# PatrykChrabaszcz/HpBandSter

Hardware: AMD Instinct MI355X
Metric: candidate KDE evals/sec (cand×obs pairs) at D=32, 1/2/4/8 MI355X; % VALU peak (higher is better)
Workload: dtype f16 MFMA coarse pre-screen (1 product per dim, rigorous bound), f32 accumulate, f64 re-score

## Files before the change

### hpbandster_amd/_native.py

```python

import ctypes
import os
import threading

_HERE = os.path.dirname(os.path.abspath(__file__))
LIB_PATH = os.environ.get("HBX_LIB_PATH") or os.path.join(_HERE, "_lib", "libhbx.so")
DIAGNOSTIC_BUILD = bool(os.environ.get("HBX_LIB_PATH"))

_lock = threading.Lock()
_lib = None

c_i32, c_i64, c_f64p, c_vp = ctypes.c_int32, ctypes.c_int64, ctypes.c_void_p, ctypes.c_void_p

SIGNATURES = {
    "hbx_last_error": (ctypes.c_char_p, []),
    "hbx_version": (ctypes.c_char_p, []),
    "hbx_kde_param_bytes": (c_i64, []),
    "hbx_kde_param_bw_offset": (c_i64, []),
    "hbx_kde_est_bytes": (c_i64, []),
    "hbx_acq_result_bytes": (c_i64, []),
    "hbx_max_dims": (c_i32, []),
    "hbx_sort_scratch_bytes": (c_i64, [c_i64]),
    "hbx_seg_argsort": (c_i32, [c_vp, c_vp, c_i64, c_i64, c_i64, c_vp, c_vp, c_i64, c_vp]),
    "hbx_kde_fit": (c_i32, [c_vp, c_i32, c_vp, c_i64, c_vp, c_vp, c_vp, c_vp, c_vp, c_vp, c_vp, c_vp, c_vp,
                            c_vp, c_vp]),
    "hbx_kde_bucket": (c_i32, [c_i32, c_i32, c_vp, c_vp, c_vp]),
    "hbx_kde_table_floats": (c_i64, [c_i32, c_i32, c_i32]),
    "hbx_kde_prepare": (c_i32, [c_vp, c_i32, c_vp, c_i32, c_vp, c_vp, c_vp, c_vp, c_vp, c_i64, c_vp, c_vp]),
    "hbx_kde_refit_out_bytes": (c_i64, [c_i64, c_i32]),
    "hbx_kde_refit_scratch_bytes": (c_i64, [c_i64, c_i32]),
    "hbx_kde_refit": (c_i32, [c_vp, c_vp, c_i64, c_i32, c_vp, c_vp, c_i64, c_i64, c_i64, ctypes.c_double,
                              ctypes.c_double, c_vp, c_vp, c_i64, c_vp, c_vp, c_i64, c_vp, c_vp, c_i64, c_vp]),
    "hbx_kde_refit_sync": (c_i32, [c_vp, c_vp, c_i64, c_i32, c_vp, c_vp, c_i64, c_i64, c_i64, ctypes.c_double,
                                   ctypes.c_double, c_vp, c_vp, c_i64, c_vp, c_vp, c_i64, c_vp, c_vp, c_i64,
                                   c_vp, c_vp]),
    "hbx_stream_order": (c_i32, [c_vp, c_vp]),
    "hbx_kde_logpdf": (c_i32, [c_vp, c_i64, c_i32, c_vp, c_vp, c_i32, c_i32, c_i32, c_vp, c_vp]),
    "hbx_kde_workspace_bytes": (c_i64, [c_i64, c_i64]),
    "hbx_kde_acquire": (c_i32, [c_vp, c_i64, c_i64, c_vp, c_vp, c_vp, c_vp, c_i64, c_vp, c_vp]),
    "hbx_kde_pair_bind": (c_vp, [c_i32, c_vp, c_vp, c_vp, c_vp, c_i32, c_vp, c_vp, c_vp, c_vp, c_i32, c_i32, c_i32,
                                 c_i64]),
    "hbx_kde_acquire_bound": (c_i32, [c_vp, c_vp, c_i64, c_i64, c_vp, c_i64, c_vp, c_vp, c_vp, c_vp, c_vp]),
    "hbx_kde_pair_free": (None, [c_vp]),
    "hbx_kde_batch_workspace_bytes": (c_i64, [c_i64, c_i64, c_i64]),
    "hbx_kde_acquire_batch": (c_i32, [c_vp, c_i64, c_i64, c_i64, c_vp, c_vp, c_vp, c_vp, c_vp, c_i64, c_vp]),
    "hbx_kde_topk_workspace_bytes": (c_i64, [c_i64, c_i32, c_i64]),
    "hbx_kde_topk_result_bytes": (c_i64, [c_i32]),
    "hbx_kde_acquire_topk": (c_i32, [c_vp, c_i64, c_i32, c_i64, c_vp, c_vp, c_vp, c_i64, c_vp]),
    "hbx_kde_groups_workspace_bytes": (c_i64, [c_i64, c_i64, c_i32]),
    "hbx_kde_acquire_groups": (c_i32, [c_vp, c_i32, c_vp, c_i64, c_vp, c_vp, c_vp, c_vp, c_vp, c_vp, c_vp, c_vp,
                                       c_vp, c_i64, c_vp, c_vp, c_i64, c_vp]),
    "hbx_kde_groups_batch_workspace_bytes": (c_i64, [c_i64, c_i64, c_i64, c_i32]),
    "hbx_kde_acquire_groups_batch": (c_i32, [c_vp, c_i32, c_vp, c_i64, c_vp, c_vp, c_vp, c_vp, c_vp, c_vp, c_vp,
                                             c_vp, c_vp, c_i64, c_i64, c_vp, c_vp, c_i64, c_vp]),
    "hbx_kde_groups_topk_workspace_bytes": (c_i64, [c_i64, c_i64, c_i32, c_i32]),
    "hbx_kde_acquire_groups_topk": (c_i32, [c_vp, c_i32, c_vp, c_i64, c_vp, c_vp, c_vp, c_vp, c_vp, c_vp, c_vp, c_vp,
                                            c_vp, c_i64, c_i32, c_vp, c_vp, c_i64, c_vp]),
    "hbx_kde_logpdf_groups_workspace_bytes": (c_i64, [c_i64, c_i64, c_i32]),
    "hbx_kde_logpdf_groups": (c_i32, [c_vp, c_i32, c_vp, c_i64, c_vp, c_vp, c_vp, c_vp, c_vp, c_vp, c_vp, c_vp, c_vp,
                                      c_i64, ctypes.c_double, c_i32, c_vp, c_vp, c_vp, c_vp, c_i64, c_vp]),
    "hbx_kde_logpdf_groups_stats": (c_i32, [c_vp, c_vp]),
    "hbx_kde_sample_groups": (c_i32, [c_vp, c_i32, c_vp, c_i64, c_vp, c_vp, c_vp, c_vp, ctypes.c_double,
                                      ctypes.c_uint64, ctypes.c_uint64, ctypes.c_uint32, c_i64, c_vp, c_vp, c_vp]),
    "hbx_kde_finish_groups": (c_i32, [c_vp, c_vp, c_vp, c_vp, c_i32, c_i64, c_i64, c_i64, ctypes.c_double,
                                      ctypes.c_uint64, ctypes.c_uint64, ctypes.c_uint32, c_vp, c_vp, c_vp]),
    "hbx_kde_propose_groups_workspace_bytes": (c_i64, [c_i64, c_i64, c_i64, c_i32]),
    "hbx_kde_propose_groups_ws_offsets": (c_i32, [c_i64, c_i64, c_i64, c_i32, c_vp]),
    "hbx_kde_propose_groups": (c_i32, [c_vp, c_i32, c_vp, c_i64, c_vp, c_vp, c_vp, c_vp, c_vp, c_vp, c_vp, c_vp, c_vp,
                                       ctypes.c_double, ctypes.c_double, ctypes.c_uint64, ctypes.c_uint64,
                                       ctypes.c_uint32, c_i64, c_i64, c_vp, c_vp, c_vp, c_vp, c_vp, c_i64, c_vp]),
    "hbx_philox4x32_10": (c_i32, [c_vp, c_vp, c_vp]),
    "hbx_kde_sample": (c_i32, [c_vp, c_i32, c_vp, c_i64, c_vp, c_vp, c_vp, ctypes.c_double, ctypes.c_uint64,
                               ctypes.c_uint64, ctypes.c_uint32, c_i64, c_vp, c_vp, c_vp, c_vp]),
    "hbx_norm_ppf": (c_i32, [c_vp, c_i64, c_vp, c_vp]),
    "hbx_kde_sample_table_bytes": (c_i64, [c_i64, c_i32]),
    "hbx_kde_sample_table": (c_i32, [c_vp, c_i32, c_vp, c_i64, c_vp, c_vp, c_vp, c_vp]),
    "hbx_kde_cv_terms": (c_i32, [c_vp, c_i64, c_i32, c_vp, c_vp, c_vp, c_vp, c_vp, ctypes.c_double,
                                 ctypes.c_double, ctypes.c_double, c_vp, c_vp, c_vp]),
    "hbx_event_create": (c_i32, [c_vp]),
    "hbx_event_destroy": (c_i32, [c_vp]),
    "hbx_event_elapsed_ms": (c_i32, [c_vp, c_vp, c_vp]),
    "hbx_kde_result_ptr": (c_vp, [c_vp]),
    "hbx_fetch": (c_i32, [c_vp, c_vp, c_i64, c_vp]),
    "hbx_mapped_host_buffers": (c_i64, []),
    "hbx_kde_ws_offsets": (c_i32, [c_i64, c_i64, c_i64, c_vp]),
    "hbx_kde_acquire_stats": (c_i32, [c_vp, c_i64, c_i64, c_vp]),
    "hbx_np_exp": (c_i32, [c_vp, c_i64, c_vp, c_vp]),
    "hbx_kde_pdf_scratch_bytes": (c_i64, [c_i64]),
    "hbx_kde_pdf_exact": (c_i32, [c_vp, c_i64, c_i32, c_vp, c_vp, c_vp, c_i64, c_vp, c_vp, c_i64, c_vp]),
    "hbx_kde_logpdf_exact": (c_i32, [c_vp, c_i64, c_i32, c_vp, c_vp, c_vp, c_vp, c_vp]),
    "hbx_rccl_unique_id_bytes": (c_i64, []),
    "hbx_rccl_get_unique_id": (c_i32, [c_vp]),
    "hbx_rccl_comm_init": (c_i32, [c_vp, c_i32, c_vp, c_i32, c_i32]),
    "hbx_rccl_comm_count": (c_i32, [c_vp, c_vp]),
    "hbx_rccl_comm_destroy": (c_i32, [c_vp]),
    "hbx_argmax_gather_bytes": (c_i64, [c_i32]),
    "hbx_argmax_allreduce": (c_i32, [c_vp, c_vp, c_vp, c_i32, c_vp, c_vp]),
    "hbx_argmax_records": (c_i32, [c_vp, c_i32, c_vp, c_vp]),
    "hbx_sh_promote": (c_i32, [c_vp, c_vp, c_i64, c_i64, c_i64, c_vp, c_vp, c_vp, c_vp, c_vp, c_i64, c_vp]),
    "hbx_seg_argsort_ex": (c_i32, [c_vp, c_vp, c_i64, c_i64, c_i64, c_vp, c_vp, c_i64, c_i32, c_vp]),
    "hbx_sh_promote_scratch_bytes": (c_i64, [c_i64, c_i64, c_i64, c_i32, c_i32]),
    "hbx_sh_promote_ex": (c_i32, [c_vp, c_vp, c_i64, c_i64, c_i64, c_vp, c_vp, c_vp, c_vp, c_vp, c_i64, c_i32,
                                  c_vp, c_vp]),
    "hbx_sh_promote_one": (c_i32, [c_vp, c_i64, ctypes.c_double, c_vp, c_vp, c_i32, c_vp, c_i32, c_vp]),
    "hbx_sh_advance_mapped": (c_i32, [c_vp, c_i64, ctypes.c_double, c_vp, c_vp, c_vp, c_vp, c_i32, c_vp, c_i32,
                                      c_vp]),
    "hbx_sh_advance_state": (c_i32, [c_vp, c_i64, ctypes.c_double, c_vp]),
    "hbx_host_alloc": (c_i32, [c_i64, c_vp]),
    "hbx_kde_logpdf_rtol_scratch_bytes": (c_i64, [c_i64]),
    "hbx_kde_logpdf_rtol": (c_i32, [c_vp, c_i64, c_i32, c_vp, c_vp, c_vp, c_vp, c_i32, c_i32, c_i32, ctypes.c_double,
                                    c_vp, c_vp, c_i64, c_vp]),
    "hbx_host_free": (c_i32, [c_vp]),
    "hbx_np_argsort_host": (c_i32, [c_vp, c_i64, c_vp]),
    "hbx_sh_advance_host": (c_i32, [c_vp, c_i64, c_i64, c_vp, c_vp]),
    "hbx_mt_state_bytes": (c_i64, []),
    "hbx_mt_draw": (c_i32, [c_vp, c_i32, c_i64, c_i64, c_vp]),
    "hbx_bohb_draw": (c_i32, [c_vp, c_vp, c_i64, c_i32, c_vp, c_vp, ctypes.c_double, c_i64, c_vp, c_vp, c_vp, c_vp,
                              c_vp, c_vp, c_vp]),
}

ORDER_NUMPY = 0
ORDER_STABLE = 1


def order_mode(name):
    if name in ("numpy", ORDER_NUMPY):
        return ORDER_NUMPY
    if name in ("stable", ORDER_STABLE):
        return ORDER_STABLE
    raise ValueError("tie order must be 'numpy' or 'stable', got %r" % (name,))


class HbxError(RuntimeError):
    pass


def lib():
    global _lib
    if _lib is not None:
        return _lib
    with _lock:
        if _lib is not None:
            return _lib
        if not os.path.exists(LIB_PATH):
            raise HbxError("libhbx.so not found at %s -- build it with `python -m hpbandster_amd.build` "
                           "(the engine has no CPU fallback)" % LIB_PATH)
        import torch
        L = ctypes.CDLL(LIB_PATH)
        for name, (res, args) in SIGNATURES.items():
            if DIAGNOSTIC_BUILD and not hasattr(L, name):
                continue
            f = getattr(L, name)
            f.restype = res
            f.argtypes = args
        _lib = L
        return _lib


def check(rc):
    if rc != 0:
        msg = lib().hbx_last_error()
        raise HbxError("libhbx error %d: %s" % (rc, msg.decode() if msg else "?"))


def call(name, *args):
    check(getattr(lib(), name)(*args))


def ptr(t):
    if t is None:
        return None
    if hasattr(t, "data_ptr"):
        return t.data_ptr()
    return t.ctypes.data


_RAW = None


def _raw_fns():
    global _RAW
    if _RAW is None:
        import torch
        _RAW = (getattr(torch._C, "_cuda_getDevice", None), getattr(torch._C, "_cuda_getCurrentRawStream", None))
    return _RAW


def stream_handle(stream=None, device=None):
    if stream is not None:
        return stream.cuda_stream
    import torch
    raw = _raw_fns()[1]
    if raw is not None:
        idx = None if device is None else device if isinstance(device, int) else torch.device(device).index
        return raw(torch.cuda.current_device() if idx is None else int(idx))
    return torch.cuda.current_stream(device).cuda_stream


def home_stream(dev_index):
    cur, raw = _RAW or _raw_fns()
    if cur is not None and raw is not None and cur() == dev_index:
        return raw(dev_index)
    return None


class on_device(object):

    def __init__(self, device, stream=None):
        import torch
        self._ctx = [torch.cuda.device(device)]
        if stream is not None:
            self._ctx.append(torch.cuda.stream(stream))

    def __enter__(self):
        for c in self._ctx:
            c.__enter__()
        return self

    def __exit__(self, *exc):
        for c in reversed(self._ctx):
            c.__exit__(*exc)
        return False
```

### hpbandster_amd/csrc/hbx_acquire.h

```cpp
#pragma once
#include "hbx_score.h"

struct KdePairRef {
  int32_t D;
  const void* params_good;
  const float* table_good;
  const double* X_good;
  const int64_t* rows_good;
  int32_t variant_good;
  const void* params_bad;
  const float* table_bad;
  const double* X_bad;
  const int64_t* rows_bad;
  int32_t variant_bad, dc_pad, du_pad;
  int64_t nmax;
  const KdeParams* Pg() const { return (const KdeParams*)params_good; }
  const KdeParams* Pb() const { return (const KdeParams*)params_bad; }
};

struct WsLayout {
  size_t res, U, count, flags, segcnt, segnear, best, key, first1, rescue, est_l, est_g, lo, list, near, exact_l,
      exact_g, part, total;
  size_t stage, seeds, surv, lpart;
  int32_t list_cap;
};
#define STAGED_LIST_CAP 4096
WsLayout ws_layout(int64_t Nc, int64_t nmax, int64_t B = 1);

struct AcqWs {
  AcqResult* res;
  uint32_t* U;
  int32_t *count, *flags, *segcnt, *segnear;
  uint64_t *best, *key;
  int32_t *first1, *rescue;
  KdeEst *el, *eg;
  float* lo;
  int32_t *list, *near;
  double *exact_l, *exact_g, *part;
  uint32_t* stage;
  int32_t *seeds, *surv;
  KdeEst* lpart;
  int32_t list_cap;
  AcqWs(void* workspace, const WsLayout& w) {
    char* ws = (char*)workspace;
    res = (AcqResult*)(ws + w.res);
    U = (uint32_t*)(ws + w.U);
    count = (int32_t*)(ws + w.count);
    flags = (int32_t*)(ws + w.flags);
    segcnt = (int32_t*)(ws + w.segcnt);
    segnear = (int32_t*)(ws + w.segnear);
    best = (uint64_t*)(ws + w.best);
    key = (uint64_t*)(ws + w.key);
    first1 = (int32_t*)(ws + w.first1);
    rescue = (int32_t*)(ws + w.rescue);
    el = (KdeEst*)(ws + w.est_l);
    eg = (KdeEst*)(ws + w.est_g);
    lo = (float*)(ws + w.lo);
    list = (int32_t*)(ws + w.list);
    near = (int32_t*)(ws + w.near);
    exact_l = (double*)(ws + w.exact_l);
    exact_g = (double*)(ws + w.exact_g);
    part = (double*)(ws + w.part);
    stage = (uint32_t*)(ws + w.stage);
    seeds = (int32_t*)(ws + w.seeds);
    surv = (int32_t*)(ws + w.surv);
    lpart = (KdeEst*)(ws + w.lpart);
    list_cap = w.list_cap;
  }
  KdePairArgs::AcqInitPtrs init() const { return {U, count, flags, first1, res}; }
};

struct AcqPlan {
  ScoreFns fg, fb;
  bool exact_only;
};
const KdePairRef* acq_pair(const char* who, const void* pair);
int acq_check(const char* who, const KdePairRef& p, const double* cand, int64_t Nc, const void* workspace);
int acq_plan(const KdePairRef& p, bool fast, AcqPlan* plan);
int acq_score(const AcqPlan& plan, const KdePairRef& p, const AcqWs& a, const ScoreRequest& rq, int64_t batch_B,
              ScoreResult* out);
#ifndef HBX_STAGED_MIN_PAIRS
#define HBX_STAGED_MIN_PAIRS 1e9
#endif
#ifndef HBX_STAGED_TOPK_MIN_PAIRS
#define HBX_STAGED_TOPK_MIN_PAIRS 4e9
#endif
bool acq_staged_supported(const AcqPlan& plan);
int acq_score_staged(const AcqPlan& plan, const KdePairRef& p, const double* cand, int64_t Nc, const AcqWs& a,
                     hipEvent_t* ev, hipStream_t s, bool tail);
int staged_score_l(const AcqPlan& plan, const KdePairRef& p, const double* cand, int64_t Nc, const AcqWs& a,
                   hipEvent_t* ev, hipStream_t s, uint32_t* lkey, uint32_t* hist, int32_t hist_words);
int staged_score_seeds(const AcqPlan& plan, const KdePairRef& p, const double* cand, int64_t Nc, const AcqWs& a,
                       hipStream_t s, bool mark_rest, bool update_u);
int staged_score_survivors(const AcqPlan& plan, const KdePairRef& p, const double* cand, int64_t Nc, const AcqWs& a,
                           hipStream_t s, bool lonly);
int acq_exact_only_init(int64_t Nc, uint32_t seg, const AcqWs& a, hipStream_t s);
#define EXACT_SCAN_MAX 1024
int acq_exact(const KdePairRef& p, const double* cand, int64_t Nc, const AcqWs& a, bool scan, bool combine,
              hipStream_t s);
```

### hpbandster_amd/csrc/hbx_common.h

```cpp
#pragma once

#include <hip/hip_runtime.h>
#include <stdint.h>
#include <stdlib.h>

#define HBX_MAX_D 256
#define HBX_WAVE 64

#include "hbx.h"

int hbx_fail(int code, const char* fmt, ...);

#define HBX_HIP(call)                                                                 \
  do {                                                                                \
    hipError_t _e = (call);                                                           \
    if (_e != hipSuccess)                                                             \
      return hbx_fail(HBX_ERR_HIP, "%s failed: %s (%s:%d)", #call, hipGetErrorString(_e), \
                      __FILE__, __LINE__);                                            \
  } while (0)

#define HBX_LAUNCH_CHECK()                                                            \
  do {                                                                                \
    hipError_t _e = hipGetLastError();                                                \
    if (_e != hipSuccess)                                                             \
      return hbx_fail(HBX_ERR_HIP, "kernel launch failed: %s (%s:%d)",               \
                      hipGetErrorString(_e), __FILE__, __LINE__);                    \
  } while (0)

static inline bool hbx_switch_on(const char* name) {
  const char* e = getenv(name);
  return !(e && atoi(e) == 0);
}
static inline int hbx_staged_mode() {
  const char* e = getenv("HBX_STAGED");
  if (!e) return 1;
  const int v = atoi(e);
  return v == 0 ? 0 : v == 2 ? 2 : 1;
}
static inline bool hbx_staged_tail() { return hbx_switch_on("HBX_STAGED_TAIL"); }

struct KdeParams {
  int32_t n;
  int32_t D;
  int32_t dc;
  int32_t du;
  int32_t nconst;
  int32_t nan_all;
  int32_t has_neg;
  int32_t unsupported;
  int32_t stride;
  int32_t dc_pad;
  int32_t du_pad;
  int32_t exact_only;
  double log_norm;
  double m0_log2;
  double lb_sum;
  double prod_bw_c;
  float cmax;
  float sum_abs_delta;
  float cmax2;
  int32_t pad1;
  int32_t kc;
  int32_t hmode;
  int32_t nsc;
  int32_t chunk_floats;
  int32_t oh_total;
  int32_t coarse_off;
  int32_t coarse_chunk_floats;
  const double* X;
  const int64_t* rows;
  int32_t oh_dim[64];
  int32_t oh_level[64];
  int32_t oh_col[64];
  double oh_val[64];
  int32_t oh_start[64];
  int32_t cat_maxcode[HBX_MAX_D];
  int32_t cont_dim[HBX_MAX_D];
  double cont_scale[HBX_MAX_D];
  double center[HBX_MAX_D];
  float xmax[HBX_MAX_D];
  int32_t cat_dim[HBX_MAX_D];
  float cat_delta[HBX_MAX_D];
  float cat_negf[HBX_MAX_D];
  int32_t const_dim[HBX_MAX_D];
  double const_level[HBX_MAX_D];
  int32_t vartype[HBX_MAX_D];
  int32_t nlev[HBX_MAX_D];
  double bw[HBX_MAX_D];
};

#define HBX_PARAM_STAGE ((sizeof(KdeParams) + 255) & ~(size_t)255)
#define HBX_COLSTATS_OFF (HBX_PARAM_STAGE + 8 * HBX_MAX_D + 4 * HBX_MAX_D + 64)
#define HBX_PARAM_BYTES (HBX_COLSTATS_OFF + 8 * HBX_MAX_D + 4 * HBX_MAX_D)
struct ColStats {
  double mean[HBX_MAX_D];
  int32_t maxcode[HBX_MAX_D];
};

struct KdeEst {
  float lpos;
  float lneg;
  float err;
  float pad;
};

struct AcqResult {
  int64_t index;
  double score;
  float rel;
  int32_t flags;
  int32_t shortlist;
  int32_t near;
  double pdf_l;
  double pdf_g;
};

__device__ __forceinline__ void hbx_publish_store(uint32_t* dst, uint32_t v) {
  __hip_atomic_store(dst, v, __ATOMIC_RELAXED, __HIP_MEMORY_SCOPE_SYSTEM);
}
__device__ __forceinline__ void hbx_publish_store64(uint64_t* dst, uint64_t v) {
  __hip_atomic_store(dst, v, __ATOMIC_RELAXED, __HIP_MEMORY_SCOPE_SYSTEM);
}
__device__ __forceinline__ void hbx_publish_done(int32_t* done, int32_t seq) {
  __asm__ volatile("s_waitcnt vmcnt(0)" ::: "memory");
  __hip_atomic_store(done, seq, __ATOMIC_RELAXED, __HIP_MEMORY_SCOPE_SYSTEM);
}

__device__ __forceinline__ uint32_t hbx_f2ord(float f) {
  uint32_t u = __float_as_uint(f);
  return (u & 0x80000000u) ? ~u : (u | 0x80000000u);
}
__device__ __forceinline__ float hbx_ord2f(uint32_t u) {
  return __uint_as_float((u & 0x80000000u) ? (u & 0x7fffffffu) : ~u);
}

__device__ __forceinline__ uint64_t hbx_d2ord(double d) {
  if (d != d) return ~0ull;
  if (d == 0.0) d = 0.0;
  uint64_t u = (uint64_t)__double_as_longlong(d);
  return (u & 0x8000000000000000ull) ? ~u : (u | 0x8000000000000000ull);
}

template <typename Op>
__device__ __forceinline__ uint32_t wave_reduce_dpp(uint32_t v, Op op) {
  v = op(v, (uint32_t)__builtin_amdgcn_update_dpp(0, (int)v, 0xb1, 0xf, 0xf, false));
  v = op(v, (uint32_t)__builtin_amdgcn_update_dpp(0, (int)v, 0x4e, 0xf, 0xf, false));
  v = op(v, (uint32_t)__builtin_amdgcn_update_dpp(0, (int)v, 0x141, 0xf, 0xf, false));
  v = op(v, (uint32_t)__builtin_amdgcn_update_dpp(0, (int)v, 0x140, 0xf, 0xf, false));
  return op(op((uint32_t)__builtin_amdgcn_readlane((int)v, 0), (uint32_t)__builtin_amdgcn_readlane((int)v, 16)),
            op((uint32_t)__builtin_amdgcn_readlane((int)v, 32), (uint32_t)__builtin_amdgcn_readlane((int)v, 48)));
}
struct OpAdd { __device__ uint32_t operator()(uint32_t a, uint32_t b) const { return a + b; } };
struct OpAnd { __device__ uint32_t operator()(uint32_t a, uint32_t b) const { return a & b; } };
struct OpOr { __device__ uint32_t operator()(uint32_t a, uint32_t b) const { return a | b; } };
struct OpMax { __device__ uint32_t operator()(uint32_t a, uint32_t b) const { return a > b ? a : b; } };
```

### hpbandster_amd/csrc/hbx_kde.hip

```cpp
#include "hbx_acquire.h"

#include <string.h>

#include <new>

#include "hbx_acq_impl.h"
#include "hbx_host.h"
#include "hbx_pairwise.h"
#include "hbx_rescue_impl.h"


__global__ void acq_init_kernel(uint32_t* U, int32_t* count, int32_t* flags, int32_t* first1, AcqResult* res) {
  if (threadIdx.x == 0 && blockIdx.x == 0) acq_init_state(U, count, flags, first1, res);
}

__global__ void acq_init_batch_kernel(int64_t B, uint32_t* __restrict__ U, int32_t* __restrict__ flags,
                                      int32_t* __restrict__ segcnt, uint64_t* __restrict__ best,
                                      uint64_t* __restrict__ key, int32_t* __restrict__ first1,
                                      int32_t* __restrict__ count, int32_t* __restrict__ segnear) {
  const int64_t b = (int64_t)blockIdx.x * blockDim.x + threadIdx.x;
  if (b == 0) *count = 0;
  if (b < B) {
    U[b] = hbx_f2ord(INFINITY);
    flags[b] = 0;
// ... 160 lines not shown
  const bool all = (flags[sg] & 1) != 0;
  const float l = lo[i];
  if ((l == l && (all || l <= u)) || (int32_t)i == first1[sg]) {
    const int pos = atomicAdd(count, 1);
    list[pos] = (int32_t)i;
    if (segcnt) atomicAdd(segcnt + sg, 1);
  }
}

struct PickOut {
  const double* cand;
  const uint8_t* err;
  int64_t Nc;
  int32_t D;
  char* out;
};

__global__ __launch_bounds__(256) void kde_final_kernel(const int32_t* __restrict__ list,
                                                        const int32_t* __restrict__ count,
                                                        const double* exact_l,
                                                        const double* exact_g, const int32_t* __restrict__ flags,
                                                        int64_t index_base, const KdeParams* __restrict__ Pg,
                                                        const KdeParams* __restrict__ Pb,
                                                        const KdeEst* __restrict__ el, const KdeEst* __restrict__ eg,
                                                        int32_t* __restrict__ near_list, AcqResult* __restrict__ res,
                                                        int32_t nbuf, const double* __restrict__ part,
                                                        double* exact_lw, double* exact_gw, AcqResult* host_res,
                                                        int32_t seq, PickOut pick) {
  __shared__ double bs[256];
  __shared__ AcqResult rec_sh;
  __shared__ int64_t bi[256];
  __shared__ int32_t bp[256];
  __shared__ double exl[256], exg[256];
  __shared__ double rb_sh;
  __shared__ int32_t nnear;
  const int cnt = *count;
  int err_any = 0;
  if (pick.out && pick.err) {
    bool e = false;
    for (int64_t i = threadIdx.x; i < pick.Nc; i += 256) e = e || pick.err[i] != 0;
    err_any = __syncthreads_or(e);
  }
  const bool small = cnt <= 256;
  const int tp = threadIdx.x;
  const int64_t my_idx = (small && tp < cnt) ? list[tp] : 0;
  const double my_rel = (small && tp < cnt) ? score_rel(Pg, Pb, el, eg, my_idx) : 0.0;
  if (part && cnt <= EXACT_SPLIT_CAP) {
    for (int pk = threadIdx.x >> 6; pk < 2 * cnt; pk += 4) {
      const bool isl = pk & 1;
      const int n = (isl ? Pg : Pb)->n;
      const double* us = part + (int64_t)pk * nbuf * PW_SPLIT_UNITS;
      double acc = 0.0;
      for (int c = 0, b = 0; c < n; c += PW_BUF, ++b) {
        const int m = (n - c) < PW_BUF ? (n - c) : PW_BUF;
        acc = acc + pw_combine_units_wave<PW_SPLIT_CUT>(m, us + b * PW_SPLIT_UNITS);
      }
      if ((threadIdx.x & 63) == 0) {
        const double pdf = acc / (double)n;
        (isl ? exact_lw : exact_gw)[pk >> 1] = pdf;
        if (small) (isl ? exl : exg)[pk >> 1] = pdf;
      }
    }
    __threadfence_block();
    __syncthreads();
  } else if (small) {
    if (tp < cnt) {
      exl[tp] = exact_l[tp];
      exg[tp] = exact_g[tp];
    }
    __syncthreads();
  }
  double best = INFINITY;
  int64_t bidx = INT64_MAX;
  int32_t bpos = -1;
  if (threadIdx.x == 0) nnear = 0;
  for (int p = threadIdx.x; p < cnt; p += 256) {
    const double s = bohb_score(small ? exg[p] : exact_g[p], small ? exl[p] : exact_l[p]);
    const int64_t idx = small ? my_idx : list[p];
    if (s < INFINITY && (s < best || (s == best && idx < bidx))) {
      best = s;
      bidx = idx;
      bpos = p;
    }
  }
  bs[threadIdx.x] = best;
  bi[threadIdx.x] = bidx;
  bp[threadIdx.x] = bpos;
  __syncthreads();
  for (int w = 128; w > 0; w >>= 1) {
    if (threadIdx.x < w) {
      const double s2 = bs[threadIdx.x + w];
      const int64_t i2 = bi[threadIdx.x + w];
      if (s2 < bs[threadIdx.x] || (s2 == bs[threadIdx.x] && i2 < bi[threadIdx.x])) {
        bs[threadIdx.x] = s2;
        bi[threadIdx.x] = i2;
        bp[threadIdx.x] = bp[threadIdx.x + w];
      }
    }
    __syncthreads();
  }
  const int32_t wp = bp[0];
  double rb = 0.0;
  if (small) {
    if (tp == wp) rb_sh = my_rel;
    __syncthreads();
    if (wp >= 0) rb = rb_sh;
  }
  if (wp >= 0) {
    const double sb = bs[0];
    if (!small) rb = score_rel(Pg, Pb, el, eg, list[wp]);
    for (int p = threadIdx.x; p < cnt; p += 256) {
      const double s = bohb_score(small ? exg[p] : exact_g[p], small ? exl[p] : exact_l[p]);
      const int64_t ip = small ? my_idx : list[p];
      if (p == wp || near_best(s, small ? my_rel : score_rel(Pg, Pb, el, eg, ip), sb, rb))
        near_list[atomicAdd(&nnear, 1)] = (int32_t)ip;
    }
  }
  __syncthreads();
  if (threadIdx.x == 0) {
    AcqResult r;
    r.index = -1;
    r.score = r.pdf_l = r.pdf_g = NAN;
    r.shortlist = cnt;
    r.flags = *flags | (nnear > 1 ? HBX_ACQ_NEAR_TIE : 0);
    r.near = nnear;
    r.rel = (float)rb;
    if (wp >= 0) {
      r.index = bi[0] + index_base;
      r.score = bs[0];
      r.pdf_l = small ? exl[wp] : exact_l[wp];
      r.pdf_g = small ? exg[wp] : exact_g[wp];
    }
    *res = r;
    rec_sh = r;
  }
  if (host_res || pick.out) {
    static_assert(sizeof(AcqResult) % 4 == 0, "record of whole words");
    __syncthreads();
    uint64_t* out = (uint64_t*)(pick.out ? pick.out : (char*)host_res);
    const uint64_t tag = (uint64_t)(uint32_t)seq << 32;
    constexpr int RW = (int)(sizeof(AcqResult) / 4);
    if (threadIdx.x < RW) hbx_publish_store64(out + threadIdx.x, tag | ((const uint32_t*)&rec_sh)[threadIdx.x]);
    if (pick.out) {
      if (threadIdx.x == 0) hbx_publish_store64(out + RW, tag | (err_any ? 1u : 0u));
      const int64_t idx = rec_sh.index - index_base;
      if (rec_sh.index >= 0 && idx < pick.Nc)
        for (int w = threadIdx.x; w < 2 * pick.D; w += 256)
          hbx_publish_store64(out + RW + 1 + w, tag | ((const uint32_t*)(pick.cand + idx * pick.D))[w]);
    }
  }
}


__global__ __launch_bounds__(256) void kde_batch_min_kernel(const int32_t* __restrict__ list,
                                                            const int32_t* __restrict__ count, uint32_t seg,
                                                            const double* __restrict__ exact_l,
                                                            const double* __restrict__ exact_g,
                                                            uint64_t* __restrict__ best) {
  const int p = blockIdx.x * 256 + threadIdx.x;
  if (p >= *count) return;
  const double s = bohb_score(exact_g[p], exact_l[p]);
  if (s < INFINITY) atomicMin((unsigned long long*)best + (uint32_t)list[p] / seg,
                              (unsigned long long)__double_as_longlong(s));
}

__global__ __launch_bounds__(256) void kde_batch_key_kernel(const int32_t* __restrict__ list,
                                                            const int32_t* __restrict__ count, uint32_t seg,
                                                            const double* __restrict__ exact_l,
                                                            const double* __restrict__ exact_g,
                                                            const uint64_t* __restrict__ best,
                                                            uint64_t* __restrict__ key) {
  const int p = blockIdx.x * 256 + threadIdx.x;
  if (p >= *count) return;
  const double s = bohb_score(exact_g[p], exact_l[p]);
  const uint32_t i = (uint32_t)list[p], sg = i / seg;
  if (s < INFINITY && (uint64_t)__double_as_longlong(s) == best[sg])
    atomicMin((unsigned long long*)key + sg, ((unsigned long long)(i - sg * seg) << 32) | (uint32_t)p);
}

__global__ __launch_bounds__(256) void kde_batch_near_kernel(const int32_t* __restrict__ list,
                                                             const int32_t* __restrict__ count, uint32_t seg,
                                                             const double* __restrict__ exact_l,
                                                             const double* __restrict__ exact_g,
                                                             const uint64_t* __restrict__ key,
                                                             const KdeParams* __restrict__ Pg,
                                                             const KdeParams* __restrict__ Pb,
                                                             const KdeEst* __restrict__ el,
                                                             const KdeEst* __restrict__ eg,
                                                             int32_t* __restrict__ near_flag,
                                                             int32_t* __restrict__ segnear) {
  const int p = blockIdx.x * 256 + threadIdx.x;
  if (p >= *count) return;
  const uint32_t i = (uint32_t)list[p], sg = i / seg;
  const uint64_t k = key[sg];
  int f = 0;
  if (k != ~0ull) {
    const int wp = (int)(uint32_t)k;
    const double sb = bohb_score(exact_g[wp], exact_l[wp]);
    const double rb = score_rel(Pg, Pb, el, eg, list[wp]);
    const double s = bohb_score(exact_g[p], exact_l[p]);
    f = (p == wp || near_best(s, score_rel(Pg, Pb, el, eg, i), sb, rb)) ? 1 : 0;
  }
  near_flag[p] = f;
  if (f) atomicAdd(segnear + sg, 1);
}

__global__ __launch_bounds__(256) void kde_batch_final_kernel(int64_t B, const uint64_t* __restrict__ key,
                                                              const int32_t* __restrict__ segcnt,
                                                              const int32_t* __restrict__ flags,
                                                              const int32_t* __restrict__ segnear,
                                                              const int32_t* __restrict__ list,
                                                              const double* __restrict__ exact_l,
                                                              const double* __restrict__ exact_g,
                                                              const KdeParams* __restrict__ Pg,
                                                              const KdeParams* __restrict__ Pb,
                                                              const KdeEst* __restrict__ el,
                                                              const KdeEst* __restrict__ eg,
                                                              int64_t index_base, AcqResult* __restrict__ res) {
  const int64_t b = (int64_t)blockIdx.x * 256 + threadIdx.x;
  if (b >= B) return;
  AcqResult r;
  r.shortlist = segcnt[b];
  r.near = segnear[b];
  r.flags = flags[b] | (r.near > 1 ? HBX_ACQ_NEAR_TIE : 0);
  r.rel = 0.f;
  const uint64_t k = key[b];
  if (k == ~0ull) {
    r.index = -1;
    r.score = NAN;
    r.pdf_l = NAN;
    r.pdf_g = NAN;
  } else {
    const int p = (int)(uint32_t)k;
    r.index = (int64_t)(k >> 32) + index_base;
    r.pdf_l = exact_l[p];
    r.pdf_g = exact_g[p];
    r.score = bohb_score(r.pdf_g, r.pdf_l);
    r.rel = (float)score_rel(Pg, Pb, el, eg, list[p]);
  }
  res[b] = r;
}

__global__ __launch_bounds__(256) void kde_exact_only_init_kernel(int64_t Nc, uint32_t seg, KdeEst* __restrict__ el,
                                                                  KdeEst* __restrict__ eg, float* __restrict__ lo,
                                                                  int32_t* __restrict__ flags) {
  const int64_t i = (int64_t)blockIdx.x * 256 + threadIdx.x;
  if (i >= Nc) return;
  const KdeEst e = {0.f, -INFINITY, -2.f, 0.f};
  el[i] = e;
  eg[i] = e;
  lo[i] = 0.f;
  if ((uint32_t)i % seg == 0) flags[(uint32_t)i / seg] = HBX_ACQ_OVERFLOW;
}

__global__ __launch_bounds__(256) void kde_exact_logs_kernel(const int32_t* __restrict__ list,
                                                             const int32_t* __restrict__ count,
                                                             const double* __restrict__ exact_l,
                                                             const double* __restrict__ exact_g,
                                                             float* __restrict__ logl, float* __restrict__ logg) {
  const int p = blockIdx.x * 256 + threadIdx.x;
  if (p >= *count) return;
  const int i = list[p];
  if (logl) logl[i] = (float)log(exact_l[p]);
  if (logg) logg[i] = (float)log(exact_g[p]);
}


WsLayout ws_layout(int64_t Nc, int64_t nmax, int64_t B) {
  WsLayout w;
  size_t o = 0;
  auto take = [&](size_t bytes) {
    size_t r = o;
    o += (bytes + 255) & ~(size_t)255;
    return r;
  };
  w.res = take(sizeof(AcqResult));
  w.count = take(4);
  w.U = take(4 * B);
  w.flags = take(4 * B);
  w.segcnt = take(4 * B);
  w.segnear = take(4 * B);
  w.best = take(8 * B);
  w.key = take(8 * B);
  w.first1 = take(4 * B);
  w.rescue = take(4);
  const int sp = obs_splits((unsigned)((Nc + 511) / 512), nmax, true);
  const int64_t cap16 = 16 * Nc < 196608 ? 16 * Nc : 196608;
  const int64_t nest = Nc * sp > cap16 ? Nc * sp : cap16;
  w.est_l = take(sizeof(KdeEst) * nest);
  w.est_g = take(sizeof(KdeEst) * nest);
  w.lo = take(4 * Nc);
  w.list = take(4 * Nc);
  w.near = take(4 * Nc);
  w.exact_l = take(8 * Nc);
  w.exact_g = take(8 * Nc);
  w.part = take(8 * (size_t)2 * EXACT_SPLIT_CAP * PW_SPLIT_UNITS * ((nmax + PW_BUF - 1) / PW_BUF));
  static_assert(sizeof(AcqResult) + 4 * HBX_ST_WORDS <= 256, "the state words fit the result slot's padding");
  w.stage = w.res + sizeof(AcqResult);
  const int64_t tiles = (Nc + 511) / 512;
  w.list_cap = (int32_t)(512 * (tiles < 1 ? 1 : tiles > STAGED_LIST_CAP / 512 ? STAGED_LIST_CAP / 512 : tiles));
  w.seeds = take(4 * (size_t)w.list_cap);
  w.surv = take(4 * Nc);
  w.lpart = take(sizeof(KdeEst) * (size_t)OBS_SPLIT_MAX * w.list_cap);
  w.total = o;
  return w;
}

int acq_check(const char* who, const KdePairRef& p, const double* cand, int64_t Nc, const void* workspace) {
  if ((!cand && Nc > 0) || !p.params_good || !p.table_good || !p.X_good || !p.rows_good || !p.params_bad ||
      !p.table_bad || !p.X_bad || !p.rows_bad || !workspace)
    return hbx_fail(HBX_ERR_ARG, "%s: null pointer", who);
  if (Nc < 0 || Nc > INT32_MAX) return hbx_fail(HBX_ERR_ARG, "Nc=%lld out of range", (long long)Nc);
  return HBX_OK;
}

const KdePairRef* acq_pair(const char* who, const void* pair) {
  if (!pair) hbx_fail(HBX_ERR_ARG, "%s: null pair", who);
  return (const KdePairRef*)pair;
}

int acq_plan(const KdePairRef& p, bool fast, AcqPlan* plan) {
  plan->exact_only = KdeVariant::decode(p.variant_good).exact_only || KdeVariant::decode(p.variant_bad).exact_only;
  plan->fg = pick_logpdf(p.dc_pad, p.du_pad, p.variant_good, fast);
  plan->fb = pick_logpdf(p.dc_pad, p.du_pad, p.variant_bad, fast);
  if (!plan->exact_only && (!plan->fg.main || !plan->fb.main))
    return hbx_fail(HBX_ERR_UNSUPPORTED, "no kernel for dc_pad=%d du_pad=%d", p.dc_pad, p.du_pad);
  return HBX_OK;
}

int acq_score(const AcqPlan& plan, const KdePairRef& p, const AcqWs& a, const ScoreRequest& rq, int64_t batch_B,
              ScoreResult* out) {
  *out = ScoreResult{};
  const hipStream_t s = rq.s;
  const bool scored = rq.Nc > 0 && !plan.exact_only;
  if (scored) {
    const int rc = launch_score2({plan.fg, p.params_good, p.table_good, a.el},
                                 {plan.fb, p.params_bad, p.table_bad, a.eg}, rq, out);
    if (rc) return rc;
  }
  if (batch_B) {
    hipLaunchKernelGGL(acq_init_batch_kernel, dim3((unsigned)((batch_B + 255) / 256)), dim3(256), 0, s, batch_B, a.U,
                       a.flags, a.segcnt, a.best, a.key, a.first1, a.count, a.segnear);
    HBX_LAUNCH_CHECK();
  } else if (!out->inited) {
    hipLaunchKernelGGL(acq_init_kernel, dim3(1), dim3(64), 0, s, a.U, a.count, a.flags, a.first1, a.res);
    HBX_LAUNCH_CHECK();
  }
  if (scored && (out->nsplit[0] > 1 || out->nsplit[1] > 1)) {
    hipLaunchKernelGGL(kde_merge_splits_kernel, dim3((unsigned)((2 * rq.Nc + 255) / 256)), dim3(256), 0, s, a.el,
                       a.eg, rq.Nc, out->nsplit[0], out->nsplit[1]);
    HBX_LAUNCH_CHECK();
  }
  return HBX_OK;
}

int acq_exact_only_init(int64_t Nc, uint32_t seg, const AcqWs& a, hipStream_t s) {
  hipLaunchKernelGGL(kde_exact_only_init_kernel, dim3((unsigned)((Nc + 255) / 256)), dim3(256), 0, s, Nc, seg, a.el,
                     a.eg, a.lo, a.flags);
  HBX_LAUNCH_CHECK();
  return HBX_OK;
}

struct AcqCall {
  const char* who;
  const double* cand;
  int64_t Nc, seg, index_base;
  float *logl_out, *logg_out;
  AcqResult* batch_res;
  void* workspace;
  int64_t ws_bytes;
  void *events, *stream;
  AcqResult* host_res;
  int32_t seq;
  PickOut pick;
};

static int acquire_impl(const void* pair, const AcqCall& c) {
  const KdePairRef* pp = acq_pair(c.who, pair);
  if (!pp) return HBX_ERR_ARG;
  const KdePairRef& p = *pp;
  const double* cand = c.cand;
  const int64_t Nc = c.Nc, seg = c.seg;
  float *logl_out = c.logl_out, *logg_out = c.logg_out;
  AcqResult* batch_res = c.batch_res;
  int rc = acq_check(c.who, p, cand, Nc, c.workspace);
  if (rc) return rc;
  if (seg < 1) return hbx_fail(HBX_ERR_ARG, "%s: segment length %lld", c.who, (long long)seg);
  const int64_t B = batch_res ? (Nc + seg - 1) / seg : 1;
  const WsLayout w = ws_layout(Nc, p.nmax, B);
  if ((size_t)c.ws_bytes < w.total)
    return hbx_fail(HBX_ERR_ARG, "workspace too small: %lld < %lld bytes", (long long)c.ws_bytes,
                    (long long)w.total);
  const bool fast = !logl_out && !logg_out;
  AcqPlan plan;
  rc = acq_plan(p, fast, &plan);
  if (rc) return rc;
  const AcqWs a(c.workspace, w);
  hipStream_t s = (hipStream_t)c.stream;
  hipEvent_t* ev = (hipEvent_t*)c.events;
  const uint32_t sg = (uint32_t)(batch_res ? seg : (Nc > 0 ? Nc : 1));
  if (B == 0) return HBX_OK;
  bool rescue_inline = false;
  const int stg = (!batch_res && fast && Nc > 0) ? hbx_staged_mode() : 0;
  const bool staged = stg && acq_staged_supported(plan) &&
                      (stg == 2 || (double)Nc * (double)p.nmax >= HBX_STAGED_MIN_PAIRS);
  const bool tail = staged && hbx_staged_tail();
  if (staged) {
    rc = acq_score_staged(plan, p, cand, Nc, a, ev, s, tail);
    rescue_inline = true;
  } else {
    const ScoreRequest rq{cand, Nc, p.D, ev, a.rescue, batch_res ? KdePairArgs::AcqInitPtrs{} : a.init(),
                          fast ? p.nmax : 0, !batch_res, s};
    ScoreResult sr;
    rc = acq_score(plan, p, a, rq, batch_res ? B : 0, &sr);
    rescue_inline = sr.rescue_inline;
  }
  if (rc) return rc;
  const dim3 grid((unsigned)((Nc + 255) / 256));
  bool fuse_combine = false;
  if (Nc > 0) {
    if (plan.exact_only) {
      rc = acq_exact_only_init(Nc, sg, a, s);
      if (rc) return rc;
    } else if (!tail) {
      const CombineRescue rs{cand, p.D, p.Pg(), p.Pb(), a.rescue};
      const bool sgn = KdeVariant::decode(p.variant_good).has_neg;
      const combine_fn cf = !rescue_inline ? kde_combine_kernel<false, false>
                            : sgn          ? kde_combine_kernel<true, true>
                                           : kde_combine_kernel<false, true>;
      hipLaunchKernelGGL(cf, dim3((unsigned)((Nc + 256 * COMBINE_SUB - 1) / (256 * COMBINE_SUB))), dim3(256), 0, s,
                         a.el, a.eg, Nc, sg, logl_out, logg_out, a.lo, a.U, a.flags, a.first1, rs);
      HBX_LAUNCH_CHECK();
    }
    const bool scan = !batch_res && Nc <= EXACT_SCAN_MAX && !tail;
    if (!scan && !tail) {
      hipLaunchKernelGGL(kde_shortlist_kernel, grid, dim3(256), 0, s, a.lo, Nc, sg, a.U, a.flags, a.list, a.count,
                         batch_res ? a.segcnt : (int32_t*)nullptr, a.first1, a.rescue);
      HBX_LAUNCH_CHECK();
    }
    fuse_combine = !batch_res && !(plan.exact_only && (logl_out || logg_out));
    rc = acq_exact(p, cand, Nc, a, scan, !fuse_combine, s);
    if (rc) return rc;
    if (plan.exact_only && (logl_out || logg_out)) {
      hipLaunchKernelGGL(kde_exact_logs_kernel, grid, dim3(256), 0, s, a.list, a.count, a.exact_l, a.exact_g, logl_out,
                         logg_out);
      HBX_LAUNCH_CHECK();
    }
  }
  if (!batch_res) {
    hipLaunchKernelGGL(kde_final_kernel, dim3(1), dim3(256), 0, s, a.list, a.count, a.exact_l, a.exact_g, a.flags,
                       c.index_base, p.Pg(), p.Pb(), a.el, a.eg, a.near, a.res,
                       (int32_t)((p.nmax + PW_BUF - 1) / PW_BUF), fuse_combine ? a.part : (const double*)nullptr,
                       a.exact_l, a.exact_g, c.host_res, c.seq, c.pick);
    HBX_LAUNCH_CHECK();
    return HBX_OK;
  }
  if (Nc > 0) {
    hipLaunchKernelGGL(kde_batch_min_kernel, grid, dim3(256), 0, s, a.list, a.count, sg, a.exact_l, a.exact_g, a.best);
    HBX_LAUNCH_CHECK();
    hipLaunchKernelGGL(kde_batch_key_kernel, grid, dim3(256), 0, s, a.list, a.count, sg, a.exact_l, a.exact_g, a.best,
                       a.key);
    HBX_LAUNCH_CHECK();
    hipLaunchKernelGGL(kde_batch_near_kernel, grid, dim3(256), 0, s, a.list, a.count, sg, a.exact_l, a.exact_g, a.key,
                       p.Pg(), p.Pb(), a.el, a.eg, a.near, a.segnear);
    HBX_LAUNCH_CHECK();
    hipLaunchKernelGGL(kde_batch_final_kernel, dim3((unsigned)((B + 255) / 256)), dim3(256), 0, s, B, a.key, a.segcnt,
                       a.flags, a.segnear, a.list, a.exact_l, a.exact_g, p.Pg(), p.Pb(), a.el, a.eg, c.index_base,
                       batch_res);
    HBX_LAUNCH_CHECK();
  }
  return HBX_OK;
}

extern "C" {

int64_t hbx_kde_workspace_bytes(int64_t Nc, int64_t nmax) { return (int64_t)ws_layout(Nc, nmax).total; }

int64_t hbx_kde_batch_workspace_bytes(int64_t Nc, int64_t seg, int64_t nmax) {
  if (seg < 1) return -1;
  return (int64_t)ws_layout(Nc, nmax, (Nc + seg - 1) / seg).total;
}

void* hbx_kde_result_ptr(void* workspace) { return (char*)workspace + ws_layout(0, 0).res; }

int hbx_kde_acquire(const double* cand, int64_t Nc, int64_t index_base, const void* pair, float* logl_out,
                    float* logg_out, void* workspace, int64_t ws_bytes, void* events, void* stream) {
  return acquire_impl(pair, {"hbx_kde_acquire", cand, Nc, Nc > 0 ? Nc : 1, index_base, logl_out, logg_out, nullptr,
                             workspace, ws_bytes, events, stream, nullptr, 0, PickOut{}});
}

int hbx_kde_acquire_batch(const double* cand, int64_t Nc, int64_t seg, int64_t index_base, const void* pair,
                          float* logl_out, float* logg_out, void* results, void* workspace, int64_t ws_bytes,
                          void* stream) {
  if (!results) return hbx_fail(HBX_ERR_ARG, "hbx_kde_acquire_batch: null results");
  return acquire_impl(pair, {"hbx_kde_acquire_batch", cand, Nc, seg, index_base, logl_out, logg_out,
                             (AcqResult*)results, workspace, ws_bytes, nullptr, stream, nullptr, 0, PickOut{}});
}

void* hbx_kde_pair_bind(int32_t D, const void* params_good, const float* table_good, const double* X_good,
                        const int64_t* rows_good, int32_t variant_good, const void* params_bad,
                        const float* table_bad, const double* X_bad, const int64_t* rows_bad, int32_t variant_bad,
                        int32_t dc_pad, int32_t du_pad, int64_t nmax) {
  if (D <= 0 || D > HBX_MAX_D || !params_good || !params_bad || nmax < 0) {
    hbx_fail(HBX_ERR_ARG, "hbx_kde_pair_bind: bad arguments (D=%d, nmax=%lld)", D, (long long)nmax);
    return nullptr;
  }
  KdePairRef* b = new (std::nothrow) KdePairRef{D, params_good, table_good, X_good, rows_good, variant_good,
                                                params_bad, table_bad, X_bad, rows_bad, variant_bad, dc_pad,
                                                du_pad, nmax};
  if (!b) hbx_fail(HBX_ERR_ARG, "hbx_kde_pair_bind: out of host memory");
  return b;
}

void hbx_kde_pair_free(void* pair) { delete (KdePairRef*)pair; }

int hbx_kde_acquire_bound(const void* pair, const double* cand, int64_t Nc, int64_t index_base, void* workspace,
                          int64_t ws_bytes, const uint8_t* err, void* events, void* stream, void* rec_out,
                          double* row_out) {
  const char* who = "hbx_kde_acquire_bound";
  if (!pair || !rec_out || Nc < 0) return hbx_fail(HBX_ERR_ARG, "hbx_kde_acquire_bound: bad arguments");
  const KdePairRef& b = *(const KdePairRef*)pair;
  MappedBuf* mb = nullptr;
  int rc = hbx_mapped_acq(&mb);
  if (rc) return rc;
  char* pub = mb->p + PUB_OFF;
  const int32_t seq = mb->seq;
  const hipStream_t s = (hipStream_t)stream;
  const bool pick = err || row_out;
  rc = acquire_impl(pair, {who, cand, Nc, Nc > 0 ? Nc : 1, index_base, nullptr, nullptr, nullptr, workspace, ws_bytes,
                           events, stream, pick ? nullptr : (AcqResult*)pub, seq,
                           pick ? PickOut{cand, err, Nc, b.D, pub} : PickOut{}});
  if (rc) return rc;
  constexpr int RW = (int)(sizeof(AcqResult) / 4);
  constexpr int64_t SPIN = 20000000;
  const volatile uint64_t* w = (const volatile uint64_t*)pub;
  uint32_t words[RW];
  rc = wait_tagged(w, RW, seq, words, s, SPIN, who);
  if (rc) return rc;
  AcqResult r;
  memcpy(&r, words, sizeof(AcqResult));
  if (pick) {
    uint32_t e = 0;
    rc = wait_tagged(w + RW, 1, seq, &e, s, SPIN, who);
    if (rc) return rc;
    if (e) r.flags |= HBX_ACQ_DOMAIN_ERR;
    if (row_out && r.index >= 0 && r.index - index_base < Nc) {
      rc = wait_tagged(w + RW + 1, 2 * b.D, seq, (uint32_t*)row_out, s, SPIN, who);
      if (rc) return rc;
    }
  }
  memcpy(rec_out, &r, sizeof(AcqResult));
  return HBX_OK;
}

int hbx_kde_ws_offsets(int64_t Nc, int64_t seg, int64_t nmax, int64_t* out) {
  if (!out || seg < 1) return hbx_fail(HBX_ERR_ARG, "hbx_kde_ws_offsets: bad arguments");
  const WsLayout w = ws_layout(Nc, nmax, seg >= Nc ? 1 : (Nc + seg - 1) / seg);
  out[0] = (int64_t)w.count;
  out[1] = (int64_t)w.list;
  out[2] = (int64_t)w.near;
  out[3] = (int64_t)w.exact_l;
  out[4] = (int64_t)w.exact_g;
  return HBX_OK;
}

}
```

### hpbandster_amd/csrc/hbx_kde_impl.h

```cpp
#pragma once
#include <math.h>
#include <stdlib.h>
#include <string.h>

#include <vector>

#include "hbx_common.h"

#define HBX_LN2f 0.69314718055994531f
#define HBX_LN_CLAMP (-18.420680743952367)
#define HBX_INV_SQRT_2PI 0.3989422804014327
#ifndef EXACT_GRID
#define EXACT_GRID 2048
#endif
#define SUM_BLOCK 32
#define OBS_CHUNK 64
#define KROW 80
#define MFMA_WAVES 8
#ifndef H_ROW_TILES
#define H_ROW_TILES 2
#endif
#ifndef H_WAVES_PER_EU
#if H_ROW_TILES <= 2
#define H_WAVES_PER_EU 4
#else
#define H_WAVES_PER_EU 2
#endif
#endif
#define H16_WAVES 8
#ifndef H32C_WAVES
#define H32C_WAVES 8
#endif
#ifndef H32C_EU
#define H32C_EU 4
#endif
#ifndef H32C_CT
#define H32C_CT 2
#endif
#define H32C_ROW_DS 33
#define H32C_ROW_DMIN 16

#define OH_MAX_KC 4
__host__ __device__ constexpr int kp_of(int dc_pad) { return (dc_pad + 2 + 3) & ~3; }
__host__ __device__ constexpr int cat_floats(int du_pad, int kc, int sgn) {
  return kc == 0 ? OBS_CHUNK * du_pad : OBS_CHUNK * kc * 16 * (sgn ? 2 : 1);
}
__host__ __device__ constexpr int chunk_floats(int dc_pad, int du_pad, int kc = 0, int sgn = 0) {
  return kp_of(dc_pad) * KROW + cat_floats(du_pad, kc, sgn);
}
#define H_CMAX 60000.f
__host__ __device__ constexpr int nsc_of(int dc_pad) { return (4 * dc_pad + 31) / 32; }
__host__ __device__ constexpr int h_ktp(int dc_pad, int kc) { return 32 * (nsc_of(dc_pad) + kc) + 16; }
__host__ __device__ constexpr int h_kpp(int kc) { return 32 * kc + 16; }
__host__ __device__ constexpr int h_chunk_floats(int dc_pad, int kc, int sgn) {
  return (OBS_CHUNK + OBS_CHUNK * h_ktp(dc_pad, kc) / 2 + (sgn ? OBS_CHUNK * h_kpp(kc) / 2 : 0) + 2047) & ~2047;
}
__host__ __device__ constexpr int h32_nd(int nsc) { return (6 + 24 * nsc + 15) / 16; }
__host__ __device__ constexpr int h32_kp(int kc) { return (kc + 1) / 2; }
__host__ __device__ constexpr bool h32_ok(int nsc, int kp, int sgn = 0) {
  return kp <= 2 && (h32_nd(nsc) + 2 * kp <= 8 || (nsc == 4 && kp == 1)) && (!sgn || kp >= 1);
}
__host__ __device__ constexpr int h32_ksp(int kp) { return kp == 3 ? 4 : kp; }
__host__ __device__ constexpr int h32_ixw(int kp) { return kp == 1 ? 4 : 2 * h32_ksp(kp); }
__host__ __device__ constexpr int h32_par(int nsc, int kp) {
  return (16 * h32_nd(nsc) + 32 * kp + 2 * h32_ixw(kp) + 7) & ~7;
}
__host__ __device__ constexpr int h32_ktp(int nsc, int kp, int sgn = 0) {
  return 8 * (((h32_par(nsc, kp) + (sgn ? 16 * kp : 0) + 7) / 8) | 1);
}
__host__ __device__ constexpr int h32_chunk_floats(int nsc, int kp, int sgn = 0) {
  return (OBS_CHUNK * h32_ktp(nsc, kp, sgn) / 2 + 255) & ~255;
}
#define H32_ROW_MAX 112
__host__ __device__ constexpr int h32c_nd(int nsc) { return (6 + 8 * nsc + 15) / 16; }
__host__ __device__ constexpr int h32c_par(int nsc, int kp) { return (16 * h32c_nd(nsc) + 16 * kp + 2 * h32_ixw(kp) + 7) & ~7; }
__host__ __device__ constexpr int h32c_ktp(int nsc, int kp) { return 8 * (((h32c_par(nsc, kp) + 7) / 8) | 1); }
__host__ __device__ constexpr int h32c_chunk_floats(int nsc, int kp) {
  return (OBS_CHUNK * h32c_ktp(nsc, kp) / 2 + 255) & ~255;
}
struct KdeVariant {
  int has_neg;
  int kc;
  int hmode;
  int exact_only;
  int h32;
  int coarse;
  int small_codes;
  __host__ __device__ int encode() const {
    return has_neg | (kc << 1) | (hmode << 4) | (exact_only << 5) | (h32 << 6) | (coarse << 7) | (small_codes << 8);
  }
  __host__ __device__ static KdeVariant decode(int v) {
    return {v & 1, (v >> 1) & 7, (v >> 4) & 1, (v >> 5) & 1, (v >> 6) & 1, (v >> 7) & 1, (v >> 8) & 1};
  }
};


typedef float f32x4 __attribute__((ext_vector_type(4)));

__device__ __forceinline__ float cat_match(float a, float b) {
  const float d = a - b;
  return __builtin_amdgcn_fmed3f(fmaf(-d, d, 1.f), 0.f, 1.f);
}

__device__ __forceinline__ float cand_code(double xv) {
  return (xv == rint(xv) && fabs(xv) < 1e6) ? (float)xv : -1e9f;
}

__device__ __forceinline__ KdeEst finish_est_terms(const KdeParams* __restrict__ P, float S, float Sn, float off,
                                                   bool nan_c, float ci, float bnd, bool SIGNED, float sum_terms) {
  KdeEst o;
  o.pad = 0.f;
  if (nan_c || S != S) {
    o.lpos = NAN;
    o.lneg = -INFINITY;
    o.err = 0.f;
    return o;
  }
  const float lnorm = (float)P->log_norm;
  const float Sp = SIGNED ? (S - Sn) : S;
  o.lpos = (Sp > 0.f) ? (__log2f(Sp) + off) * HBX_LN2f + lnorm : -INFINITY;
  o.lneg = (SIGNED && Sn > 0.f) ? (__log2f(Sn) + off) * HBX_LN2f + lnorm : -INFINITY;
  const float u = 0x1p-24f;
  const float Mabs = fabsf(ci) + P->cmax + bnd + P->sum_abs_delta;
  const float dt = 3.f * (float)(P->dc + P->du + 4) * u * Mabs;
  const float es = sum_terms * u * (SIGNED ? 3.f : 1.f);
  o.err = 2.f * (dt * HBX_LN2f + es) + 16.f * u;
  return o;
}

__device__ __forceinline__ KdeEst finish_est(const KdeParams* __restrict__ P, float S, float Sn, float off,
                                             bool nan_c, float ci, float bnd, bool SIGNED, int chunk) {
  return finish_est_terms(P, S, Sn, off, nan_c, ci, bnd, SIGNED,
                          (float)chunk + (float)P->n / (float)chunk + 24.f);
}

__device__ __forceinline__ void stage_rows(const double* __restrict__ src, int64_t nv, int D, int DS, double* xs,
                                           int lane) {
  if (D <= 64) {
    const int rpp = 64 / D;
    const int lr = lane / D, lc = lane - lr * D;
    if (lr < rpp) {
      const int npf = (int)nv / rpp;
      const unsigned vo = (unsigned)(lr * D + lc), xo = (unsigned)(lr * DS + lc);
      const int sq = __builtin_amdgcn_readfirstlane(rpp * D), xq = __builtin_amdgcn_readfirstlane(rpp * DS);
      for (int p0 = 0; p0 < npf; p0 += 16) {
        double t[16];
#pragma unroll
        for (int q = 0; q < 16; ++q)
          if (p0 + q < npf) t[q] = (src + (int64_t)(p0 + q) * sq)[vo];
#pragma unroll
        for (int q = 0; q < 16; ++q)
          if (p0 + q < npf) (xs + (p0 + q) * xq)[xo] = t[q];
      }
      const int row = npf * rpp + lr;
      if (row < (int)nv) xs[row * DS + lc] = src[row * D + lc];
    }
    return;
  }
  const int tot = (int)nv * D;
  for (int e0 = 0; e0 < tot; e0 += 16 * 64) {
    double t[16];
    int at[16];
#pragma unroll
    for (int q = 0; q < 16; ++q) {
      const int e = min(e0 + 64 * q + lane, tot - 1);
      const int row = e / D;
      at[q] = row * DS + (e - row * D);
      t[q] = src[e];
    }
#pragma unroll
    for (int q = 0; q < 16; ++q) xs[at[q]] = t[q];
  }
}

typedef _Float16 f16x8 __attribute__((ext_vector_type(8)));
typedef _Float16 f16x16 __attribute__((ext_vector_type(16)));

typedef void (*logpdf_fn)(const double*, int64_t, int32_t, const KdeParams*, const float*, KdeEst*);

#ifndef HBX_PAIR_INIT
#define HBX_PAIR_INIT 1
#endif

struct KdePairArgs {
  const KdeParams* P0;
  const KdeParams* P1;
  const float* table0;
  const float* table1;
  KdeEst* out0;
  KdeEst* out1;
  unsigned nblk0;
  int32_t* rescue;
  struct AcqInitPtrs {
    uint32_t* U;
    int32_t* count;
    int32_t* flags;
    int32_t* first1;
    struct AcqResult* res;
  } init;
  unsigned tiles = 0;
  int32_t nsplit0 = 1, nsplit1 = 1;
  int32_t row_stage = 1;
};
typedef void (*logpdf_pair_fn)(const double*, int64_t, int32_t, KdePairArgs);
typedef void (*logpdf_co_fn)(const double*, int64_t, int32_t, const KdeParams*, const float*, KdeEst*, int32_t);

struct KdeListArgs {
  const KdeParams* P;
  const float* table;
  KdeEst* out;
  KdeEst* part;
  const int32_t* idx;
  const int32_t* count;
  int32_t* rescue;
  int32_t cap, maxcount, nsplit;
  unsigned tiles_cap;
  int32_t row_stage;
};
typedef void (*logpdf_list_fn)(const double*, int32_t, KdeListArgs);

enum {
  HBX_ST_FLAG = 0,
  HBX_ST_LMAX,
  HBX_ST_USEED,
  HBX_ST_NSEED,
  HBX_ST_NSURV,
  HBX_ST_NPRE,
  HBX_ST_WORDS
};

__device__ __forceinline__ void acq_init_state(uint32_t* U, int32_t* count, int32_t* flags, int32_t* first1,
                                               AcqResult* res) {
  uint32_t* st = (uint32_t*)(res + 1);
  st[HBX_ST_FLAG] = 0;
  st[HBX_ST_LMAX] = hbx_f2ord(-INFINITY);
  st[HBX_ST_USEED] = hbx_f2ord(INFINITY);
  st[HBX_ST_NSEED] = 0;
  st[HBX_ST_NSURV] = 0;
  st[HBX_ST_NPRE] = 0;
  *U = hbx_f2ord(INFINITY);
  *first1 = INT32_MAX;
  *count = 0;
  *flags = 0;
  res->index = -1;
  res->score = NAN;
  res->pdf_l = NAN;
  res->pdf_g = NAN;
  res->shortlist = 0;
  res->flags = 0;
  res->near = 0;
  res->rel = 0.f;
}

__host__ __device__ inline KdeEst kde_est_neutral() {
  KdeEst e;
  e.lpos = -INFINITY;
  e.lneg = -INFINITY;
  e.err = 0.f;
  e.pad = 0.f;
  return e;
}

__host__ __device__ inline void obs_split_range(int nchunks, int r, int nsplit, int* c0, int* nch) {
  const int per = (nchunks + nsplit - 1) / nsplit;
  *c0 = r * per;
  const int e = (*c0 + per) < nchunks ? (*c0 + per) : nchunks;
  *nch = e - *c0;
}

struct RefitMeta {
  int64_t seg[2];
  int64_t n_good, n_bad;
  double fac_good, fac_bad;
  int32_t vt[HBX_MAX_D];
};
struct RefitMetaArgs {
  int64_t n, n_good, n_bad;
  double fac_good, fac_bad;
  int32_t D;
  uint32_t vt[HBX_MAX_D / 32];
};
#define REFIT_SORT_SMALL 1024
#define REFIT_INLINE 256
int refit_sort_small(double* X, double* loss, const double* staged, const double* staged_inline, int64_t n_new,
                     const RefitMetaArgs& a, RefitMeta* m, int64_t* order, int32_t* arrays, hipStream_t s);

int refit_fit_colstats(const double* X, int32_t D, const int64_t* seg_off, const int64_t* order, const int64_t* n_good,
                       const int64_t* n_bad, const double* fac_good, const double* fac_bad, const int32_t* vartype,
                       double* bw_good, double* bw_bad, int32_t* nlev_good, int32_t* nlev_bad, ColStats* cs_good,
                       ColStats* cs_bad, hipStream_t s);
#define FIT_TILE_ROWS 16384

logpdf_fn hbx_pick_f32(int dc_pad, int du_pad, bool sg);
logpdf_fn hbx_pick_oh(int dc_pad, int kc, bool sg);
logpdf_fn hbx_pick_h(int nsc, int kc, bool sg);
logpdf_pair_fn hbx_pick_h_pair(int nsc, int kc, bool sg);
logpdf_fn hbx_pick_h32(int nsc, int kp, bool sg, bool fast);
logpdf_co_fn hbx_pick_h32_co(int nsc, int kp);
logpdf_pair_fn hbx_pick_h32_pair(int nsc, int kp, bool sg, bool fast, bool coarse = false);
logpdf_pair_fn hbx_pick_h32_pair1(int nsc, int kp);
logpdf_list_fn hbx_pick_h32_list(int nsc, int kp);

int hbx_logpdf_estimate(const double* cand, int64_t Nc, int32_t D, const void* params, const float* table,
                        int32_t dc_pad, int32_t du_pad, int32_t variant, KdeEst* est, hipStream_t s);
int hbx_logpdf_exact_listed(const double* cand, int64_t Nc, int32_t D, const KdeParams* P, const double* X,
                            const int64_t* rows, double* out, const int32_t* list, const int32_t* count,
                            bool per_point, hipStream_t s);
```

### hpbandster_amd/csrc/hbx_prep.hip

```cpp
#include <math.h>
#include <string.h>

#include "hbx_prep.h"
#include "hbx_sort.h"

__host__ __device__ static int table_stride(int dc_pad, int du_pad) { return chunk_floats(dc_pad, du_pad); }
static int64_t n_chunks(int64_t n) { return (n + OBS_CHUNK - 1) / OBS_CHUNK; }
__device__ __forceinline__ int64_t n_chunks_dev(int64_t n) { return (n + OBS_CHUNK - 1) / OBS_CHUNK; }
static int64_t table_floats(int64_t n, int dc_pad, int du_pad) {
  if (dc_pad < 0 || du_pad < 0) return 1;
  int a = chunk_floats(dc_pad, du_pad, 0, 0), b = chunk_floats(dc_pad, du_pad, OH_MAX_KC, 1);
  const int c = h_chunk_floats(dc_pad, OH_MAX_KC, 1), d = h32_chunk_floats(nsc_of(dc_pad), OH_MAX_KC, 1);
  a = a > b ? a : b;
  a = a > d ? a : d;
  const int e = h32c_chunk_floats(nsc_of(dc_pad), 2);
  return n_chunks(n) * (int64_t)((a > c ? a : c) + e);
}

__device__ __forceinline__ void prep_publish_rows(const PrepPub& q, int k, int t, int nt) {
  const uint64_t tag = (uint64_t)(uint32_t)q.seq << 32;
  auto put = [&](int64_t i, uint32_t w) {
    __hip_atomic_store(q.dst + i, tag | w, __ATOMIC_RELAXED, __HIP_MEMORY_SCOPE_SYSTEM);
  };
  if (k == 0) {
    const int64_t* order = (const int64_t*)q.src;
    for (int i = t; i < q.n; i += nt) put(i, (uint32_t)order[i]);
  }
  const int64_t bw0 = (int64_t)q.n + 2 * (int64_t)q.D * k, nl0 = (int64_t)q.n + 4 * (int64_t)q.D + (int64_t)q.D * k;
  for (int i = t; i < 2 * q.D; i += nt) put(bw0 + i, q.src[q.bw_off[k] + i]);
  for (int i = t; i < q.D; i += nt) put(nl0 + i, q.src[q.nl_off[k] + i]);
}
__device__ __forceinline__ void prep_publish_vals(const PrepPub& q, const int32_t (&vals)[8], int k) {
  for (int i = 0; i < 8; ++i)
    __hip_atomic_store(q.ll + 8 * k + i, ((uint64_t)(uint32_t)q.seq << 32) | (uint32_t)vals[i], __ATOMIC_RELAXED,
                       __HIP_MEMORY_SCOPE_SYSTEM);
}
__device__ __forceinline__ void prep_publish_info(const PrepPub& q, const PrepArgs& A, int k) {
  for (int i = 0; i < 8; ++i)
    __hip_atomic_store(q.ll + 8 * k + i, ((uint64_t)(uint32_t)q.seq << 32) | (uint32_t)A.info[i], __ATOMIC_RELAXED,
                       __HIP_MEMORY_SCOPE_SYSTEM);
}

__device__ __forceinline__ bool prep_cat(const PrepArgs& A, int d) { return (A.vt[d >> 5] >> (d & 31)) & 1u; }


__global__ __launch_bounds__(256) void kde_colstats_kernel(PrepSet ps) {
  const PrepArgs& A = (int)blockIdx.x >= ps.k[0].D ? ps.k[1] : ps.k[0];
  const int d = blockIdx.x % ps.k[0].D;
  const int n = A.n, D = A.D;
  ColStats* cs = col_stats(A.P);
  __shared__ double red[4];
  __shared__ int mred[4];
  if (!prep_cat(A, d)) {
    double acc = 0.0;
    for (int j = threadIdx.x; j < n; j += 256) acc += A.X[A.rows[j] * (int64_t)D + d];
    for (int o = 32; o > 0; o >>= 1) acc += __shfl_xor(acc, o);
    if ((threadIdx.x & 63) == 0) red[threadIdx.x >> 6] = acc;
    __syncthreads();
    if (threadIdx.x == 0) cs->mean[d] = ((red[0] + red[1]) + (red[2] + red[3])) / (double)n;
  } else {
    int m = -1;
    for (int j = threadIdx.x; j < n; j += 256) {
      const double v = A.X[A.rows[j] * (int64_t)D + d];
      m = max(m, (!(v >= 0.0 && v < 1024.0) || v != floor(v)) ? 100000 : (int)v);
    }
    for (int o = 32; o > 0; o >>= 1) m = max(m, __shfl_xor(m, o));
    if ((threadIdx.x & 63) == 0) mred[threadIdx.x >> 6] = m;
    __syncthreads();
    if (threadIdx.x == 0) {
      const int mm = max(max(mred[0], mred[1]), max(mred[2], mred[3]));
      cs->maxcode[d] = mm >= 100000 ? -1 : mm;
    }
  }
}

__device__ __forceinline__ int32_t* prep_counter(KdeParams* P) {
  return (int32_t*)((char*)P + HBX_PARAM_STAGE + 8 * HBX_MAX_D + 4 * HBX_MAX_D + 32);
}

#ifdef PREP_STAMPS
__device__ unsigned long long prep_stamps[32];
#define PSTAMP(i) \
  if (threadIdx.x == 0) prep_stamps[i] = __builtin_amdgcn_s_memtime()
#else
#define PSTAMP(i)
#endif

struct ParamsScratch {
  double t0[HBX_MAX_D], t1[HBX_MAX_D], h[HBX_MAX_D], mean[HBX_MAX_D];
  int32_t c[HBX_MAX_D], maxc[HBX_MAX_D], cm[HBX_MAX_D], cd[HBX_MAX_D];
  int32_t ix[HBX_MAX_D];
  uint8_t kind[HBX_MAX_D];
  int32_t ohs[HBX_MAX_D];
  int32_t du, dcp, dup, exo, neg, dc_tot, du_tot, dc, nconst, kc, tot;
};

__device__ __forceinline__ void kde_params_body(const PrepArgs& A, KdeParams* P, const ColStats* cs, ParamsScratch& S) {
  const int D = A.D, n = A.n;
  const int tid = threadIdx.x;
  uint32_t* pz = (uint32_t*)P;
  for (int i = tid; i < (int)(sizeof(KdeParams) / 4); i += blockDim.x) pz[i] = 0u;
  if (tid == 0) S.neg = 0;
  const double LOG2E = 1.4426950408889634;
  if (blockIdx.x == 0) PSTAMP(0);
  for (int d = tid; d < D; d += blockDim.x) {
    const double h = A.bw[d];
    const int c = A.nlev[d];
    S.h[d] = h;
    S.c[d] = c;
    S.mean[d] = cs->mean[d];
    S.maxc[d] = cs->maxcode[d];
    if (!prep_cat(A, d)) {
      S.kind[d] = 0;
      S.t0[d] = (h > 0.0) ? log(h) : 0.0;
      S.t1[d] = (h > 0.0) ? sqrt(LOG2E / 2.0) / h : 0.0;
    } else {
      S.kind[d] = (c == 1 && h == 0.0) ? 2 : ((c < 2 || !(h > 0.0) || h != h) ? 3 : 1);
      const double a = 1.0 - h, b = h / (double)(c - 1);
      S.t0[d] = log2(b);
      S.t1[d] = (a == 0.0) ? -INFINITY : log2(fabs(a));
    }
  }
  __syncthreads();
  if (blockIdx.x == 0) PSTAMP(1);
  if (tid < 64) {
    const uint64_t below = (1ull << tid) - 1ull;
    int bc = 0, bu = 0, bk = 0, nu = 0;
    for (int g = 0; g < D; g += 64) {
      const int d = g + tid;
      const int kd = d < D ? S.kind[d] : -1;
      const uint64_t mc = __ballot(kd == 0), mu = __ballot(kd == 1), mk = __ballot(kd == 2), ma = __ballot(kd >= 1);
      if (d < D) S.ix[d] = kd == 0 ? bc + __popcll(mc & below) : kd == 1 ? bu + __popcll(mu & below)
                                                                         : bk + __popcll(mk & below);
      bc += __popcll(mc);
      bu += __popcll(mu);
      bk += __popcll(mk);
      nu += __popcll(ma);
    }
    if (tid == 0) {
      S.dc_tot = bc;
      S.du_tot = nu;
      S.du = bu;
      S.nconst = bk;
    }
  }
  __syncthreads();
  for (int d = tid; d < D; d += blockDim.x) {
    const double h = S.h[d];
    const int kd = S.kind[d], ix = S.ix[d];
    P->vartype[d] = kd != 0 ? 1 : 0;
    P->nlev[d] = S.c[d];
    P->bw[d] = h;
    if (kd == 0) {
      P->cont_dim[ix] = d;
      const double m = S.mean[d];
      P->center[ix] = (m == m && m - m == 0.0) ? m : 0.0;
      if (!(h > 0.0)) {
        P->nan_all = 1;
        P->cont_scale[ix] = 0.0;
      } else {
        P->cont_scale[ix] = S.t1[d];
      }
    } else if (kd == 2) {
      P->const_dim[ix] = d;
    } else if (kd == 3) {
      P->unsupported = 1;
    } else {
      const double a = 1.0 - h;
      P->cat_dim[ix] = d;
      P->cat_maxcode[ix] = S.maxc[d];
      S.cm[ix] = S.maxc[d];
      S.cd[ix] = d;
      P->cat_delta[ix] = (a == 0.0) ? -1e30f : (float)(S.t1[d] - S.t0[d]);
      P->cat_negf[ix] = (a < 0.0) ? 1.f : 0.f;
      if (a < 0.0) {
        P->has_neg = 1;
        S.neg = 1;
      }
    }
  }
  if (tid == 0) {
    double sum_ln_h = 0.0, m0 = 0.0, lb_sum = 0.0, prod_bw_c = 1.0;
    float sad = 0.f;
#pragma unroll 4
    for (int d = 0; d < D; ++d) {
      const int kd = S.kind[d];
      const double h = S.h[d], lb = S.t0[d], la = S.t1[d];
      prod_bw_c *= (kd == 0) ? h : 1.0;
      sum_ln_h += (kd == 0 && h > 0.0) ? lb : 0.0;
      m0 += (kd == 1) ? ((la > lb) ? la : lb) : 0.0;
      lb_sum += (kd == 1) ? lb : 0.0;
      sad += (kd == 1 && 1.0 - h != 0.0) ? fabsf((float)(la - lb)) : 0.f;
    }
    int dcp, dup;
    bucket_dims(S.dc_tot, S.du_tot, &dcp, &dup);
    P->n = n;
    P->D = D;
    P->dc_pad = dcp;
    P->du_pad = dup;
    const int exo = (dcp < 0 || dup < 0) ? 1 : 0;
    P->exact_only = exo;
    P->stride = exo ? 0 : table_stride(dcp, dup);
    const int dc = S.dc_tot;
    P->dc = dc;
    P->du = S.du;
    S.dcp = dcp;
    S.dup = dup;
    S.exo = exo;
    P->nconst = S.nconst;
    P->m0_log2 = m0;
    P->lb_sum = lb_sum;
    P->prod_bw_c = prod_bw_c;
    P->sum_abs_delta = sad;
    P->log_norm = -log((double)n) - sum_ln_h - 0.5 * (double)dc * log(2.0 * M_PI) + m0 * M_LN2;
    P->X = A.X;
    P->rows = A.rows;
  }
  __syncthreads();
  if (blockIdx.x == 0) PSTAMP(2);
  for (int t = tid; t < 64; t += blockDim.x) {
    P->oh_col[t] = 0;
    P->oh_val[t] = NAN;
  }
  const int du = S.du;
  if (tid == 0) {
    int tot = 0;
    bool ok = true;
    for (int u = 0; u < du; ++u) {
      if (S.cm[u] < 0) {
        ok = false;
      } else {
        S.ohs[u] = (tot + 1) & ~1;
        tot = S.ohs[u] + S.cm[u] + 1;
      }
    }
    S.kc = (!S.exo && du > 0 && ok && 2 * tot <= 32 * OH_MAX_KC && tot <= 64) ? (2 * tot + 31) / 32 : 0;
    S.tot = tot;
  }
  __syncthreads();
  const int kc = S.kc;
  if (kc > 0) {
    for (int u = tid; u < du; u += blockDim.x) {
      int t = S.ohs[u];
      P->oh_start[u] = t;
      if (t > 0 && (u == 0 || t != S.ohs[u - 1] + S.cm[u - 1] + 1)) {
        P->oh_dim[t - 1] = u;
        P->oh_level[t - 1] = -1;
      }
      for (int l = 0; l <= S.cm[u]; ++l, ++t) {
        P->oh_dim[t] = u;
        P->oh_level[t] = l;
        P->oh_col[t] = S.cd[u];
        P->oh_val[t] = (double)l;
      }
    }
  }
  if (threadIdx.x != 0) return;
  const int dcp = S.dcp, dup = S.dup, has_neg = S.neg;
  if (S.exo) {
    P->hmode = 0;
    P->nsc = 0;
    P->chunk_floats = 0;
    return;
  }
  if (kc > 0) {
    P->kc = kc;
    P->oh_total = S.tot;
  }
  const bool hm_ok = (du == 0 || kc > 0) && dcp >= 8;
  int hmode = (hm_ok && A.hm_allowed) ? 1 : 0;
  if (hmode && A.h32_allowed && h32_ok(nsc_of(dcp), h32_kp(kc), has_neg)) hmode = 2;
  P->hmode = hmode;
  P->nsc = nsc_of(dcp);
  P->chunk_floats = hmode == 2 ? h32_chunk_floats(nsc_of(dcp), h32_kp(kc), has_neg)
                               : (hmode ? h_chunk_floats(dcp, kc, has_neg) : chunk_floats(dcp, dup, kc, kc ? has_neg : 0));
  const bool co = hmode == 2 && !has_neg && A.co_allowed;
  P->coarse_chunk_floats = co ? h32c_chunk_floats(nsc_of(dcp), h32_kp(kc)) : 0;
  P->coarse_off = co ? (int32_t)(n_chunks_dev(n) * P->chunk_floats) : 0;
  if (blockIdx.x == 0) PSTAMP(3);
}

__global__ __launch_bounds__(256) void kde_params_kernel(PrepSet ps) {
  const PrepArgs& A = blockIdx.x ? ps.k[1] : ps.k[0];
  __shared__ ParamsScratch S;
  if (threadIdx.x == 0) *prep_counter(A.P) = 0;
  if (ps.pub.dst) prep_publish_rows(ps.pub, blockIdx.x ? 1 : 0, threadIdx.x, blockDim.x);
  kde_params_body(A, A.P, col_stats(A.P), S);
  if (ps.pub.dst) __asm__ volatile("s_waitcnt vmcnt(0)" ::: "memory");
}

__device__ __forceinline__ uint64_t onehot_hits(const double* x, const KdeParams* P, bool ok) {
  uint64_t hit = 0;
  if (!ok) return hit;
  for (int u = 0; u < P->du; ++u) {
    const double v = x[P->cat_dim[u]];
    if (v >= 0.0 && v <= (double)P->cat_maxcode[u]) {
      const int l = (int)v;
      if (v == (double)l) hit |= 1ull << (P->oh_start[u] + l);
    }
  }
  return hit;
}

__device__ __forceinline__ void kde_table_body(const double* __restrict__ x, const KdeParams* __restrict__ P,
                                               KdeParams* __restrict__ Pw, float* __restrict__ table, int j,
                                               int hm, int chunk_f, float* cmax_acc, _Float16* hst) {
  const int n = P->n;
  const int nslots = ((n + OBS_CHUNK - 1) / OBS_CHUNK) * OBS_CHUNK;
  const bool ok = j < n;
  const bool slot = j < nslots;
  const int dc = P->dc, du = P->du, dcp = P->dc_pad, dup = P->du_pad;
  const int KP = kp_of(dcp);
  float* ch = table + (int64_t)(j / OBS_CHUNK) * chunk_f;
  const int jj = j % OBS_CHUNK;
  const int KTP = hm == 2 ? h32_ktp(P->nsc, h32_kp(P->kc), P->has_neg) : h_ktp(dcp, P->kc);
  _Float16* hrow = (_Float16*)(hm == 2 ? ch : ch + OBS_CHUNK) + jj * KTP;
  _Float16* crow = (hm == 2 && P->coarse_off > 0 && slot)
                       ? (_Float16*)(table + P->coarse_off + (int64_t)(j / OBS_CHUNK) * P->coarse_chunk_floats) +
                             jj * h32c_ktp(P->nsc, h32_kp(P->kc))
                       : nullptr;
  double C = 0.0;
  typedef _Float16 h8 __attribute__((ext_vector_type(8)));
  h8 grp = {};
  const int nd32 = h32_nd(P->nsc);
  if (hm == 2) {
    for (int q = 0; q < 2 * nd32; ++q) *(h8*)(hst + 8 * q) = h8{};
    for (int k0 = 0; k0 < dcp; k0 += 8) {
      float v[8];
#pragma unroll
      for (int i = 0; i < 8; ++i) {
        const int k = k0 + i;
        const bool live = ok && k < dc;
        const double xv = x[live ? P->cont_dim[k] : 0];
        v[i] = live ? (float)(P->cont_scale[k] * (xv - P->center[k])) : 0.f;
      }
#pragma unroll
      for (int i = 0; i < 8; ++i) {
        const int k = k0 + i;
        C -= (double)v[i] * (double)v[i];
        if (slot && k < dcp) {
          const float vc = fminf(fmaxf(v[i], -60000.f), 60000.f);
          const _Float16 h = (_Float16)vc;
          const _Float16 l = (_Float16)(vc - (float)h);
          hst[6 + 3 * k] = h;
          hst[7 + 3 * k] = l;
          hst[8 + 3 * k] = h;
        }
      }
      __shared__ __align__(16) uint32_t vab[8][64];
      const int ln = threadIdx.x & 63;
#pragma unroll
      for (int i = 0; i < 8; ++i) vab[i][ln] = __float_as_uint(fabsf(v[i]));
      __syncthreads();
      {
        const int i = ln >> 3, p8 = ln & 7;
        const uint4 q0 = *(const uint4*)&vab[i][8 * p8], q1 = *(const uint4*)&vab[i][8 * p8 + 4];
        uint32_t mx = max(max(max(q0.x, q0.y), max(q0.z, q0.w)), max(max(q1.x, q1.y), max(q1.z, q1.w)));
        mx = max(mx, lane_xor_u32(mx, 1, ln));
        mx = max(mx, lane_xor_u32(mx, 2, ln));
        mx = max(mx, lane_xor_u32(mx, 4, ln));
        if (p8 == 0 && k0 + i < dc) atomicMax((unsigned int*)&Pw->xmax[k0 + i], mx);
      }
      __syncthreads();
    }
  }
#pragma unroll 8
  for (int k = 0; k < (hm == 2 ? 0 : hm ? dcp : KP - 2); ++k) {
    float v = 0.f;
    if (ok && k < dc) v = (float)(P->cont_scale[k] * (x[P->cont_dim[k]] - P->center[k]));
    C -= (double)v * (double)v;
    if (slot) {
      if (hm) {
        const float vc = fminf(fmaxf(v, -60000.f), 60000.f);
        const _Float16 h = (_Float16)vc;
        const _Float16 l = (_Float16)(vc - (float)h);
        const int o = 4 * (k & 1);
        grp[o + 0] = h;
        grp[o + 1] = l;
        grp[o + 2] = h;
        grp[o + 3] = l;
        if (k & 1) *(h8*)(hrow + 4 * (k - 1)) = grp;
      } else {
        ch[(2 + k) * KROW + jj] = v;
      }
    }
    const uint32_t a = wave_reduce_dpp(__float_as_uint(fabsf(v)), OpMax());
    if ((threadIdx.x & 63) == 0 && k < dc) atomicMax((unsigned int*)&Pw->xmax[k], a);
  }
  if (blockIdx.x == 1) PSTAMP(14);
  const h8 z8 = {};
  if (hm == 1 && slot) {
    for (int k = 4 * dcp; k < 32 * P->nsc; k += 8) *(h8*)(hrow + k) = z8;
    for (int k = 32 * (P->nsc + P->kc); k < KTP; k += 8) *(h8*)(hrow + k) = z8;
  }
  if (hm == 2 && slot)
    for (int k = (16 * nd32 + 32 * h32_kp(P->kc) + 2 * h32_ixw(h32_kp(P->kc))) & ~7; k < KTP; k += 8)
      *(h8*)(hrow + k) = z8;
  if (P->kc == 0) {
    if (hm == 0)
      for (int u = 0; u < dup; ++u) {
        const float v = (ok && u < du) ? (float)x[P->cat_dim[u]] : -2.0f;
        if (slot) ch[KP * KROW + jj * dup + u] = v;
      }
  } else if (slot && hm == 2) {
    const int kp = h32_kp(P->kc);
    _Float16* cz = hrow + 16 * nd32;
    _Float16* cp = hrow + h32_par(P->nsc, kp);
    _Float16* cc = crow ? crow + 16 * h32c_nd(P->nsc) : nullptr;
    const int ksp = h32_ksp(kp);
    if (blockIdx.x == 1) PSTAMP(17);
    for (int q = 0; q < 2 * kp; ++q) {
      *(h8*)(cz + 8 * q) = z8;
      *(h8*)(cz + 16 * kp + 8 * q) = z8;
      if (cc) *(h8*)(cc + 8 * q) = z8;
      if (P->has_neg) *(h8*)(cp + 8 * q) = z8;
    }
    if (blockIdx.x == 1) PSTAMP(18);
    uint64_t hit = 0;
    for (int u0 = 0; u0 < (ok ? du : 0); u0 += 8) {
      int cd[8], cm[8], os[8];
      float dlt[8], ngf[8];
      double v[8];
#pragma unroll
      for (int i = 0; i < 8; ++i) {
        cd[i] = P->cat_dim[u0 + i];
        cm[i] = u0 + i < du ? P->cat_maxcode[u0 + i] : -1;
        os[i] = P->oh_start[u0 + i];
        dlt[i] = P->cat_delta[u0 + i];
        ngf[i] = P->cat_negf[u0 + i];
      }
#pragma unroll
      for (int i = 0; i < 8; ++i) v[i] = x[u0 + i < du ? cd[i] : 0];
#pragma unroll
      for (int i = 0; i < 8; ++i) {
        if (!(v[i] >= 0.0 && v[i] <= (double)cm[i]) || v[i] != (double)(int)v[i]) continue;
        const int t = os[i] + (int)v[i], h = t >> 1;
        hit |= 1ull << t;
        const float dl = fminf(fmaxf(dlt[i], -60000.f), 60000.f);
        const float hi = (float)(_Float16)dl;
        cz[h] = (_Float16)hi;
        cz[16 * kp + h] = (_Float16)(fabsf(dl) < 60000.f ? dl - hi : 0.f);
        if (cc) cc[h] = (_Float16)hi;
        if (P->has_neg && ngf[i] != 0.f) cp[h] = (_Float16)0.5f;
      }
    }
    if (blockIdx.x == 1) PSTAMP(19);
    if (blockIdx.x == 1) PSTAMP(20);
    uint32_t iw[8];
#pragma unroll
    for (int q = 0; q < 8; ++q) {
      const int hh = q / ksp, st = q - hh * ksp, sh = 32 * st + 16 * hh;
      const uint32_t win = (st < kp && hh < 2 && sh < 64) ? (uint32_t)(hit >> sh) & 0xFFFFu : 0u;
      iw[q] = (st < kp && hh < 2) ? 0x8888u | ((win & 0xAAAAu) >> 1) : 0u;
    }
    for (int w = 0; w < (crow ? 2 : 1); ++w) {
      uint32_t* ix = w == 0 ? (uint32_t*)(hrow + 16 * nd32 + 32 * kp) : (uint32_t*)(crow + 16 * h32c_nd(P->nsc) + 16 * kp);
      if (kp == 1) {
        const int b = (jj >> 4) & 1;
        for (int q = 0; q < 4; ++q) ix[q] = (q >> 1) == b ? iw[q & 1] : 0u;
      } else {
        for (int q = 0; q < 2 * ksp; ++q) ix[q] = iw[q];
      }
    }
  } else if (slot) {
    const int W = P->kc * 32;
    _Float16* oh;
    _Float16* par;
    if (hm == 1) {
      oh = hrow + 32 * P->nsc;
      par = (_Float16*)(ch + OBS_CHUNK + OBS_CHUNK * KTP / 2) + jj * h_kpp(P->kc);
    } else {
      oh = (_Float16*)(ch + KP * KROW) + jj * W;
      par = (_Float16*)(ch + KP * KROW) + OBS_CHUNK * W + jj * W;
    }
    const uint64_t hit = onehot_hits(x, P, ok);
    h8 og = {}, pg = {};
#pragma unroll 8
// ... 336 lines not shown
```

### hpbandster_amd/csrc/hbx_score_h32.hip

```cpp
#include "hbx_common.h"
#include "hbx_kde_impl.h"

typedef float f32x16 __attribute__((ext_vector_type(16)));
typedef uint32_t u32x2 __attribute__((ext_vector_type(2)));
typedef uint32_t u32x4 __attribute__((ext_vector_type(4)));

#define H32_CMAX 30000.f

template <int KS> struct H32Idx { typedef u32x4 T; };
template <> struct H32Idx<1> { typedef u32x2 T; };
template <> struct H32Idx<2> { typedef u32x2 T; };
template <int KS, typename T> __device__ __forceinline__ int h32_idx(const T& v, int s, int h) {
  if constexpr (KS == 1) return (int)(h ? v[1] : v[0]);
  else return (int)v[s];
}

template <int I, int NM, int NV, int NRL, bool RD = true>
struct SgbH32 {
  static __device__ __forceinline__ void run() {
    __builtin_amdgcn_sched_group_barrier(0x008, 1, 0);
    constexpr int nr = !RD ? 0 : I == NM - 1 ? NRL : 1;
    if constexpr (nr > 0) __builtin_amdgcn_sched_group_barrier(0x100, nr, 0);
    constexpr int n = NV / NM + (I < NV % NM ? 1 : 0);
    if constexpr (n > 0) __builtin_amdgcn_sched_group_barrier(0x002, n, 0);
    SgbH32<I + 1, NM, NV, NRL, RD>::run();
  }
};
template <int NM, int NV, int NRL, bool RD>
struct SgbH32<NM, NM, NV, NRL, RD> {
  static __device__ __forceinline__ void run() {}
};

__device__ __forceinline__ void stage_rows_list(const double* __restrict__ cand, const int32_t* __restrict__ idx,
                                                int64_t nv, int D, int DS, double* xs, int lane) {
  const int tot = (int)nv * D;
  for (int e0 = 0; e0 < tot; e0 += 8 * 64) {
    double t[8];
    int at[8];
#pragma unroll
    for (int q = 0; q < 8; ++q) {
      const int e = min(e0 + 64 * q + lane, tot - 1);
      const int row = e / D, col = e - row * D;
      at[q] = row * DS + col;
      t[q] = cand[(int64_t)idx[row] * D + col];
    }
#pragma unroll
    for (int q = 0; q < 8; ++q) xs[at[q]] = t[q];
  }
}

template <int NSC, int KP, bool SG, bool FAST, bool CO = false, int CT = 1, bool LIST = false>
__device__ __forceinline__ void kde_logpdf_h32_body(const double* __restrict__ cand, int64_t Nc, int32_t D,
                                                    const KdeParams* __restrict__ P,
                                                    const float* __restrict__ table, KdeEst* __restrict__ out,
                                                    const unsigned blk, int32_t* __restrict__ rescue_cnt = nullptr,
                                                    const int split = 0, const int nsplit = 1,
                                                    const int32_t* __restrict__ idx = nullptr,
                                                    const bool scatter = false, const bool row_stage = true) {
  constexpr int ND = CO ? h32c_nd(NSC) : h32_nd(NSC);
  constexpr int KS = KP;
  constexpr int KL = (FAST || CO) ? 0 : KP;
  constexpr int NMT = ND + KS + KL;
  constexpr int KTP = CO ? h32c_ktp(NSC, KP) : h32_ktp(NSC, KP, SG);
  constexpr int CHF = CO ? h32c_chunk_floats(NSC, KP) : h32_chunk_floats(NSC, KP, SG);
  constexpr int PAR = h32_par(NSC, KP);
  static_assert(!SG || KP > 0, "signed sums come from categorical dims");
  static_assert(!FAST || KP > 0, "the fast instance drops the one-hot lo parts");
  static_assert(!CO || !SG, "the coarse instance is built for unsigned sums");
  static_assert(CT == 1 || (CT == 2 && CO), "two candidate column tiles per wave: the coarse instance");
  constexpr int HW = CO ? H32C_WAVES : H16_WAVES;
  constexpr int AUXF = HW * 32 * CT * 4;
  constexpr int NBUF = 2 * (4 * CHF + AUXF) * 4 <= 160 * 1024 ? 4 : 3;
  static_assert(2 * (NBUF * CHF + AUXF) * 4 <= 160 * 1024, "two blocks per CU");
  constexpr int GP = CHF * 4 / 1024;
  constexpr int GL = GP / HW, NX = GP % HW;
  static_assert(GP * 1024 == CHF * 4, "chunk must be a multiple of 1 KB");
  struct ContPrm { double scale, center; float xmax; int32_t col; };
  struct OhPrm { double val; int32_t col, pad; };
  constexpr int PRM_BYTES = 8 * NSC * (int)sizeof(ContPrm) + 32 * (KP > 0 ? KP : 1) * (int)sizeof(OhPrm);
  constexpr int RDS = !CO ? 0 : ((8 * NSC + 16 * KP) | 1) < H32C_ROW_DS ? ((8 * NSC + 16 * KP) | 1) : H32C_ROW_DS;
  constexpr int RSF = RDS >= (H32C_ROW_DMIN | 1) ? (HW * 32 * RDS * 8 + PRM_BYTES) / 4 : 0;
  constexpr int LDSF = NBUF * CHF + AUXF > RSF ? NBUF * CHF + AUXF : RSF;
  static_assert(2 * LDSF * 4 <= 160 * 1024, "two blocks per CU");
  __shared__ __align__(16) float lds[LDSF];
  float* aux = lds + NBUF * CHF;
  if constexpr (CO) table += P->coarse_off;
  int c0 = 0, nchunks = (P->n + OBS_CHUNK - 1) / OBS_CHUNK;
  if (nsplit > 1) {
    obs_split_range(nchunks, split, nsplit, &c0, &nchunks);
    if constexpr (!LIST) out += (int64_t)split * Nc;
    if (nchunks <= 0) {
      const int64_t cb = (int64_t)blk * HW * 32 * CT;
      for (int k = threadIdx.x; k < HW * 32 * CT; k += blockDim.x)
        if (cb + k < Nc) out[cb + k] = kde_est_neutral();
      return;
    }
    table += (int64_t)c0 * CHF;
  }

  const int lane = threadIdx.x & 63, wave = __builtin_amdgcn_readfirstlane(threadIdx.x >> 6);
  const int c = lane & 31, h = lane >> 5;
  const int64_t cbase = ((int64_t)blk * HW + wave) * 32 * CT;
  const bool xpiece = wave < NX;
  const int dc = P->dc;

  static_assert(PRM_BYTES <= NBUF * CHF * 4, "parameters must fit in the ring");
  const int DS = D | 1;
  const int64_t rows_bytes = (int64_t)HW * 32 * CT * DS * 8;
  const bool stage_on = !CO || row_stage;
  const bool rows_fit = stage_on && rows_bytes + PRM_BYTES <= (int64_t)NBUF * CHF * 4;
  const bool tile_fit = RSF > 0 && stage_on && !rows_fit && D >= H32C_ROW_DMIN && DS <= RDS;
  ContPrm* cprm = (ContPrm*)((char*)lds + (rows_fit ? rows_bytes : tile_fit ? (int64_t)HW * 32 * DS * 8 : 0));
  OhPrm* oprm = (OhPrm*)(cprm + 8 * NSC);
  const int tid = threadIdx.x;
  if (tid < 8 * NSC) {
    const bool act = tid < dc;
    cprm[tid] = ContPrm{act ? P->cont_scale[tid] : 0.0, act ? P->center[tid] : 0.0, act ? P->xmax[tid] : 0.f,
                        act ? P->cont_dim[tid] : 0};
  }
  if (tid < 32 * KP) oprm[tid] = OhPrm{P->oh_val[tid], P->oh_col[tid], 0};
  const bool staged = rows_fit && cbase < Nc;
  const int64_t nv = (Nc - cbase) < 32 * CT ? (Nc - cbase) : 32 * CT;
  double* xs = (double*)lds + (int64_t)wave * 32 * (tile_fit ? 1 : CT) * DS;
  if constexpr (LIST) {
    if (staged) stage_rows_list(cand, idx + cbase, nv, D, DS, xs, lane);
  } else {
    if (staged) stage_rows(cand + cbase * (int64_t)D, nv, D, DS, xs, lane);
  }
  const bool tstaged = tile_fit && cbase < Nc;
  auto stage_tile = [&](const int t) -> int {
    const int nt = (int)nv - 32 * t < 32 ? (int)nv - 32 * t : 32;
    if (nt > 0) {
      if constexpr (LIST) stage_rows_list(cand, idx + cbase + 32 * t, nt, D, DS, xs, lane);
      else stage_rows(cand + (cbase + 32 * t) * (int64_t)D, nt, D, DS, xs, lane);
    }
    return nt;
  };
  int nt0 = 0;
  if constexpr (RSF > 0)
    if (tstaged) nt0 = stage_tile(0);
  __syncthreads();

  f16x8 bd[CT][ND];
  f16x16 bsp[CT][KS > 0 ? KS : 1];
  float ci[CT], bnd[CT], cer[CT];
  auto build = [&](const double* x, const int t) {
    ci[t] = bnd[t] = cer[t] = 0.f;
    auto coord = [&](int d) {
      const ContPrm q = cprm[d];
      const float v0 = (float)(q.scale * (x[q.col] - q.center));
      return d < dc ? v0 : 0.f;
    };
#pragma unroll
    for (int s = 0; s < ND; ++s) bd[t][s] = f16x8{};
    if (h == 0) bd[t][0][0] = bd[t][0][1] = bd[t][0][2] = (_Float16)1.f;
    if constexpr (CO) {
#pragma unroll
      for (int j = 0; j < 8 * ND; ++j) {
        const int d = 16 * (j >> 3) + 8 * h + (j & 7) - 6;
        if (d < 0) continue;
        const bool act = d < 8 * NSC;
        const ContPrm q = cprm[act ? d : 0];
        const float v0 = (float)(q.scale * (x[q.col] - q.center));
        const float v = (act && d < dc) ? v0 : 0.f;
        ci[t] = fmaf(-v, v, ci[t]);
        const float xm = act ? q.xmax : 0.f;
        bnd[t] = fmaf(2.f * fabsf(v), xm, bnd[t]);
        const float xc = fminf(fmaxf(2.f * v, -60000.f), 60000.f);
        const _Float16 hi = (_Float16)xc;
        bd[t][j >> 3][j & 7] = hi;
        cer[t] = fmaf(fabsf((float)hi), fmaf(0x1p-11f, xm, 0x1p-25f), cer[t]);
        cer[t] = fmaf(fabsf(xc - (float)hi), xm, cer[t]);
      }
      ci[t] += __shfl_xor(ci[t], 32);
      bnd[t] += __shfl_xor(bnd[t], 32);
      cer[t] += __shfl_xor(cer[t], 32);
    } else {
#pragma unroll
      for (int d = 0; d < 8 * NSC; ++d) {
        const float v = coord(d);
        ci[t] = fmaf(-v, v, ci[t]);
        bnd[t] = fmaf(2.f * fabsf(v), cprm[d].xmax, bnd[t]);
        const float xc = fminf(fmaxf(2.f * v, -60000.f), 60000.f);
        const _Float16 hi = (_Float16)xc;
        const _Float16 lo = (_Float16)(xc - (float)hi);
#pragma unroll
        for (int comp = 0; comp < 3; ++comp) {
          const int k = 6 + 3 * d + comp;
          if (h == ((k >> 3) & 1)) bd[t][k >> 4][k & 7] = comp < 2 ? hi : lo;
        }
      }
    }
#pragma unroll
    for (int s = 0; s < KS; ++s) {
#pragma unroll
      for (int j = 0; j < 8; ++j) {
        const OhPrm o0 = oprm[32 * s + 8 * h + j], o1 = oprm[32 * s + 16 + 8 * h + j];
        bsp[t][s][j] = (x[o0.col] == o0.val) ? (_Float16)1.f : (_Float16)0.f;
        bsp[t][s][8 + j] = (x[o1.col] == o1.val) ? (_Float16)1.f : (_Float16)0.f;
      }
    }
  };
#pragma unroll
  for (int t = 0; t < CT; ++t) {
    int loc = 32 * t + c < nv ? 32 * t + c : (int)nv - 1;
    if (staged || (RSF > 0 && tstaged)) {
      if constexpr (RSF > 0) {
        if (tstaged) {
          const int nt = t == 0 ? nt0 : stage_tile(t);
          loc = c < nt ? c : nt > 0 ? nt - 1 : 0;
        }
      }
      build(xs + loc * DS, t);
    } else {
      int64_t ii = cbase + 32 * t + c;
      if (ii >= Nc) ii = Nc - 1;
      if constexpr (LIST) ii = idx[ii];
      build(cand + ii * (int64_t)D, t);
    }
    asm volatile("" ::: "memory");
  }

  auto issue = [&](int cc, int slot, int part) {
    const float* src = table + (int64_t)(cc < nchunks ? cc : nchunks - 1) * CHF;
    float* dst = lds + slot * CHF;
#pragma unroll
    for (int g = 0; g < GL + (NX ? 1 : 0); ++g) {
      const int piece = (g < GL || xpiece) ? wave + g * HW : wave % GP;
      if (g % 2 == part)
        __builtin_amdgcn_global_load_lds((__attribute__((address_space(1))) const void*)(src + piece * 256 + lane * 4),
                                         (__attribute__((address_space(3))) void*)(dst + piece * 256), 16, 0, 0);
    }
  };
  constexpr int GW = GL + (NX ? 1 : 0);
  constexpr int PD = NBUF - 1;
  __syncthreads();
#pragma unroll
  for (int i = 0; i < PD; ++i) {
    issue(i, i, 0);
    issue(i, i, 1);
  }
  asm volatile("s_waitcnt vmcnt(%0)" ::"n"(GW * (PD - 1)) : "memory");
  __builtin_amdgcn_s_barrier();

  f16x8 ad[ND];
  f16x8 asp[KS > 0 ? KS : 1];
  f16x8 asl[KL > 0 ? KL : 1];
  f16x8 apar[SG ? KS : 1];
  typename H32Idx<KS>::T aix;
  const int ixo = 16 * ND + (CO ? 16 : 32) * KP + (KP == 1 ? 4 * ((c >> 4) & 1) : 2 * h32_ksp(KP) * h) - 8 * h;
  auto arow = [&](const float* buf, int jt) { return (const _Float16*)buf + (32 * jt + c) * KTP + 8 * h; };
  auto readA = [&](const float* buf, int jt) {
    const _Float16* a = arow(buf, jt);
#pragma unroll
    for (int s = 0; s < ND; ++s) ad[s] = *(const f16x8*)(a + 16 * s);
#pragma unroll
    for (int s = 0; s < KS; ++s) asp[s] = *(const f16x8*)(a + 16 * ND + 16 * s);
#pragma unroll
    for (int s = 0; s < KL; ++s) asl[s] = *(const f16x8*)(a + 16 * ND + 16 * KP + 16 * s);
    if constexpr (SG)
#pragma unroll
      for (int s = 0; s < KS; ++s) apar[s] = *(const f16x8*)(a + PAR + 16 * s);
    if constexpr (KS > 0) aix = *(const typename H32Idx<KS>::T*)(a + ixo);
  };
  const f32x16 zero16 = {};
  auto mma = [&](f32x16& acc, const int t) {
    acc = __builtin_amdgcn_mfma_f32_32x32x16_f16(ad[0], bd[t][0], zero16, 0, 0, 0);
#pragma unroll
    for (int s = 1; s < ND; ++s) acc = __builtin_amdgcn_mfma_f32_32x32x16_f16(ad[s], bd[t][s], acc, 0, 0, 0);
#pragma unroll
    for (int s = 0; s < KS; ++s)
      acc = __builtin_amdgcn_smfmac_f32_32x32x32_f16(asp[s], bsp[t][s], acc, h32_idx<KS>(aix, s, h), 0, 0);
#pragma unroll
    for (int s = 0; s < KL; ++s)
      acc = __builtin_amdgcn_smfmac_f32_32x32x32_f16(asl[s], bsp[t][s], acc, h32_idx<KS>(aix, s, h), 0, 0);
  };
  auto mma_rd = [&](f32x16& acc, f32x16& accp, const float* nb, int jt, const int t = CT - 1) {
    const _Float16* a = arow(nb, jt);
    acc = __builtin_amdgcn_mfma_f32_32x32x16_f16(ad[0], bd[t][0], zero16, 0, 0, 0);
    ad[0] = *(const f16x8*)a;
#pragma unroll
    for (int s = 1; s < ND; ++s) {
      acc = __builtin_amdgcn_mfma_f32_32x32x16_f16(ad[s], bd[t][s], acc, 0, 0, 0);
      ad[s] = *(const f16x8*)(a + 16 * s);
    }
#pragma unroll
    for (int s = 0; s < KS; ++s) {
      acc = __builtin_amdgcn_smfmac_f32_32x32x32_f16(asp[s], bsp[t][s], acc, h32_idx<KS>(aix, s, h), 0, 0);
      asp[s] = *(const f16x8*)(a + 16 * ND + 16 * s);
      if (!SG && KL == 0 && s == KS - 1) aix = *(const typename H32Idx<KS>::T*)(a + ixo);
    }
#pragma unroll
    for (int s = 0; s < KL; ++s) {
      acc = __builtin_amdgcn_smfmac_f32_32x32x32_f16(asl[s], bsp[t][s], acc, h32_idx<KS>(aix, s, h), 0, 0);
      asl[s] = *(const f16x8*)(a + 16 * ND + 16 * KP + 16 * s);
      if (!SG && s == KL - 1) aix = *(const typename H32Idx<KS>::T*)(a + ixo);
    }
    if constexpr (SG) {
#pragma unroll
      for (int s = 0; s < KS; ++s) {
        accp = __builtin_amdgcn_smfmac_f32_32x32x32_f16(apar[s], bsp[t][s], s == 0 ? zero16 : accp, h32_idx<KS>(aix, s, h),
                                                        0, 0);
        apar[s] = *(const f16x8*)(a + PAR + 16 * s);
        if (s == KS - 1) aix = *(const typename H32Idx<KS>::T*)(a + ixo);
      }
    }
  };
#pragma unroll
  for (int t = 0; t < CT; ++t) {
    f32x16 a0, a1;
    readA(lds, 0);
    mma(a0, t);
    readA(lds, 1);
    mma(a1, t);
    float mx = fmaxf(a0[0], a1[0]);
#pragma unroll
    for (int r = 1; r < 16; ++r) mx = fmaxf(mx, fmaxf(a0[r], a1[r]));
    mx = fmaxf(mx, __shfl_xor(mx, 32));
    const float d = rintf(-(ci[t] + mx));
    const float dl = (d > 0.f && d < 1e30f) ? d : 0.f;
    const float cs = ci[t] + dl;
    const bool big = fabsf(cs) > H32_CMAX;
    const float cv = big ? 0.f : cs;
    const _Float16 p0 = (_Float16)cv;
    const float r1 = cv - (float)p0;
    const _Float16 p1 = (_Float16)r1;
    const _Float16 p2 = (_Float16)(r1 - (float)p1);
    if (h == 0) {
      bd[t][0][3] = p0;
      bd[t][0][4] = p1;
      bd[t][0][5] = p2;
    }
    if (h == 0) {
      float* ax = aux + ((wave * CT + t) * 32 + c) * 4;
      ax[0] = ci[t];
      ax[1] = bnd[t];
      ax[2] = dl;
      ax[3] = big ? -1.f : cer[t] * (1.f + 0x1p-18f);
    }
  }

  auto tile_sum = [&](const f32x16& a, const f32x16& ap, float& sn) -> float {
    float e[16];
#pragma unroll
    for (int r = 0; r < 16; ++r) e[r] = __builtin_amdgcn_exp2f(a[r]);
    if constexpr (SG) {
      sn = __builtin_amdgcn_fractf(ap[0]) * e[0];
#pragma unroll
      for (int r = 1; r < 16; ++r) sn = fmaf(__builtin_amdgcn_fractf(ap[r]), e[r], sn);
    }
#pragma unroll
    for (int w = 8; w >= 1; w >>= 1)
#pragma unroll
      for (int r = 0; r < w; ++r) e[r] = e[2 * r] + e[2 * r + 1];
    return e[0];
  };
  auto schedule = [&]() {
    SgbH32<0, NMT, 32, (KS > 0 ? 2 : 1)>::run();
    __builtin_amdgcn_sched_barrier(0);
  };
  auto schedule_nr = [&]() {
    SgbH32<0, NMT, 32, (KS > 0 ? 2 : 1), false>::run();
    __builtin_amdgcn_sched_barrier(0);
  };

  float S[CT], Sb[CT], Sn = 0.f, Snb = 0.f;
#pragma unroll
  for (int t = 0; t < CT; ++t) S[t] = Sb[t] = 0.f;
  f32x16 accA, accB, accpA, accpB;
#pragma unroll
  for (int r = 0; r < 16; ++r) {
    accB[r] = -INFINITY;
    accpB[r] = 0.f;
  }
  readA(lds, 0);
  auto chunk1 = [&](int cc, int b) {
    const float* buf = lds + b * CHF;
    const float* nbuf = lds + ((b + 1) % NBUF) * CHF;
    issue(cc + PD, (b + PD) % NBUF, 0);
    mma_rd(accA, accpA, buf, 1);
    float tn;
    Sb[0] += tile_sum(accB, accpB, tn);
    S[0] += Sb[0];
    if constexpr (SG) {
      Snb += tn;
      Sn += Snb;
    }
    schedule();
    issue(cc + PD, (b + PD) % NBUF, 1);
    asm volatile("s_waitcnt vmcnt(%0) lgkmcnt(0)" ::"n"(GW * (PD - 1)) : "memory");
    __builtin_amdgcn_s_barrier();
    mma_rd(accB, accpB, nbuf, 0);
    Sb[0] = tile_sum(accA, accpA, tn);
    if constexpr (SG) Snb = tn;
    schedule();
  };
  auto chunk2s = [&](int cc, int b) {
    const float* buf = lds + b * CHF;
    const float* nbuf = lds + ((b + 1) % NBUF) * CHF;
    float tn;
    issue(cc + PD, (b + PD) % NBUF, 0);
    mma(accA, 0);
    Sb[0] += tile_sum(accB, accpB, tn);
    S[0] += Sb[0];
    schedule_nr();
    mma_rd(accB, accpB, buf, 1, 1);
    Sb[0] = tile_sum(accA, accpA, tn);
    schedule();
    issue(cc + PD, (b + PD) % NBUF, 1);
    mma(accA, 1);
    Sb[CT - 1] = tile_sum(accB, accpB, tn);
    schedule_nr();
    asm volatile("s_waitcnt vmcnt(%0) lgkmcnt(0)" ::"n"(GW * (PD - 1)) : "memory");
    __builtin_amdgcn_s_barrier();
    mma_rd(accB, accpB, nbuf, 0, 0);
    Sb[CT - 1] += tile_sum(accA, accpA, tn);
    S[CT - 1] += Sb[CT - 1];
    schedule();
  };
  auto chunk = [&](int cc, int b) {
    if constexpr (CT == 1) chunk1(cc, b);
    else chunk2s(cc, b);
  };
  int cc = 0;
  for (; cc + NBUF <= nchunks; cc += NBUF) {
    chunk(cc, 0);
    chunk(cc + 1, 1);
    chunk(cc + 2, 2);
    if constexpr (NBUF == 4) chunk(cc + 3, 3);
  }
  for (; cc < nchunks; ++cc) chunk(cc, cc % NBUF);
  {
    float tn;
    constexpr int tl = 0;
    Sb[tl] += tile_sum(accB, accpB, tn);
    S[tl] += Sb[tl];
    if constexpr (SG) Sn += Snb + tn;
  }
  asm volatile("s_waitcnt vmcnt(0)" ::: "memory");
#pragma unroll
  for (int t = 0; t < CT; ++t) S[t] += __shfl_xor(S[t], 32);
  if constexpr (SG) Sn = 2.f * (Sn + __shfl_xor(Sn, 32));
#pragma unroll
  for (int t = 0; t < CT; ++t) {
  if (h == 0) {
    const int64_t ii = cbase + 32 * t + c;
    if (ii < Nc) {
      const float* ax = aux + ((wave * CT + t) * 32 + c) * 4;
      const float ci_q = ax[0], bnd_q = ax[1], dq = ax[2];
      const bool big = ax[3] < 0.f;
      const float cer_q = big ? 0.f : ax[3];
      int64_t irow = ii;
      if constexpr (LIST) irow = idx[ii];
      const int64_t iout = LIST && !scatter ? ii : irow;
      const double* x = cand + irow * (int64_t)D;
      bool nq = P->nan_all != 0;
      for (int k = 0; k < P->nconst; ++k)
        if (x[P->const_dim[k]] != P->const_level[k]) nq = true;
      KdeEst o = finish_est_terms(P, S[t], Sn, -dq, nq, ci_q - dq, bnd_q, SG, (float)(nchunks + (SG ? 18 : 6) + 24));
      if (o.err > 0.f) o.err += (6.f * 0x1p-22f * bnd_q + 0x1p-19f) * HBX_LN2f;
      if constexpr (FAST || CO) {
        float lo_err = CO ? cer_q : 0.f;
        for (int u = 0; u < P->du; ++u) {
          const float dl = fminf(fmaxf(P->cat_delta[u], -60000.f), 60000.f);
          if (fabsf(dl) < 60000.f) lo_err += fabsf(dl - (float)(_Float16)dl);
        }
        if (o.err > 0.f) o.err = (1.f + o.err) * exp2f(lo_err * (1.f + 0x1p-20f)) * (1.f + 0x1p-20f) - 1.f;
      }
      if (!nq && S[t] == S[t] && (big || S[t] < 0x1p-64f || S[t] > 0x1p100f)) {
        o.err = -1.f;
        if (rescue_cnt) atomicAdd(rescue_cnt, 1);
      }
      out[iout] = o;
    }
  }
  }
}

template <int NSC, int KP, bool FAST>
__global__ __launch_bounds__(64 * H16_WAVES) __attribute__((amdgpu_waves_per_eu(4))) void kde_logpdf_h32_kernel(
    const double* __restrict__ cand, int64_t Nc, int32_t D, const KdeParams* __restrict__ P,
    const float* __restrict__ table, KdeEst* __restrict__ out) {
  kde_logpdf_h32_body<NSC, KP, false, FAST>(cand, Nc, D, P, table, out, blockIdx.x);
}

template <int NSC, int KP>
__global__ __launch_bounds__(64 * H32C_WAVES) __attribute__((amdgpu_waves_per_eu(H32C_EU))) void kde_logpdf_h32_co_kernel(
    const double* __restrict__ cand, int64_t Nc, int32_t D, const KdeParams* __restrict__ P,
    const float* __restrict__ table, KdeEst* __restrict__ out, int32_t row_stage) {
  kde_logpdf_h32_body<NSC, KP, false, false, true, H32C_CT>(cand, Nc, D, P, table, out, blockIdx.x, nullptr, 0, 1, nullptr,
                                                             false, row_stage != 0);
}

template <int NSC, int KP, bool FAST, bool CO>
__global__ __launch_bounds__(64 * (CO ? H32C_WAVES : H16_WAVES)) __attribute__((amdgpu_waves_per_eu(CO ? H32C_EU : 4))) void kde_logpdf_h32_pair_kernel(
    const double* __restrict__ cand, int64_t Nc, int32_t D, KdePairArgs a) {
#if HBX_PAIR_INIT
  if (a.init.U && blockIdx.x == 0 && threadIdx.x == 0)
    acq_init_state(a.init.U, a.init.count, a.init.flags, a.init.first1, a.init.res);
#endif
  const bool second = blockIdx.x >= a.nblk0;
  const unsigned loc = second ? blockIdx.x - a.nblk0 : blockIdx.x;
  const int ns = second ? a.nsplit1 : a.nsplit0;
  const unsigned tile = ns > 1 ? loc % a.tiles : loc;
  const int split = ns > 1 ? (int)(loc / a.tiles) : 0;
  kde_logpdf_h32_body<NSC, KP, false, FAST, CO, CO ? H32C_CT : 1>(cand, Nc, D, second ? a.P1 : a.P0, second ? a.table1 : a.table0,
                                                second ? a.out1 : a.out0, tile, a.rescue, split, ns, nullptr, false,
                                                a.row_stage != 0);
}

template <int NSC, int KP>
__global__ __launch_bounds__(64 * H32C_WAVES) __attribute__((amdgpu_waves_per_eu(H32C_EU))) void kde_logpdf_h32_pair1_kernel(
    const double* __restrict__ cand, int64_t Nc, int32_t D, KdePairArgs a) {
#if HBX_PAIR_INIT
  if (a.init.U && blockIdx.x == 0 && threadIdx.x == 0)
    acq_init_state(a.init.U, a.init.count, a.init.flags, a.init.first1, a.init.res);
#endif
  const bool second = blockIdx.x >= a.nblk0;
  const unsigned loc = second ? blockIdx.x - a.nblk0 : blockIdx.x;
  const int ns = second ? a.nsplit1 : a.nsplit0;
  const unsigned tile = ns > 1 ? loc % a.tiles : loc;
  const int split = ns > 1 ? (int)(loc / a.tiles) : 0;
  kde_logpdf_h32_body<NSC, KP, false, false, true, 1>(cand, Nc, D, second ? a.P1 : a.P0, second ? a.table1 : a.table0,
                                                       second ? a.out1 : a.out0, tile, a.rescue, split, ns, nullptr, false,
                                                       a.row_stage != 0);
}

template <int NSC, int KP>
__global__ __launch_bounds__(64 * H32C_WAVES) __attribute__((amdgpu_waves_per_eu(H32C_EU))) void kde_logpdf_h32_list_kernel(
    const double* __restrict__ cand, int32_t D, KdeListArgs a) {
  int32_t cnt = *a.count;
  if (cnt > a.maxcount) cnt = a.maxcount;
  constexpr int CPB = 32 * H32C_CT * H32C_WAVES;
  const bool splits = cnt <= a.cap;
  if (splits && blockIdx.x >= a.tiles_cap * (unsigned)a.nsplit) return;
  const unsigned tile = splits ? blockIdx.x % a.tiles_cap : blockIdx.x;
  const int split = splits ? (int)(blockIdx.x / a.tiles_cap) : 0;
  if ((int64_t)tile * CPB >= cnt) return;
  kde_logpdf_h32_body<NSC, KP, false, false, true, H32C_CT, true>(
      cand, cnt, D, a.P, a.table, splits ? a.part + (int64_t)split * a.cap : a.out, tile, a.rescue, split,
      splits ? a.nsplit : 1, a.idx, !splits, a.row_stage != 0);
}

template <int NSC, int KP, bool FAST>
__global__ __launch_bounds__(64 * H16_WAVES) __attribute__((amdgpu_waves_per_eu(2))) void kde_logpdf_h32s_kernel(
    const double* __restrict__ cand, int64_t Nc, int32_t D, const KdeParams* __restrict__ P,
    const float* __restrict__ table, KdeEst* __restrict__ out) {
  kde_logpdf_h32_body<NSC, KP, true, FAST>(cand, Nc, D, P, table, out, blockIdx.x);
}

template <int NSC, int KP, bool FAST>
__global__ __launch_bounds__(64 * H16_WAVES) __attribute__((amdgpu_waves_per_eu(2))) void kde_logpdf_h32s_pair_kernel(
    const double* __restrict__ cand, int64_t Nc, int32_t D, KdePairArgs a) {
#if HBX_PAIR_INIT
  if (a.init.U && blockIdx.x == 0 && threadIdx.x == 0)
    acq_init_state(a.init.U, a.init.count, a.init.flags, a.init.first1, a.init.res);
#endif
  const bool second = blockIdx.x >= a.nblk0;
  const unsigned loc = second ? blockIdx.x - a.nblk0 : blockIdx.x;
  const int ns = second ? a.nsplit1 : a.nsplit0;
  const unsigned tile = ns > 1 ? loc % a.tiles : loc;
  const int split = ns > 1 ? (int)(loc / a.tiles) : 0;
  kde_logpdf_h32_body<NSC, KP, true, FAST>(cand, Nc, D, second ? a.P1 : a.P0, second ? a.table1 : a.table0,
                                           second ? a.out1 : a.out0, tile, a.rescue, split, ns);
}

template <int NSC, int KP, bool SG, bool PAIR, bool FAST, bool CO>
static constexpr auto h32_inst() {
  if constexpr (PAIR) {
    if constexpr (SG) return (logpdf_pair_fn)kde_logpdf_h32s_pair_kernel<NSC, KP, FAST>;
    else return (logpdf_pair_fn)kde_logpdf_h32_pair_kernel<NSC, KP, FAST, CO>;
  } else {
    static_assert(!CO, "hbx_pick_h32_co");
    if constexpr (SG) return (logpdf_fn)kde_logpdf_h32s_kernel<NSC, KP, FAST>;
    else return (logpdf_fn)kde_logpdf_h32_kernel<NSC, KP, FAST>;
  }
}

template <int NSC, int KP, bool SG, bool PAIR>
static auto pick32_fast(bool fast, bool coarse) {
  if constexpr (!SG && PAIR)
    if (coarse) return h32_inst<NSC, KP, SG, PAIR, false, true>();
  if constexpr (KP > 0)
    if (fast) return h32_inst<NSC, KP, SG, PAIR, true, false>();
  return h32_inst<NSC, KP, SG, PAIR, false, false>();
}

template <int NSC, bool SG, bool PAIR>
static auto pick32_kp(int kp, bool fast, bool coarse) {
  switch (kp) {
    case 0: if constexpr (h32_ok(NSC, 0, SG)) return pick32_fast<NSC, 0, SG, PAIR>(fast, coarse); break;
    case 1: if constexpr (h32_ok(NSC, 1, SG)) return pick32_fast<NSC, 1, SG, PAIR>(fast, coarse); break;
    case 2: if constexpr (h32_ok(NSC, 2, SG)) return pick32_fast<NSC, 2, SG, PAIR>(fast, coarse); break;
  }
  return decltype(h32_inst<NSC, 1, SG, PAIR, false, false>())(nullptr);
}

template <bool SG, bool PAIR>
static auto pick32(int nsc, int kp, bool fast, bool coarse) {
  switch (nsc) {
    case 1: return pick32_kp<1, SG, PAIR>(kp, fast, coarse);
    case 2: return pick32_kp<2, SG, PAIR>(kp, fast, coarse);
    case 3: return pick32_kp<3, SG, PAIR>(kp, fast, coarse);
    case 4: return pick32_kp<4, SG, PAIR>(kp, fast, coarse);
  }
  return decltype(pick32_kp<1, SG, PAIR>(0, false, false))(nullptr);
}

logpdf_fn hbx_pick_h32(int nsc, int kp, bool sg, bool fast) {
  return sg ? pick32<true, false>(nsc, kp, fast, false) : pick32<false, false>(nsc, kp, fast, false);
}

logpdf_pair_fn hbx_pick_h32_pair(int nsc, int kp, bool sg, bool fast, bool coarse) {
  return sg ? pick32<true, true>(nsc, kp, fast, false) : pick32<false, true>(nsc, kp, fast, coarse);
}

template <int NSC>
static logpdf_pair_fn pick32_pair1_kp(int kp) {
  switch (kp) {
    case 0: if constexpr (h32_ok(NSC, 0, false)) return kde_logpdf_h32_pair1_kernel<NSC, 0>; break;
    case 1: if constexpr (h32_ok(NSC, 1, false)) return kde_logpdf_h32_pair1_kernel<NSC, 1>; break;
    case 2: if constexpr (h32_ok(NSC, 2, false)) return kde_logpdf_h32_pair1_kernel<NSC, 2>; break;
  }
  return nullptr;
}

template <int NSC>
static logpdf_list_fn pick32_list_kp(int kp) {
  switch (kp) {
    case 0: if constexpr (h32_ok(NSC, 0, false)) return kde_logpdf_h32_list_kernel<NSC, 0>; break;
    case 1: if constexpr (h32_ok(NSC, 1, false)) return kde_logpdf_h32_list_kernel<NSC, 1>; break;
    case 2: if constexpr (h32_ok(NSC, 2, false)) return kde_logpdf_h32_list_kernel<NSC, 2>; break;
  }
  return nullptr;
}

logpdf_list_fn hbx_pick_h32_list(int nsc, int kp) {
  switch (nsc) {
    case 1: return pick32_list_kp<1>(kp);
    case 2: return pick32_list_kp<2>(kp);
    case 3: return pick32_list_kp<3>(kp);
    case 4: return pick32_list_kp<4>(kp);
  }
  return nullptr;
}

template <int NSC>
static logpdf_co_fn pick32_co_kp(int kp) {
  switch (kp) {
    case 0: if constexpr (h32_ok(NSC, 0, false)) return kde_logpdf_h32_co_kernel<NSC, 0>; break;
    case 1: if constexpr (h32_ok(NSC, 1, false)) return kde_logpdf_h32_co_kernel<NSC, 1>; break;
    case 2: if constexpr (h32_ok(NSC, 2, false)) return kde_logpdf_h32_co_kernel<NSC, 2>; break;
  }
  return nullptr;
}

logpdf_co_fn hbx_pick_h32_co(int nsc, int kp) {
  switch (nsc) {
    case 1: return pick32_co_kp<1>(kp);
    case 2: return pick32_co_kp<2>(kp);
    case 3: return pick32_co_kp<3>(kp);
    case 4: return pick32_co_kp<4>(kp);
  }
  return nullptr;
}

logpdf_pair_fn hbx_pick_h32_pair1(int nsc, int kp) {
  switch (nsc) {
    case 1: return pick32_pair1_kp<1>(kp);
    case 2: return pick32_pair1_kp<2>(kp);
    case 3: return pick32_pair1_kp<3>(kp);
    case 4: return pick32_pair1_kp<4>(kp);
  }
  return nullptr;
}
```

### hpbandster_amd/csrc/hbx_staged.hip

```cpp
#include "hbx_acquire.h"

#include <hip/hip_ext.h>

#include "hbx_acq_impl.h"
#include "hbx_rescue_impl.h"

#define STAGED_PT 4
#define HBX_LN4f 1.3862943611198906f

template <bool KEYS>
__global__ __launch_bounds__(256) void staged_l_kernel(KdeEst* __restrict__ el, int64_t Nc, int32_t ns,
                                                       const double* __restrict__ cand, int32_t D,
                                                       const KdeParams* __restrict__ Pl,
                                                       const int32_t* __restrict__ rescue_cnt,
                                                       float* __restrict__ lhi, uint32_t* __restrict__ stage,
                                                       uint32_t* __restrict__ lkey, uint32_t* __restrict__ hist,
                                                       int32_t hist_words) {
  if constexpr (KEYS) {
    if (blockIdx.x == 0)
      for (int j = threadIdx.x; j < hist_words; j += 256) hist[j] = 0;
  }
  const int32_t nres = *rescue_cnt;
  KdeEst e[STAGED_PT];
  if (ns == 1) {
#pragma unroll
    for (int r = 0; r < STAGED_PT; ++r) {
      const int64_t i = ((int64_t)blockIdx.x * STAGED_PT + r) * 256 + threadIdx.x;
      if (i < Nc) e[r] = el[i];
    }
  }
  float best = -INFINITY;
#pragma unroll
  for (int r = 0; r < STAGED_PT; ++r) {
    const int64_t i = ((int64_t)blockIdx.x * STAGED_PT + r) * 256 + threadIdx.x;
    if (i >= Nc) continue;
    bool mark = false;
    if (ns > 1) {
      if (nres != 0)
        for (int q = 0; q < ns; ++q) mark = mark || el[(int64_t)q * Nc + i].err == -1.f;
      if (!mark) e[r] = merge_splits(el, Nc, i, ns);
    } else {
      mark = e[r].err == -1.f;
    }
    if (mark) e[r] = kde_rescue_one<0, false, true>(cand, i, D, Pl);
    if (ns > 1 || mark) el[i] = e[r];
    float lo = -INFINITY, hi = NAN, pt;
    if (e[r].lpos == e[r].lpos) {
      est_interval(e[r], &lo, &hi, &pt);
      best = fmaxf(best, lo);
    }
    lhi[i] = hi;
    if constexpr (KEYS) lkey[i] = hbx_f2ord(-lo);
  }
  __shared__ float rb[4];
  for (int o = 32; o > 0; o >>= 1) best = fmaxf(best, __shfl_xor(best, o));
  if ((threadIdx.x & 63) == 0) rb[threadIdx.x >> 6] = best;
  __syncthreads();
  if (threadIdx.x == 0) {
    const float b = fmaxf(fmaxf(rb[0], rb[1]), fmaxf(rb[2], rb[3]));
    const uint32_t o = hbx_f2ord(b);
    if (o > __hip_atomic_load(stage + HBX_ST_LMAX, __ATOMIC_RELAXED, __HIP_MEMORY_SCOPE_AGENT))
      atomicMax(stage + HBX_ST_LMAX, o);
  }
}

__device__ __forceinline__ int32_t staged_reserve(int n, int32_t* __restrict__ count) {
  __shared__ int32_t wtot[4];
  __shared__ int32_t base;
  const int lane = threadIdx.x & 63, wv = threadIdx.x >> 6;
  int incl = n;
  for (int o = 1; o < 64; o <<= 1) {
    const int t = __shfl_up(incl, o);
    if (lane >= o) incl += t;
  }
  if (lane == 63) wtot[wv] = incl;
  __syncthreads();
  int woff = 0, total = 0;
  for (int w = 0; w < 4; ++w) {
    if (w < wv) woff += wtot[w];
    total += wtot[w];
  }
  if (threadIdx.x == 0) base = total > 0 ? atomicAdd(count, total) : 0;
  __syncthreads();
  return base + woff + incl - n;
}

__global__ __launch_bounds__(256) void staged_seed_kernel(float* __restrict__ lhi, int64_t Nc,
                                                          KdeEst* __restrict__ eg, int32_t* __restrict__ seeds,
                                                          int32_t cap, uint32_t* __restrict__ stage,
                                                          int32_t mark_rest) {
  const float thr = hbx_ord2f(stage[HBX_ST_LMAX]) - HBX_LN4f;
  bool f[STAGED_PT];
  int n = 0;
#pragma unroll
  for (int r = 0; r < STAGED_PT; ++r) {
    const int64_t i = ((int64_t)blockIdx.x * STAGED_PT + r) * 256 + threadIdx.x;
    f[r] = false;
    if (i < Nc) {
      const float h = lhi[i];
      f[r] = h == h && h >= thr;
    }
    n += f[r] ? 1 : 0;
  }
  int32_t off = staged_reserve(n, (int32_t*)stage + HBX_ST_NSEED);
  const KdeEst none = {0.f, -INFINITY, HBX_EST_NOT_EVAL, 0.f};
#pragma unroll
  for (int r = 0; r < STAGED_PT; ++r) {
    const int64_t i = ((int64_t)blockIdx.x * STAGED_PT + r) * 256 + threadIdx.x;
    if (i >= Nc) continue;
    bool seeded = false;
    if (f[r]) {
      if (off < cap) {
        seeds[off] = (int32_t)i;
        seeded = true;
      }
      ++off;
    }
    if (seeded) lhi[i] = NAN;
    else if (mark_rest) eg[i] = none;
  }
}

__global__ __launch_bounds__(256) void staged_merge_kernel(const KdeEst* __restrict__ part, int32_t cap, int32_t ns,
                                                           const int32_t* __restrict__ idx,
                                                           const int32_t* __restrict__ count, int32_t maxcount,
                                                           const KdeEst* __restrict__ el, KdeEst* __restrict__ eg,
                                                           const KdeParams* __restrict__ Pb,
                                                           uint32_t* __restrict__ stage, int32_t update_u) {
  int32_t cnt = *count;
  if (cnt > maxcount) cnt = maxcount;
  if (cnt > cap) return;
  const int32_t k = blockIdx.x * 256 + threadIdx.x;
  float h = INFINITY;
  if (k < cnt) {
    const int32_t i = idx[k];
    bool mark = false;
    for (int q = 0; q < ns; ++q) mark = mark || part[(int64_t)q * cap + k].err == -1.f;
    KdeEst e = {0.f, -INFINITY, -1.f, 0.f};
    if (!mark) e = merge_splits(part, cap, k, ns);
    eg[i] = e;
    if (update_u && !mark) {
      const ScoreIv v = score_interval(el[i], e);
      if (!v.lnan) h = v.shi;
    }
  }
  if (update_u) {
    const bool guard = Pb->log_norm + log((double)(Pb->n > 1 ? Pb->n : 1)) < 600.0;
    for (int o = 32; o > 0; o >>= 1) h = fminf(h, __shfl_xor(h, o));
    if ((threadIdx.x & 63) == 0 && guard && h < INFINITY) {
      const uint32_t o = hbx_f2ord(h);
      if (o < __hip_atomic_load(stage + HBX_ST_USEED, __ATOMIC_RELAXED, __HIP_MEMORY_SCOPE_AGENT))
        atomicMin(stage + HBX_ST_USEED, o);
    }
  }
}

__global__ __launch_bounds__(256) void staged_survivor_kernel(float* __restrict__ lhi, int64_t Nc,
                                                              int32_t* __restrict__ surv,
                                                              uint32_t* __restrict__ stage,
                                                              int32_t* __restrict__ flags) {
  const float U = hbx_ord2f(stage[HBX_ST_USEED]);
  const float C = (float)HBX_LN_CLAMP;
  bool f[STAGED_PT];
  int n = 0;
#pragma unroll
  for (int r = 0; r < STAGED_PT; ++r) {
    const int64_t i = ((int64_t)blockIdx.x * STAGED_PT + r) * 256 + threadIdx.x;
    f[r] = false;
    if (i < Nc) {
      const float h = lhi[i];
      f[r] = h == h && (C - fmaxf(h, C)) <= U;
      if (flags && h == h) {
        lhi[i] = C - fmaxf(h, C);
        if (h > 700.f) atomicOr(flags, 1);
      }
    }
    n += f[r] ? 1 : 0;
  }
  int32_t off = staged_reserve(n, (int32_t*)stage + HBX_ST_NSURV);
#pragma unroll
  for (int r = 0; r < STAGED_PT; ++r) {
    const int64_t i = ((int64_t)blockIdx.x * STAGED_PT + r) * 256 + threadIdx.x;
    if (i < Nc && f[r]) surv[off++] = (int32_t)i;
  }
  if (blockIdx.x == 0 && threadIdx.x == 0) stage[HBX_ST_FLAG] = 1;
}

struct StagedTailArgs {
  const KdeEst* part;
  int32_t cap, ns;
  const int32_t* seeds;
  const int32_t* surv;
  int64_t Nc;
  const double* cand;
  int32_t D;
  const KdeParams* Pb;
  const KdeEst* el;
  KdeEst* eg;
  float* lo;
  uint32_t* U;
  int32_t* flags;
  int32_t* first1;
  int32_t* list;
  int32_t* count;
  int32_t* rescue_cnt;
  uint32_t* stage;
};

__device__ __forceinline__ uint32_t ld_agent(const uint32_t* p) {
  return __hip_atomic_load(p, __ATOMIC_RELAXED, __HIP_MEMORY_SCOPE_AGENT);
}
__device__ __forceinline__ int32_t ld_agent(const int32_t* p) {
  return __hip_atomic_load(p, __ATOMIC_RELAXED, __HIP_MEMORY_SCOPE_AGENT);
}

#define TAIL_THREADS 1024
#define TAIL_PT 4
__global__ __launch_bounds__(256) void staged_tail_kernel(StagedTailArgs t) {
  constexpr int TAIL_THREADS_A = 256;
  constexpr int NW = TAIL_THREADS_A / 64;
  __shared__ int32_t swc[NW];
  __shared__ uint32_t pbase;
  const int lane = threadIdx.x & 63, wv = threadIdx.x >> 6;
  int64_t nseed = (int32_t)t.stage[HBX_ST_NSEED], nsurv = (int32_t)t.stage[HBX_ST_NSURV];
  if (nseed > t.cap) nseed = t.cap;
  if (nsurv > t.Nc) nsurv = t.Nc;
  const bool split = nsurv <= t.cap;
  const int64_t total = nseed + nsurv;
  constexpr int64_t EPB = (int64_t)TAIL_PT * TAIL_THREADS_A;
  const int64_t nwork = (total + EPB - 1) / EPB;
  if (blockIdx.x >= nwork) return;
  const int32_t nres = *t.rescue_cnt;
  int32_t idx[TAIL_PT];
  KdeEst ea[TAIL_PT], eb[TAIL_PT];
  float slo[TAIL_PT];
#pragma unroll
  for (int r = 0; r < TAIL_PT; ++r) {
    const int64_t k = (int64_t)blockIdx.x * EPB + r * TAIL_THREADS_A + threadIdx.x;
    idx[r] = -1;
    if (k < total) idx[r] = k < nseed ? t.seeds[k] : t.surv[k - nseed];
  }
#pragma unroll
  for (int r = 0; r < TAIL_PT; ++r) {
    const int64_t k = (int64_t)blockIdx.x * EPB + r * TAIL_THREADS_A + threadIdx.x;
    if (idx[r] < 0) continue;
    ea[r] = t.el[idx[r]];
    if (k < nseed || !split) eb[r] = t.eg[idx[r]];
  }
  float h = INFINITY;
  int32_t f1 = INT32_MAX;
  bool of = false;
#pragma unroll
  for (int r = 0; r < TAIL_PT; ++r) {
    const int64_t k = (int64_t)blockIdx.x * EPB + r * TAIL_THREADS_A + threadIdx.x;
    slo[r] = NAN;
    if (idx[r] < 0) continue;
    const int64_t i = idx[r];
    bool store = false;
    if (!(k < nseed || !split)) {
      const int64_t ks = k - nseed;
      bool mark = false;
      for (int q = 0; q < t.ns; ++q) mark = mark || t.part[(int64_t)q * t.cap + ks].err == -1.f;
      eb[r] = {0.f, -INFINITY, -1.f, 0.f};
      if (!mark) eb[r] = merge_splits(t.part, t.cap, ks, t.ns);
      store = true;
    }
    if (nres != 0 && eb[r].err == -1.f) {
      eb[r] = kde_rescue_one<0, false, true>(t.cand, i, t.D, t.Pb);
      store = true;
    }
    if (store) t.eg[i] = eb[r];
    const ScoreIv v = score_interval(ea[r], eb[r]);
    slo[r] = v.one ? NAN : v.slo;
    t.lo[i] = slo[r];
    if (!v.lnan) h = fminf(h, v.shi);
    if (v.one && (int32_t)i < f1) f1 = (int32_t)i;
    of = of || v.of;
  }
  float hw = h;
  int32_t fw = f1;
  for (int o = 32; o > 0; o >>= 1) {
    hw = fminf(hw, __shfl_xor(hw, o));
    fw = min(fw, __shfl_xor(fw, o));
  }
  const bool ofw = __ballot(of) != 0;
  bool lowered = false;
  if (lane == 0) {
    const uint32_t o = hbx_f2ord(hw);
    if (hw < INFINITY && o < ld_agent(t.U)) atomicMin(t.U, o);
    if (fw != INT32_MAX && fw < ld_agent(t.first1)) lowered = atomicMin(t.first1, fw) > fw;
    if (ofw) atomicOr(t.flags, 1);
  }
  lowered = __shfl(lowered ? 1 : 0, 0) != 0;
  __syncthreads();
  const float useed = hbx_ord2f(t.stage[HBX_ST_USEED]);
  const float u = fminf(useed, hbx_ord2f(ld_agent(t.U)));
  int n = 0;
#pragma unroll
  for (int r = 0; r < TAIL_PT; ++r) {
    const float l = slo[r];
    if (!(idx[r] >= 0 && ((l == l && l <= u) || (lowered && idx[r] == fw)))) idx[r] = -1;
    n += idx[r] >= 0 ? 1 : 0;
  }
  {
    int incl = n;
    for (int o = 1; o < 64; o <<= 1) {
      const int v = __shfl_up(incl, o);
      if (lane >= o) incl += v;
    }
    if (lane == 63) swc[wv] = incl;
    __syncthreads();
    int off = incl - n, tot = 0;
#pragma unroll
    for (int w = 0; w < NW; ++w) {
      off += w < wv ? swc[w] : 0;
      tot += swc[w];
    }
    if (threadIdx.x == 0) pbase = tot > 0 ? atomicAdd(t.stage + HBX_ST_NPRE, (uint32_t)tot) : 0u;
    __syncthreads();
    off += (int)pbase;
#pragma unroll
    for (int r = 0; r < TAIL_PT; ++r)
      if (idx[r] >= 0) t.list[off++] = idx[r];
  }
}

__global__ __launch_bounds__(TAIL_THREADS) void staged_shortlist_kernel(StagedTailArgs t) {
  constexpr int NW = TAIL_THREADS / 64;
  constexpr int64_t EPB = (int64_t)TAIL_PT * TAIL_THREADS;
  __shared__ int32_t swc[NW];
  const int lane = threadIdx.x & 63, wv = threadIdx.x >> 6;
  const int64_t npre = t.stage[HBX_ST_NPRE];
  const float uf = hbx_ord2f(t.U[0]);
  const int32_t ff = t.first1[0];
  const bool all = (t.flags[0] & 1) != 0;
  const int64_t nscan = all ? t.Nc : npre;
  int64_t base = 0;
  for (int64_t c0 = 0; c0 < nscan; c0 += EPB) {
    const int64_t c = c0 + (int64_t)TAIL_PT * threadIdx.x;
    int32_t ci[TAIL_PT];
    float cl[TAIL_PT];
#pragma unroll
    for (int r = 0; r < TAIL_PT; ++r) ci[r] = c + r < nscan ? (all ? (int32_t)(c + r) : t.list[c + r]) : -1;
#pragma unroll
    for (int r = 0; r < TAIL_PT; ++r) cl[r] = ci[r] >= 0 ? t.lo[ci[r]] : NAN;
    int n = 0;
#pragma unroll
    for (int r = 0; r < TAIL_PT; ++r) {
      if (!(ci[r] >= 0 && ((cl[r] == cl[r] && (all || cl[r] <= uf)) || ci[r] == ff))) ci[r] = -1;
      n += ci[r] >= 0 ? 1 : 0;
    }
    int incl = n;
    for (int o = 1; o < 64; o <<= 1) {
      const int v = __shfl_up(incl, o);
      if (lane >= o) incl += v;
    }
    if (lane == 63) swc[wv] = incl;
    __syncthreads();
    int64_t off = base + incl - n;
    int tot = 0;
#pragma unroll
    for (int w = 0; w < NW; ++w) {
      off += w < wv ? swc[w] : 0;
      tot += swc[w];
    }
#pragma unroll
    for (int r = 0; r < TAIL_PT; ++r)
      if (ci[r] >= 0) t.list[off++] = ci[r];
    base += tot;
    __syncthreads();
  }
  if (threadIdx.x == 0) {
    *t.count = (int32_t)base;
    *t.rescue_cnt = 0;
  }
}


bool acq_staged_supported(const AcqPlan& plan) {
  return HBX_PAIR_INIT && !plan.exact_only && plan.fg.list && plan.fb.list && plan.fg.pair && plan.fg.split_ok;
}

static dim3 staged_gsel(int64_t Nc) { return dim3((unsigned)((Nc + 256 * STAGED_PT - 1) / (256 * STAGED_PT))); }

static KdeListArgs staged_list_args(const AcqPlan& plan, const KdePairRef& p, const AcqWs& a) {
  const int32_t cap = a.list_cap;
  return KdeListArgs{p.Pb(), p.table_bad, a.eg, a.lpart, a.seeds, (const int32_t*)a.stage + HBX_ST_NSEED, a.rescue,
                     cap,    cap,         list_splits(p.nmax), (unsigned)(cap / plan.fb.cands_per_block),
                     hbx_row_stage()};
}

int staged_score_l(const AcqPlan& plan, const KdePairRef& p, const double* cand, int64_t Nc, const AcqWs& a,
                   hipEvent_t* ev, hipStream_t s, uint32_t* lkey, uint32_t* hist, int32_t hist_words) {
  const ScoreFns& f = plan.fg;
  const PairShape sh = pair_shape(f, true, 1, Nc, p.nmax);
  const int ns = sh.nsplit;
  const unsigned grid = sh.tiles * (unsigned)ns;
  KdePairArgs ka{p.Pg(), p.Pg(), p.table_good, p.table_good, a.el, a.el, grid, a.rescue, a.init()};
  ka.tiles = sh.tiles;
  ka.nsplit0 = ka.nsplit1 = ns;
  ka.row_stage = hbx_row_stage();
  if (ev)
    hipExtLaunchKernelGGL(sh.kernel, dim3(grid), dim3(f.threads), 0, s, ev[0], nullptr, 0, cand, Nc, p.D, ka);
  else
    hipLaunchKernelGGL(sh.kernel, dim3(grid), dim3(f.threads), 0, s, cand, Nc, p.D, ka);
  HBX_LAUNCH_CHECK();
  if (lkey)
    hipLaunchKernelGGL(staged_l_kernel<true>, staged_gsel(Nc), dim3(256), 0, s, a.el, Nc, (int32_t)ns, cand, p.D,
                       p.Pg(), a.rescue, a.lo, a.stage, lkey, hist, hist_words);
  else
    hipLaunchKernelGGL(staged_l_kernel<false>, staged_gsel(Nc), dim3(256), 0, s, a.el, Nc, (int32_t)ns, cand, p.D,
                       p.Pg(), a.rescue, a.lo, a.stage, (uint32_t*)nullptr, (uint32_t*)nullptr, 0);
  HBX_LAUNCH_CHECK();
  return HBX_OK;
}

int staged_score_seeds(const AcqPlan& plan, const KdePairRef& p, const double* cand, int64_t Nc, const AcqWs& a,
                       hipStream_t s, bool mark_rest, bool update_u) {
  const int32_t cap = a.list_cap;
  hipLaunchKernelGGL(staged_seed_kernel, staged_gsel(Nc), dim3(256), 0, s, a.lo, Nc, a.eg, a.seeds, cap, a.stage,
                     (int32_t)(mark_rest ? 1 : 0));
  HBX_LAUNCH_CHECK();
  const ScoreFns& fb = plan.fb;
  const KdeListArgs la = staged_list_args(plan, p, a);
  hipLaunchKernelGGL(fb.list, dim3(la.tiles_cap * (unsigned)la.nsplit), dim3(fb.threads), 0, s, cand, p.D, la);
  HBX_LAUNCH_CHECK();
  hipLaunchKernelGGL(staged_merge_kernel, dim3((unsigned)((cap + 255) / 256)), dim3(256), 0, s, a.lpart, cap,
                     la.nsplit, a.seeds, la.count, cap, a.el, a.eg, p.Pb(), a.stage, (int32_t)(update_u ? 1 : 0));
  HBX_LAUNCH_CHECK();
  return HBX_OK;
}

int staged_score_survivors(const AcqPlan& plan, const KdePairRef& p, const double* cand, int64_t Nc, const AcqWs& a,
                           hipStream_t s, bool lonly) {
  const ScoreFns& fb = plan.fb;
  hipLaunchKernelGGL(staged_survivor_kernel, staged_gsel(Nc), dim3(256), 0, s, a.lo, Nc, a.surv, a.stage,
                     lonly ? a.flags : (int32_t*)nullptr);
  HBX_LAUNCH_CHECK();
  KdeListArgs la = staged_list_args(plan, p, a);
  la.idx = a.surv;
  la.count = (const int32_t*)a.stage + HBX_ST_NSURV;
  la.maxcount = (int32_t)Nc;
  const unsigned gfull = (unsigned)((Nc + fb.cands_per_block - 1) / fb.cands_per_block);
  const unsigned gsplit = la.tiles_cap * (unsigned)la.nsplit;
  hipLaunchKernelGGL(fb.list, dim3(gfull > gsplit ? gfull : gsplit), dim3(fb.threads), 0, s, cand, p.D, la);
  HBX_LAUNCH_CHECK();
  return HBX_OK;
}

int acq_score_staged(const AcqPlan& plan, const KdePairRef& p, const double* cand, int64_t Nc, const AcqWs& a,
                     hipEvent_t* ev, hipStream_t s, bool tail) {
  int rc = staged_score_l(plan, p, cand, Nc, a, ev, s, nullptr, nullptr, 0);
  if (rc) return rc;
  rc = staged_score_seeds(plan, p, cand, Nc, a, s, !tail, true);
  if (rc) return rc;
  rc = staged_score_survivors(plan, p, cand, Nc, a, s, tail);
  if (rc) return rc;
  const int32_t cap = a.list_cap;
  const int32_t ls = list_splits(p.nmax);
  if (tail) {
    const StagedTailArgs ta{a.lpart, cap,     ls,   a.seeds, a.surv,  Nc,       cand,   p.D,     p.Pb(),
                            a.el,    a.eg,    a.lo, a.U,     a.flags, a.first1, a.list, a.count, a.rescue,
                            a.stage};
    hipLaunchKernelGGL(staged_tail_kernel, dim3((unsigned)((Nc + cap + 1023) / 1024)), dim3(256), 0, s, ta);
    HBX_LAUNCH_CHECK();
    hipLaunchKernelGGL(staged_shortlist_kernel, dim3(1), dim3(TAIL_THREADS), 0, s, ta);
  } else {
    hipLaunchKernelGGL(staged_merge_kernel, dim3((unsigned)((cap + 255) / 256)), dim3(256), 0, s, a.lpart, cap, ls,
                       a.surv, (const int32_t*)a.stage + HBX_ST_NSURV, (int32_t)Nc, a.el, a.eg, p.Pb(), a.stage, 0);
  }
  HBX_LAUNCH_CHECK();
  if (ev) {
    HBX_HIP(hipEventRecord(ev[1], s));
    HBX_HIP(hipEventRecord(ev[2], s));
  }
  return HBX_OK;
}

extern "C" {

int hbx_kde_acquire_stats(const void* workspace, int64_t Nc, int64_t nmax, int64_t* out) {
  if (!workspace || !out || Nc < 0) return hbx_fail(HBX_ERR_ARG, "hbx_kde_acquire_stats: bad arguments");
  const WsLayout w = ws_layout(Nc, nmax);
  uint32_t st[HBX_ST_WORDS];
  HBX_HIP(hipDeviceSynchronize());
  HBX_HIP(hipMemcpy(st, (const char*)workspace + w.stage, sizeof(st), hipMemcpyDeviceToHost));
  const bool staged = st[HBX_ST_FLAG] == 1;
  const int64_t seeds = staged ? ((int64_t)st[HBX_ST_NSEED] < w.list_cap ? (int64_t)st[HBX_ST_NSEED] : w.list_cap) : 0;
  const int64_t surv = staged ? (int64_t)st[HBX_ST_NSURV] : 0;
  out[0] = staged ? 1 : 0;
  out[1] = seeds;
  out[2] = surv;
  out[3] = staged ? seeds + surv : Nc;
  return HBX_OK;
}

}
```

### hpbandster_amd/kde.py

```python

import ctypes
import math
import struct
import threading

import numpy as np

from . import _native as N

RESULT_FMT = "<qdfiiidd"
RESULT_BYTES = struct.calcsize(RESULT_FMT)
ACQ_OVERFLOW, ACQ_NEAR_TIE, ACQ_RESOLVED, ACQ_DOMAIN_ERR = 1, 2, 4, 8


def _torch():
    import torch
    return torch


def default_device():
    torch = _torch()
    if not torch.cuda.is_available():
        raise N.HbxError("hpbandster_amd needs a ROCm GPU (torch.cuda.is_available() is False); "
                         "the engine has no CPU path")
# ... 86 lines not shown


class TopK(object):
    __slots__ = ("index", "score", "pdf_l", "pdf_g", "rel", "count", "shortlist", "flags")

    def __init__(self, index, score, pdf_l, pdf_g, rel, shortlist=0, flags=0):
        self.index = np.asarray(index, dtype=np.int64)
        self.score = np.asarray(score, dtype=np.float64)
        self.pdf_l = np.asarray(pdf_l, dtype=np.float64)
        self.pdf_g = np.asarray(pdf_g, dtype=np.float64)
        self.rel = np.asarray(rel, dtype=np.float32)
        self.count = int(self.index.size)
        if not (self.score.size == self.pdf_l.size == self.pdf_g.size == self.rel.size == self.count):
            raise ValueError("TopK: arrays of different lengths")
        self.shortlist, self.flags = int(shortlist), int(flags)

    @classmethod
    def from_bytes(cls, b):
        count, shortlist, flags, _ = struct.unpack("<iiii", bytes(b[:TOPK_HEAD_BYTES]))
        r = np.frombuffer(bytes(b), dtype=TOPK_REC, count=count, offset=TOPK_HEAD_BYTES)
        return cls(r["index"].copy(), r["score"].copy(), r["pdf_l"].copy(), r["pdf_g"].copy(), r["rel"].copy(),
                   shortlist, flags)

    def __len__(self):
        return self.count

    def __repr__(self):
        return "TopK(count=%d, shortlist=%d, flags=%d, index=%r)" % (self.count, self.shortlist, self.flags,
                                                                     self.index[:8].tolist())


def _rows_of(cands, idx):
    idx = np.asarray(idx, dtype=np.int64)
    if isinstance(cands, np.ndarray):
        return np.asarray(cands, dtype=np.float64)[idx]
    torch = _torch()
    return cands[torch.from_numpy(idx).to(cands.device)].cpu().numpy()


class DeviceKDE(object):

    def __init__(self, X_dev, rows_dev, var_type, bw, nlev, data_host, stream=None, prepared=None, home=None):
        self.var_type = var_type
        self.k_vars = len(var_type)
        self.bw = np.asarray(bw, dtype=np.float64)
        self.nlev = np.asarray(nlev, dtype=np.int32)
        self._data = data_host
        self.nobs = int(rows_dev.shape[0])
        self.X_dev = X_dev
        self.rows_dev = rows_dev
        self.device = X_dev.device
        D = self.k_vars
        if prepared is None:
            torch = _torch()
            L = N.lib()
            vt = var_type_codes(var_type)
            dcp, dup = scoring_bucket(vt)
            with N.on_device(self.device, stream):
                self.params = torch.empty(int(L.hbx_kde_param_bytes()), dtype=torch.uint8, device=self.device)
                tf = int(L.hbx_kde_table_floats(self.nobs, dcp, dup))
                self.table = torch.empty(tf, dtype=torch.float32, device=self.device)
                info = np.zeros(8, dtype=np.int32)
                bw_c = np.ascontiguousarray(self.bw)
                nlev_c = np.ascontiguousarray(self.nlev)
                home = N.stream_handle(stream, self.device)
                N.check(L.hbx_kde_prepare(N.ptr(X_dev), D, N.ptr(rows_dev), self.nobs, N.ptr(vt), N.ptr(bw_c),
                                          N.ptr(nlev_c), N.ptr(self.params), N.ptr(self.table), self.table.numel(),
                                          N.ptr(info), home))
        else:
            self.params, self.table, info = prepared
        self._home = home
        self._ordered = set()
        self._lv_src = self._lv_key = self._lv_dev = self._bw_ptr = self._tab = None
        self.variant, self.nan_all, unsupported, self.dc, self.du, self.nconst, self.dc_pad, self.du_pad = \
            info.tolist()
        self.has_neg, self.kc = self.variant & 1, (self.variant >> 1) & 7
        self.exact_only = bool((self.variant >> 5) & 1)
        if unsupported:
            raise N.HbxError("KDE bandwidth/level combination not modelled (bw=%r, nlev=%r)" % (self.bw, self.nlev))

    @property
    def data(self):
        if isinstance(self._data, tuple):
            src, idx = self._data
            self._data = src[idx]
        return self._data

    def _order(self, sh):
        h = self._home
        if h is None or sh == h or sh in self._ordered:
            return
        N.check(N.lib().hbx_stream_order(sh, h))
        self._ordered.add(sh)

    def pdf(self, data_predict=None, stream=None):
        torch = _torch()
        L = N.lib()
        if data_predict is None:
            pts = np.asarray(self.data, dtype=np.float64)
        else:
            pts = np.asarray(data_predict, dtype=np.float64)
            if pts.ndim <= 1:
                pts = pts.reshape(-1, self.k_vars) if pts.size != self.k_vars else pts.reshape(1, -1)
        pts = np.ascontiguousarray(pts.reshape(-1, self.k_vars))
        with N.on_device(self.device, stream):
            p_dev = torch.from_numpy(pts).to(self.device)
            out = torch.empty(pts.shape[0], dtype=torch.float64, device=self.device)
            sb = int(L.hbx_kde_pdf_scratch_bytes(self.nobs))
            scratch = torch.empty(sb, dtype=torch.uint8, device=self.device)
            sh = N.stream_handle(stream, self.device)
            self._order(sh)
            N.check(L.hbx_kde_pdf_exact(N.ptr(p_dev), pts.shape[0], self.k_vars, N.ptr(self.params),
                                        N.ptr(self.X_dev), N.ptr(self.rows_dev), self.nobs, N.ptr(out), N.ptr(scratch),
                                        sb, sh))
            return np.squeeze(out.cpu().numpy())

    def sample(self, levels, bw_factor, Nc, seed, counter_base, stream_id=0, stream=None, table=None, out=None):
        sh = N.home_stream(self.device.index) if stream is None else None
        if sh is not None:
            return self._sample(levels, bw_factor, Nc, seed, counter_base, stream_id, sh, table, out)
        with N.on_device(self.device, stream):
            return self._sample(levels, bw_factor, Nc, seed, counter_base, stream_id,
                                N.stream_handle(stream, self.device), table, out)

    def _sample(self, levels, bw_factor, Nc, seed, counter_base, stream_id, sh, table, out):
        torch = _torch()
        L = N.lib()
        D = self.k_vars
        self._order(sh)
        if levels is not self._lv_src:
            lv = np.ascontiguousarray(np.asarray(levels, dtype=np.int32))
            if lv.shape != (D,):
                raise N.HbxError("levels must have %d entries" % D)
            key = lv.tobytes()
            if self._lv_key != key:
                self._lv_dev, self._lv_key = _levels_on_device(key, lv, self.device), key
                self._tab = None
            self._lv_src = levels
        bw_ptr = self._bw_ptr
        if bw_ptr is None:
            bw_ptr = self._bw_ptr = N.ptr(self.params) + int(L.hbx_kde_param_bw_offset())
        Nc = int(Nc)
        if table is None:
            table = Nc >= 4 * self.nobs
        tab = None
        if table:
            if self._tab is None:
                self._tab = torch.empty(int(L.hbx_kde_sample_table_bytes(self.nobs, D)) // 8, dtype=torch.float64,
                                        device=self.device)
                N.check(L.hbx_kde_sample_table(N.ptr(self.X_dev), D, N.ptr(self.rows_dev), self.nobs,
                                               bw_ptr, N.ptr(self._lv_dev), N.ptr(self._tab), sh))
            tab = self._tab
        if out is not None:
            cands, datum, err = out
            if tuple(cands.shape) != (Nc, D) or datum.numel() < Nc or err.numel() < Nc:
                raise N.HbxError("sample: output tensors of the wrong size")
        else:
            cands = torch.empty((Nc, D), dtype=torch.float64, device=self.device)
            datum = torch.empty(Nc, dtype=torch.int64, device=self.device)
            err = torch.empty(Nc, dtype=torch.uint8, device=self.device)
        N.check(L.hbx_kde_sample(N.ptr(self.X_dev), D, N.ptr(self.rows_dev), self.nobs, bw_ptr,
                                 N.ptr(self._lv_dev), N.ptr(tab), float(bw_factor), int(seed) & (2 ** 64 - 1),
                                 int(counter_base) & (2 ** 64 - 1), int(stream_id) & 0xFFFFFFFF, Nc, N.ptr(cands),
                                 N.ptr(datum), N.ptr(err), sh))
        return cands, datum, err

    def logpdf(self, cands, rtol=1e-5, stream=None):
        torch = _torch()
        L = N.lib()
        C = np.ascontiguousarray(np.asarray(cands, dtype=np.float64).reshape(-1, self.k_vars))
        Nc = C.shape[0]
        if Nc == 0:
            return np.zeros(0)
        with N.on_device(self.device, stream):
            c_dev = torch.from_numpy(C).to(self.device)
            out = torch.empty(Nc, dtype=torch.float64, device=self.device)
            sb = int(L.hbx_kde_logpdf_rtol_scratch_bytes(Nc))
            scr = torch.empty(sb, dtype=torch.uint8, device=self.device)
            sh = N.stream_handle(stream, self.device)
            self._order(sh)
            N.check(L.hbx_kde_logpdf_rtol(N.ptr(c_dev), Nc, self.k_vars, N.ptr(self.params), N.ptr(self.table),
                                          N.ptr(self.X_dev), N.ptr(self.rows_dev), self.dc_pad, self.du_pad,
                                          self.variant, float(rtol), N.ptr(out), N.ptr(scr), sb, sh))
            return out.cpu().numpy()

    def _logpdf_exact(self, C, stream):
        torch = _torch()
        L = N.lib()
        if not (self.has_neg or self.nan_all or self.nconst):
            with N.on_device(self.device, stream):
                p_dev = torch.from_numpy(np.ascontiguousarray(C)).to(self.device)
                o = torch.empty(C.shape[0], dtype=torch.float64, device=self.device)
                sh = N.stream_handle(stream, self.device)
                self._order(sh)
                N.check(L.hbx_kde_logpdf_exact(N.ptr(p_dev), C.shape[0], self.k_vars, N.ptr(self.params),
                                               N.ptr(self.X_dev), N.ptr(self.rows_dev), N.ptr(o), sh))
                return o.cpu().numpy()
        exact = np.atleast_1d(self.pdf(C, stream=stream))
        with np.errstate(divide="ignore", invalid="ignore"):
            return np.log(exact)

    def logpdf_est(self, cand_dev, stream=None):
        torch = _torch()
        L = N.lib()
        Nc = int(cand_dev.shape[0])
        with N.on_device(self.device, stream):
            est = torch.empty((Nc, 4), dtype=torch.float32, device=self.device)
            sh = N.stream_handle(stream, self.device)
            self._order(sh)
            N.check(L.hbx_kde_logpdf(N.ptr(cand_dev), Nc, self.k_vars, N.ptr(self.params), N.ptr(self.table),
                                     self.dc_pad, self.du_pad, self.variant, N.ptr(est), sh))
            e = est.cpu().numpy()
        return e[:, 0], e[:, 1], e[:, 2]


_LEVELS = {}


def _levels_on_device(key, lv, device):
    t = _LEVELS.get((str(device), key))
    if t is None:
        t = _LEVELS[(str(device), key)] = _torch().from_numpy(lv.copy()).to(device)
    return t


class KDEPair(object):

    def __init__(self, good, bad):
        self.good = good
        self.bad = bad
        if (good.dc_pad, good.du_pad) != (bad.dc_pad, bad.du_pad):
            raise N.HbxError("good/bad KDEs prepared for different kernel buckets")
        self.nmax = max(good.nobs, bad.nobs)
        self._wsb = {}
        self._roff = None
        self._home = good._home if good._home == bad._home else None
        dev = good.device
        self._dev_index = dev.index if dev.index is not None else _torch().cuda.current_device()
        L = N.lib()
        self._ws_cache = {}
        self._bound = None
        self._bound_fn = L.hbx_kde_acquire_bound
        self._free_fn = L.hbx_kde_pair_free
        self._bound = L.hbx_kde_pair_bind(
            good.k_vars, good.params.data_ptr(), good.table.data_ptr(), good.X_dev.data_ptr(),
            good.rows_dev.data_ptr(), good.variant, bad.params.data_ptr(), bad.table.data_ptr(),
            bad.X_dev.data_ptr(), bad.rows_dev.data_ptr(), bad.variant, good.dc_pad, good.du_pad, self.nmax)
        if not self._bound:
            raise N.HbxError("hbx_kde_pair_bind: %s" % L.hbx_last_error().decode())

    def __del__(self):
        b, self._bound = getattr(self, "_bound", None), None
        if b:
            self._free_fn(b)

    def __getitem__(self, key):
        if key == "good":
            return self.good
        if key == "bad":
            return self.bad
        raise KeyError(key)

    def keys(self):
        return ["good", "bad"]

    def _order(self, sh):
        if sh != self._home:
            self.good._order(sh)
            self.bad._order(sh)

    def result_offset(self):
        if self._roff is None:
            self._roff = int(N.lib().hbx_kde_result_ptr(4096)) - 4096
        return self._roff

    def workspace_bytes(self, Nc):
        wsb = self._wsb.get(Nc)
        if wsb is None:
            wsb = self._wsb[Nc] = int(N.lib().hbx_kde_workspace_bytes(int(Nc), self.nmax))
        return wsb

    def _thread_workspace(self, Nc):
        key = (threading.get_ident(), Nc)
        ws = self._ws_cache.get(key)
        if ws is None:
            ws = self._ws_cache[key] = _torch().empty(self.workspace_bytes(Nc), dtype=_torch().uint8,
                                                      device=self.good.device)
        return ws

    def _acquire_bound(self, cand_ptr, Nc, index_base, ws, sh, err=None, events=None, row=None):
        if sh != self._home:
            self._order(sh)
        rec = _record_buffer()
        N.check(self._bound_fn(self._bound, cand_ptr, Nc, int(index_base), ws.data_ptr(), ws.numel(),
                               err.data_ptr() if err is not None else None,
                               events.address if events is not None else None, sh, rec,
                               row.ctypes.data if row is not None else None))
        return AcqResult.from_bytes(rec.raw[:RESULT_BYTES])

    def acquire_stats(self, workspace, Nc):
        out = (ctypes.c_int64 * 4)()
        N.check(N.lib().hbx_kde_acquire_stats(workspace.data_ptr(), int(Nc), self.nmax, ctypes.addressof(out)))
        return {"staged": bool(out[0]), "seeds": int(out[1]), "survivors": int(out[2]), "evaluated": int(out[3])}

    def acquire(self, cands, index_base=0, logs=False, stream=None, workspace=None, sync=True, events=None,
                ties="pinned"):
        if ties not in ("pinned", "process"):
            raise ValueError("ties must be 'pinned' or 'process'")
        sh = N.home_stream(self._dev_index) if sync and not logs and stream is None else None
        if sh is not None:
            r = self._acquire_sync(cands, index_base, workspace, events, sh)
            if r is not None:
                if ties == "process" and r.flags & ACQ_NEAR_TIE:
                    with N.on_device(self.good.device):
                        ws = workspace if workspace is not None else self._thread_workspace(len(cands))
                        self._resolve(r, ws, len(cands), len(cands), cands, int(index_base))
                return r
        with N.on_device(self.good.device, stream):
            return self._acquire(cands, index_base, logs, stream, workspace, sync, events, ties)

    def _acquire_sync(self, cands, index_base, workspace, events, sh):
        torch = _torch()
        if type(cands) is not torch.Tensor or cands.dtype is not torch.float64 or not cands.is_cuda:
            return None
        D = self.good.k_vars
        if cands.dim() != 2 or cands.shape[1] != D or not cands.is_contiguous() or \
                cands.device.index != self._dev_index:
            return None
        Nc = cands.shape[0]
        if workspace is None:
            workspace = self._thread_workspace(Nc)
        elif workspace.numel() < self.workspace_bytes(Nc):
            raise N.HbxError("workspace too small")
        return self._acquire_bound(cands.data_ptr(), Nc, index_base, workspace, sh, None, events)

    def _stage_cands(self, cands):
        torch = _torch()
        if isinstance(cands, np.ndarray):
            c_dev = torch.from_numpy(np.ascontiguousarray(cands, dtype=np.float64)).to(self.good.device)
        else:
            c_dev = cands
            if c_dev.dtype != torch.float64 or not c_dev.is_contiguous():
                raise N.HbxError("candidate tensor must be contiguous float64 [Nc, D]")
        Nc = int(c_dev.shape[0])
        D = self.good.k_vars
        if Nc > 0 and (c_dev.dim() != 2 or int(c_dev.shape[1]) != D):
            raise N.HbxError("candidates must be [Nc, %d], got %s" % (D, tuple(c_dev.shape)))
        return c_dev, Nc

    def _workspace(self, workspace, wsb):
        torch = _torch()
        ws = workspace if workspace is not None else torch.empty(wsb, dtype=torch.uint8, device=self.good.device)
        if ws.numel() < wsb:
            raise N.HbxError("workspace too small")
        return ws

    def _resolve_if_near(self, ties, res, ws, Nc, cands, c_dev, index_base):
        if ties == "process" and res.flags & ACQ_NEAR_TIE:
            self._resolve(res, ws, Nc, Nc, cands if isinstance(cands, np.ndarray) else c_dev, int(index_base))

    def _acquire(self, cands, index_base, logs, stream, workspace, sync, events, ties):
        torch = _torch()
        L = N.lib()
        dev = self.good.device
        c_dev, Nc = self._stage_cands(cands)
        ws = self._workspace(workspace, self.workspace_bytes(Nc))
        logl = torch.empty(Nc, dtype=torch.float32, device=dev) if logs else None
        logg = torch.empty(Nc, dtype=torch.float32, device=dev) if logs else None
        sh = N.stream_handle(stream, dev)
        if sync and not logs:
            res = self._acquire_bound(c_dev.data_ptr(), Nc, index_base, ws, sh, None, events)
            self._resolve_if_near(ties, res, ws, Nc, cands, c_dev, index_base)
            return res
        self._order(sh)
        N.check(L.hbx_kde_acquire(c_dev.data_ptr(), Nc, int(index_base), self._bound, N.ptr(logl), N.ptr(logg),
                                  ws.data_ptr(), ws.numel(), events.address if events is not None else None, sh))
        off = self.result_offset()
        rview = ws[off:off + RESULT_BYTES]
        if not sync:
            return rview
        res = AcqResult.from_bytes(fetch_bytes(rview, stream))
        self._resolve_if_near(ties, res, ws, Nc, cands, c_dev, index_base)
        if logs:
            return res, logl.cpu().numpy(), logg.cpu().numpy()
        return res

    def topk_workspace_bytes(self, Nc, k):
        return int(N.lib().hbx_kde_topk_workspace_bytes(int(Nc), int(k), self.nmax))

    def acquire_topk(self, cands, k, index_base=0, stream=None, workspace=None, ties="pinned"):
        if ties != "pinned":
            raise ValueError("acquire_topk offers ties='pinned' only")
        k = int(k)
        if k < 1 or k > TOPK_MAX_K:
            raise ValueError("k must be in [1, %d], got %d" % (TOPK_MAX_K, k))
        with N.on_device(self.good.device, stream):
            return self._acquire_topk(cands, k, index_base, stream, workspace)

    def _acquire_topk(self, cands, k, index_base, stream, workspace):
        torch = _torch()
        L = N.lib()
        dev = self.good.device
        c_dev, Nc = self._stage_cands(cands)
        ws = self._workspace(workspace, self.topk_workspace_bytes(Nc, k))
        out = torch.empty(int(L.hbx_kde_topk_result_bytes(k)), dtype=torch.uint8, device=dev)
        sh = N.stream_handle(stream, dev)
        self._order(sh)
        N.check(L.hbx_kde_acquire_topk(c_dev.data_ptr(), Nc, k, int(index_base), self._bound, N.ptr(out),
                                       ws.data_ptr(), ws.numel(), sh))
        return TopK.from_bytes(fetch_bytes(out, stream))

    def _ws_offsets(self, Nc, seg):
        o = np.zeros(5, dtype=np.int64)
        N.check(N.lib().hbx_kde_ws_offsets(int(Nc), int(max(seg, 1)), self.nmax, N.ptr(o)))
        return [int(v) for v in o]

    def _ws_ints(self, ws, off, count):
        return ws[off:off + 4 * count].view(_torch().int32).cpu().numpy().astype(np.int64)

    def _repick(self, res, cands, idx, shift):
        from . import exact_host
        pick = exact_host.resolve(self.good, self.bad, _rows_of(cands, idx), idx)
        if pick is not None:
            res.index, res.score, res.pdf_l, res.pdf_g = pick[0] + shift, pick[1], pick[2], pick[3]
        res.flags |= ACQ_RESOLVED

    def _resolve(self, res, ws, Nc, seg, cands, index_base):
        o = self._ws_offsets(Nc, seg)
        self._repick(res, cands, self._ws_ints(ws, o[2], res.near), index_base)

    def _resolve_batch(self, recs, ws, Nc, seg, cands):
        o = self._ws_offsets(Nc, seg)
        cnt = int(self._ws_ints(ws, o[0], 1)[0])
        lst, flg = self._ws_ints(ws, o[1], cnt), self._ws_ints(ws, o[2], cnt)
        for b, r in enumerate(recs):
            if r.flags & ACQ_NEAR_TIE:
                self._repick(r, cands, np.sort(lst[(flg != 0) & (lst // seg == b)]), -b * seg)

    def acquire_mapped(self, cands):
        sh = N.home_stream(self._dev_index)
        if sh is None:
            return self.acquire(np.array(cands))
        Nc = cands.shape[0]
        return self._acquire_bound(cands.ctypes.data, Nc, 0, self._thread_workspace(Nc), sh)

    def acquire_pick(self, cands, err, workspace, row, sh=None):
        if sh is None:
            sh = N.home_stream(self._dev_index)
            if sh is None:
                with N.on_device(self.good.device):
                    return self.acquire_pick(cands, err, workspace, row, N.stream_handle(None, self.good.device))
        return self._acquire_bound(cands.data_ptr(), int(cands.shape[0]), 0, workspace, sh, err, None, row)

    def batch_workspace_bytes(self, Nc, seg):
        return int(N.lib().hbx_kde_batch_workspace_bytes(int(Nc), int(seg), self.nmax))

    def acquire_batch(self, cands, seg, stream=None, workspace=None, results=None, sync=True, ties="pinned"):
        if ties not in ("pinned", "process"):
            raise ValueError("ties must be 'pinned' or 'process'")
        with N.on_device(self.good.device, stream):
            return self._acquire_batch(cands, seg, stream, workspace, results, sync, ties)

    def _acquire_batch(self, cands, seg, stream, workspace, results, sync, ties):
        torch = _torch()
        L = N.lib()
        dev = self.good.device
        seg = int(seg)
        if seg < 1:
            raise N.HbxError("segment length must be >= 1")
        c_dev, Nc = self._stage_cands(cands)
        B = (Nc + seg - 1) // seg
        ws = self._workspace(workspace, self.batch_workspace_bytes(Nc, seg))
        out = results if results is not None else torch.empty(max(B, 1) * RESULT_BYTES, dtype=torch.uint8, device=dev)
        if out.numel() < B * RESULT_BYTES:
            raise N.HbxError("result buffer too small")
        sh = N.stream_handle(stream, dev)
        self._order(sh)
        N.check(L.hbx_kde_acquire_batch(N.ptr(c_dev), Nc, seg, 0, self._bound, None, None, N.ptr(out), N.ptr(ws),
                                        ws.numel(), sh))
        if not sync:
            return out[:B * RESULT_BYTES]
        raw = fetch_bytes(out[:B * RESULT_BYTES], stream)
        recs = [AcqResult.from_bytes(raw[i * RESULT_BYTES:(i + 1) * RESULT_BYTES]) for i in range(B)]
        if ties == "process" and any(r.flags & ACQ_NEAR_TIE for r in recs):
            self._resolve_batch(recs, ws, Nc, seg, cands if isinstance(cands, np.ndarray) else c_dev)
        return recs


class ScoreEvents(object):

    def __init__(self):
        L = N.lib()
        self._ev = (ctypes.c_void_p * 3)()
        for i in range(3):
            h = ctypes.c_void_p()
            N.check(L.hbx_event_create(ctypes.addressof(h)))
            self._ev[i] = h.value
        self.address = ctypes.addressof(self._ev)

    def elapsed_ms(self, fused=False):
        L = N.lib()
        a, b = ctypes.c_float(), ctypes.c_float()
        N.check(L.hbx_event_elapsed_ms(self._ev[0], self._ev[1], ctypes.addressof(a)))
        if fused:
            return a.value, 0.0
        N.check(L.hbx_event_elapsed_ms(self._ev[1], self._ev[2], ctypes.addressof(b)))
        return a.value, b.value

    def __del__(self):
        try:
            L = N.lib()
            for i in range(3):
                L.hbx_event_destroy(self._ev[i])
        except Exception:
            pass


def split_sizes(n, D, min_points, top_n_percent=15, split_rule="bohb"):
    if split_rule == "bohb":
        n_good, n_bad = bohb_split_sizes(n, min_points, top_n_percent)
        if min(n_good, n) <= D or min(n_bad, n) <= D:
            return None
    else:
        n_good = int(max(top_n_percent * n / 100., min_points))
        n_bad = int(max((100 - top_n_percent) * n / 100., min_points))
        if min(n_good, n) < D or min(n_bad, n) < D:
            return None
        if min(n_good, n) <= D or min(n_bad, n) <= D:
            raise ValueError("The number of observations must be larger than the number of variables.")
    return min(n_good, n), min(n_bad, n)


class _DevSlice(object):
    __slots__ = ("base", "_ptr", "_numel")

    def __init__(self, base, ptr, numel):
        self.base, self._ptr, self._numel = base, ptr, numel

    def data_ptr(self):
        return self._ptr

    def numel(self):
        return self._numel


class ObservationStore(object):

    def __init__(self, D, var_type, device=None, capacity=256):
        self.D = int(D)
        self.var_type = var_type
        self.vt = np.ascontiguousarray(var_type_codes(var_type))
        self.device = device or default_device()
        self.n = 0
        self.nh = 0
        self._hcap = 0
        self._Xh = self._lh = None
        self._cap = 0
        self.X_dev = self.loss_dev = None
        self._init_cap = int(capacity)
        self.dc_pad, self.du_pad = scoring_bucket(self.vt)

    def _reserve(self, n):
        torch = _torch()
        if n <= self._cap:
            return
        cap = max(self._init_cap, self._cap)
        while cap < n:
            cap *= 2
        X = torch.empty((cap, self.D), dtype=torch.float64, device=self.device)
        L = torch.empty(cap, dtype=torch.float64, device=self.device)
        if self.n:
            X[:self.n].copy_(self.X_dev[:self.n])
            L[:self.n].copy_(self.loss_dev[:self.n])
        self.X_dev, self.loss_dev, self._cap = X, L, cap

    def add(self, rows, losses):
        rows = np.asarray(rows, dtype=np.float64).reshape(-1, self.D)
        losses = np.asarray(losses, dtype=np.float64).reshape(-1)
        if losses.shape[0] != rows.shape[0]:
            raise N.HbxError("observation store: %d rows, %d losses" % (rows.shape[0], losses.shape[0]))
        cat = self.vt != 0
        if cat.any():
            codes = rows[:, cat]
            if not (np.all((codes >= 0) & (codes < 1024)) and np.all(codes == np.floor(codes))):
                raise N.HbxError("categorical codes must be integers in [0, 1024)")
        m = self.nh + rows.shape[0]
        if m > self._hcap:
            cap = max(self._init_cap, self._hcap)
            while cap < m:
                cap *= 2
            Xh = np.empty((cap, self.D))
            lh = np.empty(cap)
            if self.nh:
                Xh[:self.nh] = self._Xh[:self.nh]
                lh[:self.nh] = self._lh[:self.nh]
            self._Xh, self._lh, self._hcap = Xh, lh, cap
        self._Xh[self.nh:m] = rows
        self._lh[self.nh:m] = losses
        self.nh = m

    @property
    def X_host(self):
        return self._Xh[:self.nh]

    @property
    def losses_host(self):
# ... 84 lines not shown
```

### include/hbx.h

```cpp
#ifndef HBX_H_
#define HBX_H_

#include <stdint.h>

#ifdef __cplusplus
extern "C" {
#endif

#define HBX_OK 0
#define HBX_ERR_ARG (-1)
#define HBX_ERR_HIP (-2)
#define HBX_ERR_UNSUPPORTED (-3)

const char* hbx_last_error(void);
const char* hbx_version(void);
int64_t hbx_kde_param_bytes(void);
int64_t hbx_kde_param_bw_offset(void);
int64_t hbx_kde_est_bytes(void);
int64_t hbx_acq_result_bytes(void);
int32_t hbx_max_dims(void);

int64_t hbx_sort_scratch_bytes(int64_t N);

int hbx_seg_argsort(const double* loss, const int64_t* seg_off, int64_t B, int64_t max_seg, int64_t N,
                    int64_t* order, void* scratch, int64_t scratch_bytes, void* stream);

#define HBX_ORDER_NUMPY 0
#define HBX_ORDER_STABLE 1

int hbx_seg_argsort_ex(const double* loss, const int64_t* seg_off, int64_t B, int64_t max_seg, int64_t N,
                       int64_t* order, void* scratch, int64_t scratch_bytes, int32_t order_mode, void* stream);

int hbx_kde_fit(const double* X, int32_t D, const int64_t* seg_off, int64_t B, const int64_t* order,
                const int64_t* n_good, const int64_t* n_bad, const double* fac_good, const double* fac_bad,
                const int32_t* vartype, double* bw_good, double* bw_bad, int32_t* nlev_good, int32_t* nlev_bad,
                void* stream);

int64_t hbx_kde_refit_out_bytes(int64_t n, int32_t D);
int64_t hbx_kde_refit_scratch_bytes(int64_t n, int32_t D);
int hbx_kde_refit(double* X, double* loss, int64_t n, int32_t D, const int32_t* vartype, const double* staged,
                  int64_t n_new, int64_t n_good, int64_t n_bad, double fac_good, double fac_bad, void* params_good,
                  float* table_good, int64_t table_good_floats, void* params_bad, float* table_bad,
                  int64_t table_bad_floats, void* out, void* scratch, int64_t scratch_bytes, void* stream);
int hbx_kde_refit_sync(double* X, double* loss, int64_t n, int32_t D, const int32_t* vartype,
                       const double* staged_host, int64_t n_new, int64_t n_good, int64_t n_bad, double fac_good,
                       double fac_bad, void* params_good, float* table_good, int64_t table_good_floats,
                       void* params_bad, float* table_bad, int64_t table_bad_floats, void* out, void* scratch,
                       int64_t scratch_bytes, void* stream, void* out_host);
int hbx_stream_order(void* waiter, void* signaller);

int hbx_kde_bucket(int32_t dc, int32_t du, int32_t* dc_pad, int32_t* du_pad, int32_t* stride);
int64_t hbx_kde_table_floats(int32_t n, int32_t dc_pad, int32_t du_pad);

int hbx_kde_prepare(const double* X, int32_t D, const int64_t* rows, int32_t n, const int32_t* vartype,
                    const double* bw, const int32_t* nlev, void* params, float* table, int64_t table_floats,
                    int32_t* info, void* stream);

int hbx_kde_logpdf(const double* cand, int64_t Nc, int32_t D, const void* params, const float* table,
                   int32_t dc_pad, int32_t du_pad, int32_t variant, void* est_out, void* stream);

int64_t hbx_kde_workspace_bytes(int64_t Nc, int64_t nmax);

int hbx_kde_acquire(const double* cand, int64_t Nc, int64_t index_base, const void* pair, float* logl_out,
                    float* logg_out, void* workspace, int64_t ws_bytes, void* events, void* stream);

void* hbx_kde_pair_bind(int32_t D, const void* params_good, const float* table_good, const double* X_good,
                        const int64_t* rows_good, int32_t variant_good, const void* params_bad,
                        const float* table_bad, const double* X_bad, const int64_t* rows_bad, int32_t variant_bad,
                        int32_t dc_pad, int32_t du_pad, int64_t nmax);
int hbx_kde_acquire_bound(const void* pair, const double* cand, int64_t Nc, int64_t index_base, void* workspace,
                          int64_t ws_bytes, const uint8_t* err, void* events, void* stream, void* rec_out,
                          double* row_out);
void hbx_kde_pair_free(void* pair);

int64_t hbx_kde_batch_workspace_bytes(int64_t Nc, int64_t seg, int64_t nmax);
int hbx_kde_acquire_batch(const double* cand, int64_t Nc, int64_t seg, int64_t index_base, const void* pair,
                          float* logl_out, float* logg_out, void* results, void* workspace, int64_t ws_bytes,
                          void* stream);

#define HBX_TOPK_MAX_K 1024
int64_t hbx_kde_topk_workspace_bytes(int64_t Nc, int32_t k, int64_t nmax);
int64_t hbx_kde_topk_result_bytes(int32_t k);
int hbx_kde_acquire_topk(const double* cand, int64_t Nc, int32_t k, int64_t index_base, const void* pair,
                         void* results, void* workspace, int64_t ws_bytes, void* stream);

#define HBX_ACQ_NO_MODEL    16
#define HBX_ACQ_UNSUPPORTED 32
int64_t hbx_kde_groups_workspace_bytes(int64_t B, int64_t C, int32_t D);
int hbx_kde_acquire_groups(const double* X, int32_t D, const int64_t* seg_off, int64_t B, const int64_t* order,
                           const int64_t* n_good, const int64_t* n_bad, const int32_t* vartype,
                           const double* bw_good, const double* bw_bad,
                           const int32_t* nlev_good, const int32_t* nlev_bad,
                           const double* cand, int64_t C, void* results,
                           void* workspace, int64_t ws_bytes, void* stream);
int64_t hbx_kde_groups_batch_workspace_bytes(int64_t B, int64_t S, int64_t C, int32_t D);
int hbx_kde_acquire_groups_batch(const double* X, int32_t D, const int64_t* seg_off, int64_t B, const int64_t* order,
                                 const int64_t* n_good, const int64_t* n_bad, const int32_t* vartype,
                                 const double* bw_good, const double* bw_bad,
                                 const int32_t* nlev_good, const int32_t* nlev_bad,
                                 const double* cand, int64_t S, int64_t C, void* results,
                                 void* workspace, int64_t ws_bytes, void* stream);
int64_t hbx_kde_groups_topk_workspace_bytes(int64_t B, int64_t C, int32_t k, int32_t D);
int hbx_kde_acquire_groups_topk(const double* X, int32_t D, const int64_t* seg_off, int64_t B, const int64_t* order,
                                const int64_t* n_good, const int64_t* n_bad, const int32_t* vartype,
                                const double* bw_good, const double* bw_bad,
                                const int32_t* nlev_good, const int32_t* nlev_bad,
                                const double* cand, int64_t C, int32_t k, void* results,
                                void* workspace, int64_t ws_bytes, void* stream);
#define HBX_GRP_EXACT_L 64
#define HBX_GRP_EXACT_G 128
#define HBX_LOGPDF_FP64_ONLY 1
int64_t hbx_kde_logpdf_groups_workspace_bytes(int64_t B, int64_t C, int32_t D);
int hbx_kde_logpdf_groups(const double* X, int32_t D, const int64_t* seg_off, int64_t B, const int64_t* order,
                          const int64_t* n_good, const int64_t* n_bad, const int32_t* vartype,
                          const double* bw_good, const double* bw_bad,
                          const int32_t* nlev_good, const int32_t* nlev_bad,
                          const double* cand, int64_t C, double rtol, int32_t flags,
                          double* ln_l, double* ln_g, int32_t* status,
                          void* workspace, int64_t ws_bytes, void* stream);
int hbx_kde_logpdf_groups_stats(const void* workspace, int64_t* out4);
int hbx_kde_sample_groups(const double* X, int32_t D, const int64_t* seg_off, int64_t B, const int64_t* order,
                          const int64_t* n_good, const double* bw_good, const int32_t* levels,
                          double bw_factor, uint64_t seed, uint64_t counter_base, uint32_t stream_id,
                          int64_t C, double* cands, uint8_t* domain_err, void* stream);
#define HBX_CFG_MODEL 0
#define HBX_CFG_RANDOM_FRACTION 1
#define HBX_CFG_NO_MODEL 2
#define HBX_CFG_NO_SCORE 3
#define HBX_CFG_DOMAIN_ERR 4
int hbx_kde_finish_groups(const void* records, const double* cands, const uint8_t* domain_err, const int32_t* levels,
                          int32_t D, int64_t B, int64_t S, int64_t C, double random_fraction, uint64_t seed,
                          uint64_t counter_base, uint32_t stream_id, double* rows_out, uint8_t* source_out, void* stream);
int64_t hbx_kde_propose_groups_workspace_bytes(int64_t B, int64_t S, int64_t C, int32_t D);
int hbx_kde_propose_groups_ws_offsets(int64_t B, int64_t S, int64_t C, int32_t D, int64_t* out4);
int hbx_kde_propose_groups(const double* X, int32_t D, const int64_t* seg_off, int64_t B, const int64_t* order,
                           const int64_t* n_good, const int64_t* n_bad, const int32_t* vartype,
                           const double* bw_good, const double* bw_bad,
                           const int32_t* nlev_good, const int32_t* nlev_bad, const int32_t* levels,
                           double bandwidth_factor, double random_fraction, uint64_t seed, uint64_t counter_base,
                           uint32_t stream_id, int64_t S, int64_t C, double* rows_out, uint8_t* source_out,
                           void* records_out, double* cands_out, void* workspace, int64_t workspace_bytes, void* stream);

int hbx_event_create(void** ev);
int hbx_event_destroy(void* ev);
int hbx_event_elapsed_ms(void* start, void* stop, float* ms);

int hbx_fetch(void* host_dst, const void* dev_src, int64_t bytes, void* stream);

int64_t hbx_mapped_host_buffers(void);

#define HBX_ACQ_OVERFLOW 1
#define HBX_ACQ_NEAR_TIE 2
#define HBX_ACQ_RESOLVED 4
#define HBX_ACQ_DOMAIN_ERR 8
void* hbx_kde_result_ptr(void* workspace);
int hbx_kde_ws_offsets(int64_t Nc, int64_t seg, int64_t nmax, int64_t* out);
int hbx_kde_acquire_stats(const void* workspace, int64_t Nc, int64_t nmax, int64_t* out);

int64_t hbx_kde_pdf_scratch_bytes(int64_t nmax);

int hbx_kde_pdf_exact(const double* pts, int64_t Np, int32_t D, const void* params, const double* X,
                      const int64_t* rows, int64_t n, double* out, void* scratch, int64_t scratch_bytes,
                      void* stream);
int hbx_kde_logpdf_exact(const double* pts, int64_t Np, int32_t D, const void* params, const double* X,
                         const int64_t* rows, double* out, void* stream);

int64_t hbx_kde_logpdf_rtol_scratch_bytes(int64_t Nc);
int hbx_kde_logpdf_rtol(const double* cand, int64_t Nc, int32_t D, const void* params, const float* table,
                        const double* X, const int64_t* rows, int32_t dc_pad, int32_t du_pad, int32_t variant,
                        double rtol, double* out, void* scratch, int64_t scratch_bytes, void* stream);

int hbx_np_exp(const double* x, int64_t n, double* y, void* stream);

int hbx_philox4x32_10(const uint32_t* counter, const uint32_t* key, uint32_t* out);

int hbx_kde_sample(const double* X, int32_t D, const int64_t* rows, int64_t n, const double* bw,
                   const int32_t* levels, const double* tab, double bw_factor, uint64_t seed, uint64_t counter_base,
                   uint32_t stream_id, int64_t Nc, double* cands, int64_t* datum, uint8_t* domain_err, void* stream);
int hbx_norm_ppf(const double* p, int64_t n, double* z, void* stream);
int64_t hbx_kde_sample_table_bytes(int64_t n, int32_t D);
int hbx_kde_sample_table(const double* X, int32_t D, const int64_t* rows, int64_t n, const double* bw,
                         const int32_t* levels, double* tab, void* stream);

int hbx_kde_cv_terms(const double* X, int64_t n, int32_t D, const int32_t* vartype, const double* bw,
                     const double* lev, const int32_t* lev_off, const int32_t* loo_levels, double c4, double c2,
                     double bwprod, double* F, double* L, void* stream);

int64_t hbx_rccl_unique_id_bytes(void);
int hbx_rccl_get_unique_id(void* id_out);
int hbx_rccl_comm_init(void** comm, int32_t nranks, const void* id, int32_t rank, int32_t device);
int hbx_rccl_comm_count(void* comm, int32_t* count);
int hbx_rccl_comm_destroy(void* comm);
int64_t hbx_argmax_gather_bytes(int32_t nranks);
int hbx_argmax_allreduce(const void* local, void* gather, void* out, int32_t nranks, void* rccl_comm, void* stream);
int hbx_argmax_records(const void* all, int32_t nranks, void* out, void* stream);

int hbx_sh_promote(const double* loss, const int64_t* seg_off, int64_t B, int64_t max_seg, int64_t N,
                   const double* k, int64_t* order, uint8_t* advance, int64_t* n_advance, void* scratch,
                   int64_t scratch_bytes, void* stream);

int64_t hbx_sh_promote_scratch_bytes(int64_t B, int64_t max_seg, int64_t N, int32_t order_requested,
                                     int32_t order_mode);
int hbx_sh_promote_ex(const double* loss, const int64_t* seg_off, int64_t B, int64_t max_seg, int64_t N,
                      const double* k, int64_t* order, uint8_t* advance, int64_t* n_advance, void* scratch,
                      int64_t scratch_bytes, int32_t order_mode, void* events, void* stream);

int hbx_sh_promote_one(const double* loss, int64_t n, double k, uint8_t* advance, void* scratch, int32_t order_mode,
                       int32_t* done, int32_t seq, void* stream);
int hbx_sh_advance_mapped(const double* losses, int64_t n, double k, uint8_t* mask, double* pin, uint8_t* pout,
                          int32_t* done, int32_t seq, void* scratch, int32_t order_mode, void* stream);
int hbx_sh_advance_state(int64_t* state, int64_t n, double k, void* stream);
int hbx_host_alloc(int64_t bytes, void** out);
int hbx_host_free(void* p);

int hbx_np_argsort_host(const double* x, int64_t n, int64_t* order);
int hbx_sh_advance_host(const double* loss, int64_t n, int64_t k, uint8_t* advance, int64_t* scratch);

int64_t hbx_mt_state_bytes(void);
int hbx_mt_draw(void* state, int32_t kind, int64_t n, int64_t high, double* out);
int hbx_bohb_draw(void* state, const double* data, int64_t n, int32_t D, const double* bw, const int64_t* levels,
                  double bw_factor, int64_t num_samples, double* vals, double* uni, uint8_t* need_ppf,
                  int64_t* datum, int64_t* stop, int64_t* compact, int64_t* n_compact);

#ifdef __cplusplus
}
#endif

#endif
```

Before: 30550 billion.

## Fold stage-1 interval and block-max into coarse scoring kernel epilogue

```diff
diff --git a/hpbandster_amd/_native.py b/hpbandster_amd/_native.py
--- a/hpbandster_amd/_native.py
+++ b/hpbandster_amd/_native.py
@@ -85,6 +85,7 @@
     "hbx_mapped_host_buffers": (c_i64, []),
     "hbx_kde_ws_offsets": (c_i32, [c_i64, c_i64, c_i64, c_vp]),
     "hbx_kde_acquire_stats": (c_i32, [c_vp, c_i64, c_i64, c_vp]),
+    "hbx_kde_acquire_stage1": (c_i32, [c_vp, c_i64, c_i64, c_vp]),
     "hbx_np_exp": (c_i32, [c_vp, c_i64, c_vp, c_vp]),
     "hbx_kde_pdf_scratch_bytes": (c_i64, [c_i64]),
     "hbx_kde_pdf_exact": (c_i32, [c_vp, c_i64, c_i32, c_vp, c_vp, c_vp, c_i64, c_vp, c_vp, c_i64, c_vp]),
diff --git a/hpbandster_amd/csrc/hbx_acquire.h b/hpbandster_amd/csrc/hbx_acquire.h
--- a/hpbandster_amd/csrc/hbx_acquire.h
+++ b/hpbandster_amd/csrc/hbx_acquire.h
@@ -21,7 +21,7 @@
 struct WsLayout {
   size_t res, U, count, flags, segcnt, segnear, best, key, first1, rescue, est_l, est_g, lo, list, near, exact_l,
       exact_g, part, total;
-  size_t stage, seeds, surv, lpart;
+  size_t stage, seeds, surv, lpart, bmax;
   int32_t list_cap;
 };
 #define STAGED_LIST_CAP 4096
@@ -40,6 +40,7 @@
   uint32_t* stage;
   int32_t *seeds, *surv;
   KdeEst* lpart;
+  float* bmax;
   int32_t list_cap;
   AcqWs(void* workspace, const WsLayout& w) {
     char* ws = (char*)workspace;
@@ -65,6 +66,7 @@
     seeds = (int32_t*)(ws + w.seeds);
     surv = (int32_t*)(ws + w.surv);
     lpart = (KdeEst*)(ws + w.lpart);
+    bmax = (float*)(ws + w.bmax);
     list_cap = w.list_cap;
   }
   KdePairArgs::AcqInitPtrs init() const { return {U, count, flags, first1, res}; }
@@ -89,9 +91,10 @@
 int acq_score_staged(const AcqPlan& plan, const KdePairRef& p, const double* cand, int64_t Nc, const AcqWs& a,
                      hipEvent_t* ev, hipStream_t s, bool tail);
 int staged_score_l(const AcqPlan& plan, const KdePairRef& p, const double* cand, int64_t Nc, const AcqWs& a,
-                   hipEvent_t* ev, hipStream_t s, uint32_t* lkey, uint32_t* hist, int32_t hist_words);
+                   hipEvent_t* ev, hipStream_t s, uint32_t* lkey, uint32_t* hist, int32_t hist_words,
+                   unsigned* lhi_blocks = nullptr);
 int staged_score_seeds(const AcqPlan& plan, const KdePairRef& p, const double* cand, int64_t Nc, const AcqWs& a,
-                       hipStream_t s, bool mark_rest, bool update_u);
+                       hipStream_t s, bool mark_rest, bool update_u, unsigned lhi_blocks = 0);
 int staged_score_survivors(const AcqPlan& plan, const KdePairRef& p, const double* cand, int64_t Nc, const AcqWs& a,
                            hipStream_t s, bool lonly);
 int acq_exact_only_init(int64_t Nc, uint32_t seg, const AcqWs& a, hipStream_t s);
diff --git a/hpbandster_amd/csrc/hbx_common.h b/hpbandster_amd/csrc/hbx_common.h
--- a/hpbandster_amd/csrc/hbx_common.h
+++ b/hpbandster_amd/csrc/hbx_common.h
@@ -5,6 +5,7 @@
 #include <stdlib.h>
 
 #define HBX_MAX_D 256
+#define HBX_LO_TERMS 32
 #define HBX_WAVE 64
 
 #include "hbx.h"
@@ -38,6 +39,7 @@
   return v == 0 ? 0 : v == 2 ? 2 : 1;
 }
 static inline bool hbx_staged_tail() { return hbx_switch_on("HBX_STAGED_TAIL"); }
+static inline bool hbx_stage1_lhi() { return hbx_switch_on("HBX_STAGE1_LHI"); }
 
 struct KdeParams {
   int32_t n;
@@ -87,6 +89,7 @@
   int32_t vartype[HBX_MAX_D];
   int32_t nlev[HBX_MAX_D];
   double bw[HBX_MAX_D];
+  float lo_term[HBX_LO_TERMS];
 };
 
 #define HBX_PARAM_STAGE ((sizeof(KdeParams) + 255) & ~(size_t)255)
diff --git a/hpbandster_amd/csrc/hbx_kde.hip b/hpbandster_amd/csrc/hbx_kde.hip
--- a/hpbandster_amd/csrc/hbx_kde.hip
+++ b/hpbandster_amd/csrc/hbx_kde.hip
@@ -486,6 +486,7 @@
   w.seeds = take(4 * (size_t)w.list_cap);
   w.surv = take(4 * Nc);
   w.lpart = take(sizeof(KdeEst) * (size_t)OBS_SPLIT_MAX * w.list_cap);
+  w.bmax = take(4 * (size_t)((Nc + 255) / 256));
   w.total = o;
   return w;
 }
diff --git a/hpbandster_amd/csrc/hbx_kde_impl.h b/hpbandster_amd/csrc/hbx_kde_impl.h
--- a/hpbandster_amd/csrc/hbx_kde_impl.h
+++ b/hpbandster_amd/csrc/hbx_kde_impl.h
@@ -123,6 +123,30 @@
   const float u = 0x1p-24f;
   const float Mabs = fabsf(ci) + P->cmax + bnd + P->sum_abs_delta;
   const float dt = 3.f * (float)(P->dc + P->du + 4) * u * Mabs;
+  const float es = sum_terms * u * (SIGNED ? 3.f : 1.f);
+  o.err = 2.f * (dt * HBX_LN2f + es) + 16.f * u;
+  return o;
+}
+struct EstPrm {
+  float lnorm, cmax, sum_abs_delta;
+  int32_t dims;
+};
+__device__ __forceinline__ KdeEst finish_est_terms(const EstPrm q, float S, float Sn, float off, bool nan_c, float ci,
+                                                   float bnd, bool SIGNED, float sum_terms) {
+  KdeEst o;
+  o.pad = 0.f;
+  if (nan_c || S != S) {
+    o.lpos = NAN;
+    o.lneg = -INFINITY;
+    o.err = 0.f;
+    return o;
+  }
+  const float Sp = SIGNED ? (S - Sn) : S;
+  o.lpos = (Sp > 0.f) ? (__log2f(Sp) + off) * HBX_LN2f + q.lnorm : -INFINITY;
+  o.lneg = (SIGNED && Sn > 0.f) ? (__log2f(Sn) + off) * HBX_LN2f + q.lnorm : -INFINITY;
+  const float u = 0x1p-24f;
+  const float Mabs = fabsf(ci) + q.cmax + bnd + q.sum_abs_delta;
+  const float dt = 3.f * (float)(q.dims + 4) * u * Mabs;
   const float es = sum_terms * u * (SIGNED ? 3.f : 1.f);
   o.err = 2.f * (dt * HBX_LN2f + es) + 16.f * u;
   return o;
@@ -201,6 +225,8 @@
   unsigned tiles = 0;
   int32_t nsplit0 = 1, nsplit1 = 1;
   int32_t row_stage = 1;
+  float* lhi = nullptr;
+  float* bmax = nullptr;
 };
 typedef void (*logpdf_pair_fn)(const double*, int64_t, int32_t, KdePairArgs);
 typedef void (*logpdf_co_fn)(const double*, int64_t, int32_t, const KdeParams*, const float*, KdeEst*, int32_t);
@@ -226,6 +252,7 @@
   HBX_ST_NSEED,
   HBX_ST_NSURV,
   HBX_ST_NPRE,
+  HBX_ST_LHI1,
   HBX_ST_WORDS
 };
 
@@ -238,6 +265,7 @@
   st[HBX_ST_NSEED] = 0;
   st[HBX_ST_NSURV] = 0;
   st[HBX_ST_NPRE] = 0;
+  st[HBX_ST_LHI1] = 0;
   *U = hbx_f2ord(INFINITY);
   *first1 = INT32_MAX;
   *count = 0;
diff --git a/hpbandster_amd/csrc/hbx_prep.hip b/hpbandster_amd/csrc/hbx_prep.hip
--- a/hpbandster_amd/csrc/hbx_prep.hip
+++ b/hpbandster_amd/csrc/hbx_prep.hip
@@ -173,6 +173,10 @@
       S.cd[ix] = d;
       P->cat_delta[ix] = (a == 0.0) ? -1e30f : (float)(S.t1[d] - S.t0[d]);
       P->cat_negf[ix] = (a < 0.0) ? 1.f : 0.f;
+      if (ix < HBX_LO_TERMS) {
+        const float dl = fminf(fmaxf(P->cat_delta[ix], -60000.f), 60000.f);
+        P->lo_term[ix] = fabsf(dl) < 60000.f ? fabsf(dl - (float)(_Float16)dl) : 0.f;
+      }
       if (a < 0.0) {
         P->has_neg = 1;
         S.neg = 1;
diff --git a/hpbandster_amd/csrc/hbx_score_h32.hip b/hpbandster_amd/csrc/hbx_score_h32.hip
--- a/hpbandster_amd/csrc/hbx_score_h32.hip
+++ b/hpbandster_amd/csrc/hbx_score_h32.hip
@@ -1,5 +1,6 @@
 #include "hbx_common.h"
 #include "hbx_kde_impl.h"
+#include "hbx_acq_impl.h"
 
 typedef float f32x16 __attribute__((ext_vector_type(16)));
 typedef uint32_t u32x2 __attribute__((ext_vector_type(2)));
@@ -56,7 +57,9 @@
                                                     const unsigned blk, int32_t* __restrict__ rescue_cnt = nullptr,
                                                     const int split = 0, const int nsplit = 1,
                                                     const int32_t* __restrict__ idx = nullptr,
-                                                    const bool scatter = false, const bool row_stage = true) {
+                                                    const bool scatter = false, const bool row_stage = true,
+                                                    float* __restrict__ lhi = nullptr,
+                                                    float* __restrict__ bmax = nullptr) {
   constexpr int ND = CO ? h32c_nd(NSC) : h32_nd(NSC);
   constexpr int KS = KP;
   constexpr int KL = (FAST || CO) ? 0 : KP;
@@ -80,10 +83,15 @@
   constexpr int PRM_BYTES = 8 * NSC * (int)sizeof(ContPrm) + 32 * (KP > 0 ? KP : 1) * (int)sizeof(OhPrm);
   constexpr int RDS = !CO ? 0 : ((8 * NSC + 16 * KP) | 1) < H32C_ROW_DS ? ((8 * NSC + 16 * KP) | 1) : H32C_ROW_DS;
   constexpr int RSF = RDS >= (H32C_ROW_DMIN | 1) ? (HW * 32 * RDS * 8 + PRM_BYTES) / 4 : 0;
-  constexpr int LDSF = NBUF * CHF + AUXF > RSF ? NBUF * CHF + AUXF : RSF;
+  constexpr int NLT = CO && KP > 0 ? 16 * KP : 0;
+  static_assert(NLT <= HBX_LO_TERMS, "KdeParams::lo_term");
+  constexpr int EPF = CO ? 8 + NLT : 0;
+  constexpr int LDSB = ((NBUF * CHF + AUXF > RSF ? NBUF * CHF + AUXF : RSF) + 3) & ~3;
+  constexpr int LDSF = LDSB + EPF;
   static_assert(2 * LDSF * 4 <= 160 * 1024, "two blocks per CU");
   __shared__ __align__(16) float lds[LDSF];
   float* aux = lds + NBUF * CHF;
+  float* epi = lds + LDSB;
   if constexpr (CO) table += P->coarse_off;
   int c0 = 0, nchunks = (P->n + OBS_CHUNK - 1) / OBS_CHUNK;
   if (nsplit > 1) {
@@ -119,6 +127,17 @@
                         act ? P->cont_dim[tid] : 0};
   }
   if (tid < 32 * KP) oprm[tid] = OhPrm{P->oh_val[tid], P->oh_col[tid], 0};
+  if constexpr (CO) {
+    if (tid < EPF)
+      epi[tid] = tid == 0   ? (float)P->log_norm
+                 : tid == 1 ? P->cmax
+                 : tid == 2 ? P->sum_abs_delta
+                 : tid == 3 ? __int_as_float(P->dc + P->du)
+                 : tid == 4 ? __int_as_float(P->nconst)
+                 : tid == 5 ? __int_as_float(P->nan_all)
+                 : tid >= 8 ? P->lo_term[tid - 8]
+                            : 0.f;
+  }
   const bool staged = rows_fit && cbase < Nc;
   const int64_t nv = (Nc - cbase) < 32 * CT ? (Nc - cbase) : 32 * CT;
   double* xs = (double*)lds + (int64_t)wave * 32 * (tile_fit ? 1 : CT) * DS;
@@ -441,6 +460,7 @@
 #pragma unroll
   for (int t = 0; t < CT; ++t) S[t] += __shfl_xor(S[t], 32);
   if constexpr (SG) Sn = 2.f * (Sn + __shfl_xor(Sn, 32));
+  if constexpr (!CO) {
 #pragma unroll
   for (int t = 0; t < CT; ++t) {
   if (h == 0) {
@@ -475,6 +495,75 @@
     }
   }
   }
+  } else {
+  const EstPrm eprm{epi[0], epi[1], epi[2], __float_as_int(epi[3])};
+  const int32_t e_nconst = __float_as_int(epi[4]), e_nan = __float_as_int(epi[5]);
+  float lot[NLT > 0 ? NLT : 1];
+#pragma unroll
+  for (int u = 0; u < NLT; ++u) lot[u] = epi[8 + u];
+  float blo = -INFINITY;
+  auto finish = [&](const int t, const float St) {
+    const int64_t ii = cbase + 32 * t + c;
+    if (ii < Nc) {
+      const float* ax = aux + ((wave * CT + t) * 32 + c) * 4;
+      const float ci_q = ax[0], bnd_q = ax[1], dq = ax[2];
+      const bool big = ax[3] < 0.f;
+      const float cer_q = big ? 0.f : ax[3];
+      int64_t irow = ii;
+      if constexpr (LIST) irow = idx[ii];
+      const int64_t iout = LIST && !scatter ? ii : irow;
+      const double* x = cand + irow * (int64_t)D;
+      bool nq = e_nan != 0;
+      for (int k = 0; k < e_nconst; ++k)
+        if (x[P->const_dim[k]] != P->const_level[k]) nq = true;
+      KdeEst o = finish_est_terms(eprm, St, 0.f, -dq, nq, ci_q - dq, bnd_q, false, (float)(nchunks + 6 + 24));
+      if (o.err > 0.f) o.err += (6.f * 0x1p-22f * bnd_q + 0x1p-19f) * HBX_LN2f;
+      float lo_err = cer_q;
+      if constexpr (KP > 0)
+#pragma unroll
+        for (int u = 0; u < NLT; ++u) lo_err += lot[u];
+      if (o.err > 0.f) o.err = (1.f + o.err) * exp2f(lo_err * (1.f + 0x1p-20f)) * (1.f + 0x1p-20f) - 1.f;
+      if (!nq && St == St && (big || St < 0x1p-64f || St > 0x1p100f)) {
+        o.err = -1.f;
+        if (rescue_cnt) atomicAdd(rescue_cnt, 1);
+      }
+      out[iout] = o;
+      if constexpr (!LIST) {
+        if (lhi) {
+          float lo = -INFINITY, hi = NAN, pt;
+          if (o.err == -1.f) {
+            hi = INFINITY;
+          } else if (o.lpos == o.lpos) {
+            est_interval(o, &lo, &hi, &pt);
+            blo = lo;
+          }
+          lhi[iout] = hi;
+        }
+      }
+    }
+  };
+  if constexpr (CT == 2) {
+    finish(h, h ? S[1] : S[0]);
+  } else {
+    if (h == 0) finish(0, S[0]);
+  }
+  if constexpr (!LIST) {
+    if (bmax) {
+#pragma unroll
+      for (int o = 32; o > 0; o >>= 1) blo = fmaxf(blo, __shfl_xor(blo, o));
+      if (lane == 0) aux[wave * CT * 32 * 4] = blo;
+      asm volatile("s_waitcnt lgkmcnt(0)" ::: "memory");
+      __builtin_amdgcn_s_barrier();
+      asm volatile("" ::: "memory");
+      if (threadIdx.x == 0) {
+        float b = aux[0];
+#pragma unroll
+        for (int w = 1; w < HW; ++w) b = fmaxf(b, aux[w * CT * 32 * 4]);
+        bmax[blk] = b;
+      }
+    }
+  }
+  }
 }
 
 template <int NSC, int KP, bool FAST>
@@ -506,7 +595,7 @@
   const int split = ns > 1 ? (int)(loc / a.tiles) : 0;
   kde_logpdf_h32_body<NSC, KP, false, FAST, CO, CO ? H32C_CT : 1>(cand, Nc, D, second ? a.P1 : a.P0, second ? a.table1 : a.table0,
                                                 second ? a.out1 : a.out0, tile, a.rescue, split, ns, nullptr, false,
-                                                a.row_stage != 0);
+                                                a.row_stage != 0, a.lhi, a.bmax);
 }
 
 template <int NSC, int KP>
@@ -523,7 +612,7 @@
   const int split = ns > 1 ? (int)(loc / a.tiles) : 0;
   kde_logpdf_h32_body<NSC, KP, false, false, true, 1>(cand, Nc, D, second ? a.P1 : a.P0, second ? a.table1 : a.table0,
                                                        second ? a.out1 : a.out0, tile, a.rescue, split, ns, nullptr, false,
-                                                       a.row_stage != 0);
+                                                       a.row_stage != 0, a.lhi, a.bmax);
 }
 
 template <int NSC, int KP>
diff --git a/hpbandster_amd/csrc/hbx_staged.hip b/hpbandster_amd/csrc/hbx_staged.hip
--- a/hpbandster_amd/csrc/hbx_staged.hip
+++ b/hpbandster_amd/csrc/hbx_staged.hip
@@ -7,6 +7,7 @@
 
 #define STAGED_PT 4
 #define HBX_LN4f 1.3862943611198906f
+#define STAGED_SEED_BLOCKS 2048
 
 template <bool KEYS>
 __global__ __launch_bounds__(256) void staged_l_kernel(KdeEst* __restrict__ el, int64_t Nc, int32_t ns,
@@ -88,16 +89,48 @@
 __global__ __launch_bounds__(256) void staged_seed_kernel(float* __restrict__ lhi, int64_t Nc,
                                                           KdeEst* __restrict__ eg, int32_t* __restrict__ seeds,
                                                           int32_t cap, uint32_t* __restrict__ stage,
-                                                          int32_t mark_rest) {
-  const float thr = hbx_ord2f(stage[HBX_ST_LMAX]) - HBX_LN4f;
+                                                          int32_t mark_rest, const float* __restrict__ bmax,
+                                                          int32_t nblk, const double* __restrict__ cand, int32_t D,
+                                                          const KdeParams* __restrict__ Pl,
+                                                          KdeEst* __restrict__ el) {
+  float lmax;
+  if (bmax) {
+    __shared__ float rb[4];
+    float m = -INFINITY;
+    for (int j = threadIdx.x; j < nblk; j += 256) m = fmaxf(m, bmax[j]);
+    for (int o = 32; o > 0; o >>= 1) m = fmaxf(m, __shfl_xor(m, o));
+    if ((threadIdx.x & 63) == 0) rb[threadIdx.x >> 6] = m;
+    __syncthreads();
+    lmax = fmaxf(fmaxf(rb[0], rb[1]), fmaxf(rb[2], rb[3]));
+    if (blockIdx.x == 0 && threadIdx.x == 0) {
+      stage[HBX_ST_LMAX] = hbx_f2ord(lmax);
+      stage[HBX_ST_LHI1] = 1;
+    }
+  } else {
+    lmax = hbx_ord2f(stage[HBX_ST_LMAX]);
+  }
+  const float thr = lmax - HBX_LN4f;
+  const int64_t ntile = (Nc + 256 * STAGED_PT - 1) / (256 * STAGED_PT);
+  for (int64_t tb = blockIdx.x; tb < ntile; tb += gridDim.x) {
   bool f[STAGED_PT];
   int n = 0;
 #pragma unroll
   for (int r = 0; r < STAGED_PT; ++r) {
-    const int64_t i = ((int64_t)blockIdx.x * STAGED_PT + r) * 256 + threadIdx.x;
+    const int64_t i = (tb * STAGED_PT + r) * 256 + threadIdx.x;
     f[r] = false;
     if (i < Nc) {
-      const float h = lhi[i];
+      float h = lhi[i];
+      if (bmax && h == INFINITY) {
+        KdeEst e = el[i];
+        if (e.err == -1.f) {
+          e = kde_rescue_one<0, false, true>(cand, i, D, Pl);
+          el[i] = e;
+          float lo, pt;
+          h = NAN;
+          if (e.lpos == e.lpos) est_interval(e, &lo, &h, &pt);
+          lhi[i] = h;
+        }
+      }
       f[r] = h == h && h >= thr;
     }
     n += f[r] ? 1 : 0;
@@ -106,7 +139,7 @@
   const KdeEst none = {0.f, -INFINITY, HBX_EST_NOT_EVAL, 0.f};
 #pragma unroll
   for (int r = 0; r < STAGED_PT; ++r) {
-    const int64_t i = ((int64_t)blockIdx.x * STAGED_PT + r) * 256 + threadIdx.x;
+    const int64_t i = (tb * STAGED_PT + r) * 256 + threadIdx.x;
     if (i >= Nc) continue;
     bool seeded = false;
     if (f[r]) {
@@ -118,6 +151,7 @@
     }
     if (seeded) lhi[i] = NAN;
     else if (mark_rest) eg[i] = none;
+  }
   }
 }
 
@@ -391,7 +425,8 @@
 }
 
 int staged_score_l(const AcqPlan& plan, const KdePairRef& p, const double* cand, int64_t Nc, const AcqWs& a,
-                   hipEvent_t* ev, hipStream_t s, uint32_t* lkey, uint32_t* hist, int32_t hist_words) {
+                   hipEvent_t* ev, hipStream_t s, uint32_t* lkey, uint32_t* hist, int32_t hist_words,
+                   unsigned* lhi_blocks) {
   const ScoreFns& f = plan.fg;
   const PairShape sh = pair_shape(f, true, 1, Nc, p.nmax);
   const int ns = sh.nsplit;
@@ -400,11 +435,18 @@
   ka.tiles = sh.tiles;
   ka.nsplit0 = ka.nsplit1 = ns;
   ka.row_stage = hbx_row_stage();
+  const bool fold = lhi_blocks && !lkey && ns == 1 && hbx_stage1_lhi();
+  if (lhi_blocks) *lhi_blocks = fold ? grid : 0;
+  if (fold) {
+    ka.lhi = a.lo;
+    ka.bmax = a.bmax;
+  }
   if (ev)
     hipExtLaunchKernelGGL(sh.kernel, dim3(grid), dim3(f.threads), 0, s, ev[0], nullptr, 0, cand, Nc, p.D, ka);
   else
     hipLaunchKernelGGL(sh.kernel, dim3(grid), dim3(f.threads), 0, s, cand, Nc, p.D, ka);
   HBX_LAUNCH_CHECK();
+  if (fold) return HBX_OK;
   if (lkey)
     hipLaunchKernelGGL(staged_l_kernel<true>, staged_gsel(Nc), dim3(256), 0, s, a.el, Nc, (int32_t)ns, cand, p.D,
                        p.Pg(), a.rescue, a.lo, a.stage, lkey, hist, hist_words);
@@ -416,10 +458,13 @@
 }
 
 int staged_score_seeds(const AcqPlan& plan, const KdePairRef& p, const double* cand, int64_t Nc, const AcqWs& a,
-                       hipStream_t s, bool mark_rest, bool update_u) {
+                       hipStream_t s, bool mark_rest, bool update_u, unsigned lhi_blocks) {
   const int32_t cap = a.list_cap;
-  hipLaunchKernelGGL(staged_seed_kernel, staged_gsel(Nc), dim3(256), 0, s, a.lo, Nc, a.eg, a.seeds, cap, a.stage,
-                     (int32_t)(mark_rest ? 1 : 0));
+  dim3 gseed = staged_gsel(Nc);
+  if (lhi_blocks && gseed.x > STAGED_SEED_BLOCKS) gseed.x = STAGED_SEED_BLOCKS;
+  hipLaunchKernelGGL(staged_seed_kernel, gseed, dim3(256), 0, s, a.lo, Nc, a.eg, a.seeds, cap, a.stage,
+                     (int32_t)(mark_rest ? 1 : 0), lhi_blocks ? (const float*)a.bmax : (const float*)nullptr,
+                     (int32_t)lhi_blocks, cand, p.D, p.Pg(), a.el);
   HBX_LAUNCH_CHECK();
   const ScoreFns& fb = plan.fb;
   const KdeListArgs la = staged_list_args(plan, p, a);
@@ -450,9 +495,10 @@
 
 int acq_score_staged(const AcqPlan& plan, const KdePairRef& p, const double* cand, int64_t Nc, const AcqWs& a,
                      hipEvent_t* ev, hipStream_t s, bool tail) {
-  int rc = staged_score_l(plan, p, cand, Nc, a, ev, s, nullptr, nullptr, 0);
+  unsigned lhi_blocks = 0;
+  int rc = staged_score_l(plan, p, cand, Nc, a, ev, s, nullptr, nullptr, 0, &lhi_blocks);
   if (rc) return rc;
-  rc = staged_score_seeds(plan, p, cand, Nc, a, s, !tail, true);
+  rc = staged_score_seeds(plan, p, cand, Nc, a, s, !tail, true, lhi_blocks);
   if (rc) return rc;
   rc = staged_score_survivors(plan, p, cand, Nc, a, s, tail);
   if (rc) return rc;
@@ -495,4 +541,15 @@
   return HBX_OK;
 }
 
-}
+int hbx_kde_acquire_stage1(const void* workspace, int64_t Nc, int64_t nmax, int64_t* out) {
+  if (!workspace || !out || Nc < 0) return hbx_fail(HBX_ERR_ARG, "hbx_kde_acquire_stage1: bad arguments");
+  const WsLayout w = ws_layout(Nc, nmax);
+  uint32_t st[HBX_ST_WORDS];
+  HBX_HIP(hipDeviceSynchronize());
+  HBX_HIP(hipMemcpy(st, (const char*)workspace + w.stage, sizeof(st), hipMemcpyDeviceToHost));
+  out[0] = st[HBX_ST_FLAG] == 1 && st[HBX_ST_LHI1] == 1 ? 1 : 0;
+  out[1] = (int64_t)st[HBX_ST_LMAX];
+  return HBX_OK;
+}
+
+}
diff --git a/hpbandster_amd/kde.py b/hpbandster_amd/kde.py
--- a/hpbandster_amd/kde.py
+++ b/hpbandster_amd/kde.py
@@ -412,6 +412,11 @@
         out = (ctypes.c_int64 * 4)()
         N.check(N.lib().hbx_kde_acquire_stats(workspace.data_ptr(), int(Nc), self.nmax, ctypes.addressof(out)))
         return {"staged": bool(out[0]), "seeds": int(out[1]), "survivors": int(out[2]), "evaluated": int(out[3])}
+
+    def acquire_stage1(self, workspace, Nc):
+        out = (ctypes.c_int64 * 2)()
+        N.check(N.lib().hbx_kde_acquire_stage1(workspace.data_ptr(), int(Nc), self.nmax, ctypes.addressof(out)))
+        return {"lhi_epilogue": bool(out[0]), "lmax_bits": int(out[1])}
 
     def acquire(self, cands, index_base=0, logs=False, stream=None, workspace=None, sync=True, events=None,
                 ties="pinned"):
diff --git a/include/hbx.h b/include/hbx.h
--- a/include/hbx.h
+++ b/include/hbx.h
@@ -156,6 +156,7 @@
 void* hbx_kde_result_ptr(void* workspace);
 int hbx_kde_ws_offsets(int64_t Nc, int64_t seg, int64_t nmax, int64_t* out);
 int hbx_kde_acquire_stats(const void* workspace, int64_t Nc, int64_t nmax, int64_t* out);
+int hbx_kde_acquire_stage1(const void* workspace, int64_t Nc, int64_t nmax, int64_t* out);
 
 int64_t hbx_kde_pdf_scratch_bytes(int64_t nmax);
 
```

New measurement: 31830 billion (median of 6 runs). 1.04x the previous value.
